# genomicepidemiology/ccphylo

Measured on AMD Instinct MI355X. Metric: taxa-pairs/sec (dist) + NJ iterations/sec at N taxa, 1/2/4/8 MI355X, higher is better.
Workload: dtype u2 packed codes -> MX-fp4 MFMA (exact integer counts), f64 LT and tree

## Files before the change

ccphylo_amd/csrc/ccg_dnj_form.h:

```cpp
#pragma once
#include <stdio.h>
#include <stdlib.h>

#ifdef __HIPCC__
#define CCG_FORM_HD __host__ __device__ __forceinline__
#else
#define CCG_FORM_HD inline
#endif

#define DNJ_B 128
#define DNJ_BANDS 64
#define DNJ_BANDS_MAX 128
#define SEG 2048
#define LB_SEG_DEFAULT (2 * SEG)
#define TBF 1024
#define FIND_RPT 16
#define PLAN_MAXB 256
#define UHIST 64

CCG_FORM_HD int dnj_umax(int n, int seg) { return n > 2 ? (n - 2) / seg + 1 : 1; }

struct DnjGrid {
	int scan_div = 4, scan_max = 2048, seg_mul = 0, prefold_n = 0;
	int small_wave = 0, adapt_rows = 500;
	int sphase_b = 512;
	int plan_help = 256;
	int scan_cmp = 1, cmp_blocks = 1024;
	long long prune_cells = 20000000;
	int prune_on = 1;
	int s_top = 0, s_bands = -1, s_split_n = 16384, plan_qdelay = 2, scan_wave = -1, plan_multi = 1;
	int plan_regsel = 0, plan_fr = FIND_RPT;
	int test_withhold = 0;
	int join_pf = 1;
	int scan_fold = 0;
	int scan_prune = 2;
	int lb = 1, lb_min_n = 16384;
	int lb_groups = 0;
	int seg_lb = 0, seg_lb_knob = 0;
	int scan_vblk = 1;
	void load() {
		if(const char *e = getenv("CCG_JOIN_PF")) join_pf = atoi(e);
		if(const char *e = getenv("CCG_SCAN_FOLD")) scan_fold = atoi(e);
		if(const char *e = getenv("CCG_SCAN_PRUNE")) scan_prune = atoi(e);
		if(const char *e = getenv("CCG_SCAN_VBLK")) scan_vblk = atoi(e);
		if(const char *e = getenv("CCG_S_TOP")) s_top = atoi(e) > 0 ? atoi(e) : 0;
		if(const char *e = getenv("CCG_S_BANDS")) s_bands = atoi(e) >= 0 ? atoi(e) : -1;
		if(const char *e = getenv("CCG_S_SPLIT_N")) s_split_n = atoi(e);
		if(const char *e = getenv("CCG_SCAN_DIV")) scan_div = atoi(e) > 0 ? atoi(e) : 4;
		if(const char *e = getenv("CCG_SCAN_MAX")) scan_max = atoi(e) > 0 ? atoi(e) : 2048;
		if(const char *e = getenv("CCG_SEG_MUL")) seg_mul = atoi(e) > 0 ? atoi(e) : 0;
		if(const char *e = getenv("CCG_PREFOLD_N")) prefold_n = atoi(e) >= 0 ? atoi(e) : 0;
		if(const char *e = getenv("CCG_SCAN_ADAPT")) adapt_rows = atoi(e) > 0 ? atoi(e) : 0;
		if(const char *e = getenv("CCG_SPHASE_BLOCKS")) sphase_b = atoi(e) > 0 ? atoi(e) : 512;
		if(const char *e = getenv("CCG_PLAN_HELP")) plan_help = atoi(e) >= 0 && atoi(e) < 512 ? atoi(e) : 256;
		if(const char *e = getenv("CCG_SCAN_CMP")) scan_cmp = atoi(e);
		if(const char *e = getenv("CCG_PRUNE_CELLS")) prune_cells = atoll(e) > 0 ? atoll(e) : 0;
		prune_on = 1;
		if(const char *e = getenv("CCG_SCAN_CMPB")) cmp_blocks = atoi(e) > 0 ? atoi(e) : 1024;
		if(const char *e = getenv("CCG_PLAN_QDELAY")) plan_qdelay = atoi(e) >= 0 ? atoi(e) : 2;
		if(const char *e = getenv("CCG_SCAN_WAVE")) scan_wave = atoi(e);
		if(const char *e = getenv("CCG_PLAN_MULTI")) plan_multi = atoi(e);
		if(const char *e = getenv("CCG_PLAN_REGSEL")) plan_regsel = atoi(e);
		if(const char *e = getenv("CCG_PLAN_FR")) plan_fr = atoi(e) < 1 ? 1 : atoi(e) > FIND_RPT ? FIND_RPT : atoi(e);
		if(const char *e = getenv("CCG_TEST_WITHHOLD")) test_withhold = atoi(e) & 3;
		if(const char *e = getenv("CCG_SCAN_LB")) lb = atoi(e);
		if(const char *e = getenv("CCG_LB_MIN_N")) lb_min_n = atoi(e);
		if(const char *e = getenv("CCG_LB_GROUPS")) lb_groups = atoi(e);
		if(const char *e = getenv("CCG_SEG_LB")) {
			char *end;
			const long v = strtol(e, &end, 10);
			if(end != e && !*end && v == 0) seg_lb_knob = -1;
			else if(end != e && !*end && v >= 64 && v <= 8 * SEG && v % 64 == 0) seg_lb_knob = (int) v;
			else fprintf(stderr, "ccphylo_amd: CCG_SEG_LB=%s ignored (0, or a multiple of 64 up to %d)\n", e, 8 * SEG);
		}
	}
	int plan_flags(bool prune = false, int helpers = 0) const {
		return (plan_qdelay & 0x3fff) | (test_withhold & 3) << 14 | (plan_regsel ? 0 : 1 << 16) | ((plan_fr - 1) & 15) << 17 | (prune ? 1 << 21 : 0) |
		       (helpers & 511) << 22;
	}
	unsigned plan_blocks(int n) const {
		if(!plan_multi) return 1;
		const int step = (TBF - 64) * plan_fr;
		const int g = (n - 1 + step - 1) / step;
		return (unsigned) (g < 1 ? 1 : g > PLAN_MAXB ? PLAN_MAXB : g);
	}
	int scan_mode(int n, int et = 8) const {
		return scan_wave >= 0 ? scan_wave : n > 16384 || small_wave ? (et == 8 ? 9 : 20) : 0;
	}
	int seg(int n) const {
		int m = seg_mul ? seg_mul : n / (8 * SEG);
		m = m < 1 ? 1 : m > 8 ? 8 : m;
		return m * SEG;
	}
	int seg_bounded(int n) const { return seg_lb_knob > 0 || seg_lb > seg(n) ? seg_lb : seg(n); }
	bool prefold(int n) const { return n > prefold_n; }
	int top(int n) const {
		const int t = s_top ? s_top : n > s_split_n ? 16 : DNJ_B;
		return t < 1 ? 1 : t > DNJ_B ? DNJ_B : t;
	}
	int bands(int n) const {
		int b = s_bands >= 0 ? s_bands : n > s_split_n ? DNJ_BANDS : 0;
		b = b > DNJ_BANDS_MAX ? DNJ_BANDS_MAX : b;
		return top(n) + b > DNJ_B ? DNJ_B - top(n) : b;
	}
	unsigned sphase_blocks() const { return sphase_b; }
	unsigned scan(int n) const {
		const long long g = (n + scan_div - 1) / scan_div;
		return (unsigned) (g < scan_max ? g : scan_max);
	}
};

enum ScanKernel {
	SCAN_BLOCK,
	SCAN_WAVE,
	SCAN_WAVE16,
	SCAN_GROUP,
	SCAN_GROUP_CMP
};
enum ScanSphase {
	SPHASE_NONE,
	SPHASE_SCAN,
	SPHASE_COMPACT
};
struct ScanForm {
	ScanKernel kernel;
	bool stream;
	int G, UC;
	int prune;
	bool cmp;
	bool lb;
	bool tfold;
	int helpers;
	ScanSphase sphase;
	bool fold;
	int sfold;
	unsigned grid;
	int launches;
	int seg;
};

inline int dnj_scan_base(int sm) {
	return sm <= 0 ? 0 : sm < 4 ? 1 : sm == 9 || sm == 21 || sm > 23 ? sm : sm < 20 ? 4 : 20;
}

inline ScanForm dnj_scan_form(const DnjGrid &g, int n, int et, bool gen, bool have_lbm) {
	const int sm = dnj_scan_base(g.scan_mode(n, et));
	const bool grp = sm == 20 || sm == 21, prefold = g.prefold(n);
	ScanForm f = {};
	f.tfold = prefold && g.scan_fold && sm >= 1;
	const bool lbseg = have_lbm && g.seg_lb > 0 && !gen && sm >= 4 && g.scan_cmp && !f.tfold &&
	                   dnj_umax(n, g.seg_bounded(n)) < UHIST;
	f.seg = lbseg ? g.seg_bounded(n) : g.seg(n);
	const bool fits = dnj_umax(n, f.seg) < UHIST;
	if(!gen && g.bands(n) && prefold && sm >= 4 && sm <= 23) {
		if(g.scan_prune == 1 && g.scan_fold) f.prune = 1;
		else if(g.scan_prune == 2 && g.prune_on && !g.scan_fold && (!grp || (g.scan_cmp && fits))) f.prune = 2;
	}
	f.helpers = f.prune == 2 ? g.plan_help : 0;
	f.sphase = f.prune != 2 ? SPHASE_NONE : g.plan_help ? SPHASE_COMPACT : SPHASE_SCAN;
	f.cmp = !gen && sm >= 4 && g.scan_cmp && !f.tfold && f.prune != 1 && fits;
	if(gen || sm < 4) f.kernel = sm >= 1 ? SCAN_WAVE : SCAN_BLOCK;
	else if(have_lbm && f.cmp && grp && g.lb_groups && f.prune == 0) {
		f.kernel = SCAN_GROUP_CMP;
		f.lb = true;
		f.G = 4;
		f.UC = 8;
	} else if(have_lbm && f.cmp) {
		f.kernel = SCAN_WAVE16;
		f.lb = true;
	} else if(grp) {
		f.kernel = f.cmp ? SCAN_GROUP_CMP : SCAN_GROUP;
		f.G = sm == 21 ? 8 : 4;
		f.UC = sm == 21 ? 4 : 8;
	} else {
		f.kernel = SCAN_WAVE16;
		f.stream = sm == 9;
	}
	f.grid = f.cmp && g.scan(n) > (unsigned) g.cmp_blocks ? (unsigned) g.cmp_blocks : g.scan(n);
	f.fold = prefold && !f.tfold;
	f.sfold = f.prune == 2;
	f.launches = 1 + (f.sphase != SPHASE_NONE) + f.fold;
	return f;
}

inline ScanForm dnj_scan_form_shard(const DnjGrid &g, int n, int et, bool have_lbm) {
	const int sm = g.scan_mode(n, et);
	ScanForm f = {};
	f.kernel = sm >= 4 ? SCAN_WAVE16 : sm >= 1 ? SCAN_WAVE : SCAN_BLOCK;
	f.stream = sm == 9;
	f.lb = have_lbm && sm >= 4;
	f.grid = g.scan(n);
	f.launches = 1;
	f.seg = g.seg(n);
	return f;
}
```

ccphylo_amd/csrc/ccg_dnj_search.h:

```cpp
#pragma once
#include <stdlib.h>
#include "ccg_tree_common.h"
#include "ccg_dnj_form.h"

struct DenseRows {
	__host__ __device__ __forceinline__ bool owns(long long) const { return true; }
	__host__ __device__ __forceinline__ long long row(long long r) const { return tri(r); }
};

#define SEG_S 1024
#define SEL_RPL 8
#define SEL_STEPS 8
#define FIND_CHUNKS 2048
#define REPLAY_CAP 2048
#define JOIN_UPRE 2048
#define FOLD_BLOCKS 256
#define SRDY_REP 64


template <int ET, bool GEN, int NT, int UNR, class Rows>
__device__ __forceinline__ void row_segment_min(const Rows &rows, const typename Elem<ET>::T *__restrict__ D, double bs,
                                                const double *__restrict__ sD, const int *__restrict__ N, int r,
                                                int c0, int c1, int Nr, double sDr, int isub, int Nm, double sDm,
                                                double &q, int &idx) {
	const typename Elem<ET>::T *row = D + rows.row(r);
	typename Elem<ET>::T v[UNR];
	int nk[UNR];
	double sk[UNR];
	auto load = [&](int base, typename Elem<ET>::T (&lv)[UNR], int (&lk)[UNR], double (&ls)[UNR]) {
#pragma unroll
		for(int m = 0; m < UNR; ++m) {
			int c = base + m * NT + (int) threadIdx.x;
			c = c < c1 ? c : c1 - 1;
			lv[m] = row[c];
			lk[m] = GEN ? N[c] : Nr;
			ls[m] = sD[c];
		}
	};
	load(c0, v, nk, sk);
	for(int base = c0; base < c1; base += UNR * NT) {
		typename Elem<ET>::T vn[UNR];
		int nkn[UNR];
		double skn[UNR];
		const bool more = base + UNR * NT < c1;
		if(more) load(base + UNR * NT, vn, nkn, skn);
#pragma unroll
		for(int m = 0; m < UNR; ++m) {
			const int c = base + m * NT + (int) threadIdx.x;
			const double d = Elem<ET>::get(v[m], bs);
			const int Nc = c == isub ? Nm : nk[m];
			const double sc = c == isub ? sDm : sk[m];
			const double x = qcrit(Nr, Nc, d, sDr, sc);
			const bool take = c < c1 && 0 <= d && qarg_better(x, c, q, idx);
			q = take ? x : q;
			idx = take ? c : idx;
		}
		if(more) {
#pragma unroll
			for(int m = 0; m < UNR; ++m) {
				v[m] = vn[m];
				nk[m] = nkn[m];
				sk[m] = skn[m];
			}
		}
	}
}

__device__ __forceinline__ void fold_units(const double *__restrict__ uq, const int *__restrict__ uj, int ua, int ub,
                                           double &q, int &idx) {
	for(int u = ua; u < ub; u += 4) {
		double oq[4];
		int oi[4];
#pragma unroll
		for(int m = 0; m < 4; ++m) {
			const int v = u + m < ub ? u + m : ub - 1;
			oq[m] = uq[v];
			oi[m] = uj[v];
		}
#pragma unroll
		for(int m = 0; m < 4; ++m) {
			if(u + m < ub && qarg_better(oq[m], oi[m], q, idx)) {
				q = oq[m];
				idx = oi[m];
			}
		}
	}
}

__device__ __forceinline__ void qarg_block_reduce1(double &q, int &idx, double *sq, int *si) {
	qarg_wave_reduce(q, idx);
	const int lane = threadIdx.x & 63, wid = threadIdx.x >> 6, nw = blockDim.x >> 6;
	if(lane == 0) {
		sq[wid] = q;
		si[wid] = idx;
	}
	__syncthreads();
	if(threadIdx.x == 0) {
		for(int w = 1; w < nw; ++w) {
			if(qarg_better(sq[w], si[w], q, idx)) {
				q = sq[w];
				idx = si[w];
			}
		}
	}
}

template <int ET, class Rows>
__global__ void k_init_hnj(Rows rows, const typename Elem<ET>::T *__restrict__ D, int n, double bs,
                           const double *__restrict__ sD, const int *__restrict__ N,
                           double *__restrict__ Q, int *__restrict__ P) {
	int i = blockIdx.x * (blockDim.x >> 6) + (threadIdx.x >> 6);
	int lane = threadIdx.x & 63;
	if(i >= n || !rows.owns(i)) return;
	double bq = DBL_MAX, bd = DBL_MAX;
	int bj = 0;
	const typename Elem<ET>::T *row = D + rows.row(i);
	int Ni = N[i];
	double sDi = sD[i];
	for(int j = lane; j < i; j += 64) {
		double d = Elem<ET>::get(row[j], bs);
		const double q = qcrit(Ni, N[j], d, sDi, sD[j]);
		const bool take = (0 <= d) & ((q < bq) | ((q == bq) & ((d < bd) | ((d == bd) & (j > bj)))));
		bq = take ? q : bq;
		bd = take ? d : bd;
		bj = take ? j : bj;
	}
#pragma unroll
	for(int off = 32; off > 0; off >>= 1) {
		const double oq = __shfl_xor(bq, off, 64), od = __shfl_xor(bd, off, 64);
		const int oj = __shfl_xor(bj, off, 64);
		const bool take = (oq < bq) | ((oq == bq) & ((od < bd) | ((od == bd) & (oj > bj))));
		bq = take ? oq : bq;
		bd = take ? od : bd;
		bj = take ? oj : bj;
	}
	if(lane == 0) {
		Q[i] = bq;
		P[i] = bj;
	}
}

template <int UNUSED = 0>
__global__ __launch_bounds__(TB) void k_dnj_prep(TreeBufs b, int n) {
	__shared__ double sq[TB / 64];
	__shared__ int si[TB / 64];
	double q = DBL_MAX;
	int idx = 0;
	for(int i = 1 + threadIdx.x; i < n; i += blockDim.x) {
		if(qarg_better(b.Q[i], i, q, idx)) {
			q = b.Q[i];
			idx = i;
		}
	}
	qarg_block_reduce(q, idx, sq, si);
// ... 1000 lines not shown
		if(last) {
			__hip_atomic_store(b.rf + e, q, __ATOMIC_RELAXED, __HIP_MEMORY_SCOPE_AGENT);
			__hip_atomic_store(b.rj + e, j, __ATOMIC_RELAXED, __HIP_MEMORY_SCOPE_AGENT);
			asm volatile("s_waitcnt vmcnt(0)" ::: "memory");
			if(CHUNKS) {
				const int c = e >> 6, ce = T - (c << 6) < 64 ? T - (c << 6) : 64;
				const unsigned seen = __hip_atomic_fetch_add(b.ccnt + c, 1u, __ATOMIC_RELAXED, __HIP_MEMORY_SCOPE_AGENT);
				if((int) seen == ce - 1) {
					chunk_done = 1;
					__hip_atomic_store(b.ccnt + c, 0u, __ATOMIC_RELAXED, __HIP_MEMORY_SCOPE_AGENT);
				}
			}
			if(sent) {
				const unsigned sseen = __hip_atomic_fetch_add(&b.ctl->scnt, 1u, __ATOMIC_RELAXED,
				                                              __HIP_MEMORY_SCOPE_AGENT);
				s_done = (int) sseen == b.ctl->pS - 1;
			}
		}
	}
	if(__shfl(s_done, 0)) {
		__builtin_amdgcn_fence(__ATOMIC_ACQUIRE, "wavefront");
		s_table(b, n);
	}
	if(!CHUNKS || !__shfl(chunk_done, 0)) return;
	__builtin_amdgcn_fence(__ATOMIC_ACQUIRE, "wavefront");
	const int c = e >> 6, e2 = (c << 6) + lane;
	const bool valid = e2 < T;
	const int rr = valid ? b.crow[e2] : 0;
	const double bnd = valid ? b.cbnd[e2] : 0.0;
	const double f = valid ? __hip_atomic_load(b.rf + e2, __ATOMIC_RELAXED, __HIP_MEMORY_SCOPE_AGENT) : DBL_MAX;
	const int fj = valid ? __hip_atomic_load(b.rj + e2, __ATOMIC_RELAXED, __HIP_MEMORY_SCOPE_AGENT) : 0;
	const double mq = readlane_d(wave_incl_min(f), 63);
	const unsigned long long hm = __ballot(valid && f == mq);
	const unsigned long long bm = __ballot(valid && !(f >= bnd));
	const int first = hm ? __ffsll((long long) hm) - 1 : 0;
	const int fr = __shfl(rr, first), fjj = __shfl(fj, first);
	if(lane == 0) {
		b.chg[c] = mq;
		b.chr[c] = fr;
		b.chj[c] = fjj;
		b.chb[c] = bm != 0ull;
	}
}

__device__ __forceinline__ void tail_unit(const FoldTail &, const TreeBufs &b, int n, int u, int ua, int ub, int r,
                                          double q, int j, int e, int T, bool sent = false) {
	(void) r;
	fold_arrive(b, n, b.cq, b.cj, u, ua, ub, q, j, e, T, sent);
}

template <int ET, bool GEN, class Rows, class Tail = NoTail>
__global__ __launch_bounds__(TB) void k_dnj_scan(const typename Elem<ET>::T *__restrict__ D, double bs, TreeBufs b,
                                                 int n, Rows rows, int seg, Tail tail = Tail()) {
	__shared__ int erow[REPLAY_CAP];
	__shared__ double sq[TB / 64];
	__shared__ int si[TB / 64];
	TreeCtl *ctl = b.ctl;
	const int tid = threadIdx.x;
	TS_ENTRY(2);
	TS(2, 0);
	TS_SAMP(0);
	const int r0 = b.crow[tid];
	const int done = ctl->done, T = ctl->T;
	if(done) return;
	tail.begin(b, n);
	if(T == 0) return;
	const int umax = dnj_umax(n, seg), nunits = T * umax;
	if((int) blockIdx.x >= nunits) return;
	const bool lds = T <= REPLAY_CAP;
	if(lds) {
		if(tid < T) erow[tid] = r0;
		for(int e = TB + tid; e < T; e += TB) erow[e] = b.crow[e];
	}
	__syncthreads();
	TS(2, 1);
	TS_SAMP(1);
	for(int u = blockIdx.x; u < nunits; u += gridDim.x) {
		const int e = u / umax, ua = e * umax;
		const int r = lds ? erow[e] : b.crow[e];
		const int c0 = (u - ua) * seg;
		if(c0 >= r || !rows.owns(r)) continue;
		const int c1 = c0 + seg < r ? c0 + seg : r;
		const int Nr = GEN ? b.N[r] : n;
		double qq = DBL_MAX;
		int idx = 0;
		row_segment_min<ET, GEN, TB, SEG / TB / 2>(rows, D, bs, b.sD, b.N, r, c0, c1, Nr, b.sD[r], -1, 0, 0.0, qq, idx);
		qarg_block_reduce1(qq, idx, sq, si);
		if(tid == 0) tail.unit(b, n, u, ua, ua + dcdiv(r, seg), r, qq, idx);
		if(u + (int) gridDim.x < nunits) __syncthreads();
	}
	TS(2, 2);
	TS_SAMP(2);
	TS_EXIT(2);
}

template <int ET, bool GEN, class Rows, class Tail = NoTail, int SCAN_UW = 8>
__global__ __launch_bounds__(TB) void k_dnj_scan_w(const typename Elem<ET>::T *__restrict__ D, double bs, TreeBufs b,
                                                   int n, Rows rows, int seg, Tail tail = Tail()) {
	__shared__ int erow[REPLAY_CAP];
	TreeCtl *ctl = b.ctl;
	const int tid = threadIdx.x, lane = tid & 63;
	const int r0 = b.crow[tid];
	const int done = ctl->done, T = ctl->T;
	if(done) return;
	tail.begin(b, n);
	if(T == 0) return;
	const int umax = dnj_umax(n, seg), nunits = T * umax;
	if((int) blockIdx.x * (TB / 64) >= nunits) return;
	const bool lds = T <= REPLAY_CAP;
	if(lds) {
		if(tid < T) erow[tid] = r0;
		for(int e = TB + tid; e < T; e += TB) erow[e] = b.crow[e];
	}
	__syncthreads();
	const int gw = blockIdx.x * (TB / 64) + (tid >> 6), nw = gridDim.x * (TB / 64);
	for(int u = gw; u < nunits; u += nw) {
		const int e = u / umax, ua = e * umax;
		const int r = lds ? erow[e] : b.crow[e];
		const int c0 = (u - ua) * seg;
		if(c0 >= r || !rows.owns(r)) continue;
		const int c1 = c0 + seg < r ? c0 + seg : r;
		const int Nr = GEN ? b.N[r] : n;
		const double sDr = b.sD[r];
		const typename Elem<ET>::T *row = D + rows.row(r);
		double q = DBL_MAX;
		int idx = 0;
		for(int base = c0; base < c1; base += 64 * SCAN_UW) {
			typename Elem<ET>::T v[SCAN_UW];
			double sk[SCAN_UW];
			int nk[SCAN_UW];
#pragma unroll
			for(int m = 0; m < SCAN_UW; ++m) {
				int c = base + 64 * m + lane;
				c = c < c1 ? c : c1 - 1;
				v[m] = row[c];
				sk[m] = b.sD[c];
				nk[m] = GEN ? b.N[c] : Nr;
			}
#pragma unroll
			for(int m = 0; m < SCAN_UW; ++m) {
				const int c = base + 64 * m + lane;
				const double d = Elem<ET>::get(v[m], bs);
				const double x = qcrit(Nr, nk[m], d, sDr, sk[m]);
				const bool take = c < c1 && 0 <= d && qarg_better(x, c, q, idx);
				q = take ? x : q;
				idx = take ? c : idx;
			}
		}
		qarg_wave_reduce(q, idx);
		tail_unit(tail, b, n, u, ua, ua + dcdiv(r, seg), r, q, idx, e, T);
	}
}

static_assert(8 * SEG <= 4 * 64 * LBW && SEG_S <= 4 * 64 * LBW, "lb_unit loads at most 256 block bounds per unit");
template <int ET>
__device__ __forceinline__ int lb_unit(const typename Elem<ET>::T *__restrict__ row, double bs, const TreeBufs &b, int n,
                                       int r, int c0, int c1, double sDr, double &q, int &idx, int isub,
                                       double sDm, bool ubinf) {
	typedef typename Elem<ET>::T T;
	constexpr int BB = ET == 8 ? LB_BB_D : LB_BB_N;
	const int lane = threadIdx.x & 63;
	const int bl0 = c0 / LBW, nbk = (c1 - c0 + LBW - 1) / LBW;
	const double ub = ubinf ? INFINITY : b.ubq[r];
	unsigned lbb[4];
	double msb[4];
	const unsigned *line = lb_line(b, r);
#pragma unroll
	for(int h = 0; h < 4; ++h) {
		const int t = lane + 64 * h;
		lbb[h] = t < nbk ? line[bl0 + t] : 0u;
		msb[h] = t < nbk ? b.msd[bl0 + t] : 0.0;
	}
	unsigned long long need[4];
#pragma unroll
	for(int h = 0; h < 4; ++h) {
		const int t = lane + 64 * h;
		const double lb = qcrit(n, n, (double) __uint_as_float(lbb[h]), sDr, msb[h]);
		need[h] = __ballot(t < nbk && !(lb > ub));
	}
	int loaded = 0;
	int h = 0;
	while(true) {
		int blk[BB], nb = 0;
		while(nb < BB && h < 4) {
			if(!need[h]) {
				++h;
				continue;
			}
			const int bit = __ffsll((long long) need[h]) - 1;
			need[h] &= need[h] - 1;
			blk[nb++] = bl0 + 64 * h + bit;
		}
		if(!nb) break;
		T v[BB];
		double sk[BB];
#pragma unroll
		for(int m = 0; m < BB; ++m) {
			int c = (m < nb ? blk[m] : blk[0]) * LBW + lane;
			c = c < c1 ? c : c1 - 1;
			v[m] = row[c];
			sk[m] = b.sD[c];
		}
#pragma unroll
		for(int m = 0; m < BB; ++m) {
			const int c = (m < nb ? blk[m] : blk[0]) * LBW + lane;
			const double d = Elem<ET>::get(v[m], bs);
			const double x = qcrit(n, n, d, sDr, c == isub ? sDm : sk[m]);
			if(m < nb && c < c1 && 0 <= d && qarg_better(x, c, q, idx)) {
				q = x;
				idx = c;
			}
		}
		for(int m = 0; m < nb; ++m) loaded += (blk[m] + 1) * LBW < c1 ? LBW : c1 - blk[m] * LBW;
	}
	return (c1 - c0) - loaded;
}

template <int ET, int G>
__device__ __forceinline__ long long lb_unit_g(const typename Elem<ET>::T *const (&row)[G], double bs, const TreeBufs &b,
                                               int n, const int (&r)[G], const bool (&act)[G], int c0,
                                               const int (&c1)[G], int cmax, const double (&sDr)[G], double (&q)[G],
                                               int (&idx)[G]) {
	typedef typename Elem<ET>::T T;
	constexpr int BB = ET == 8 ? LB_BB_D : LB_BB_N;
	const int lane = threadIdx.x & 63;
	const int bl0 = c0 / LBW, nbkm = (cmax - c0 + LBW - 1) / LBW;
	double msb[4];
#pragma unroll
	for(int h = 0; h < 4; ++h) {
		const int t = lane + 64 * h;
		msb[h] = t < nbkm ? b.msd[bl0 + t] : 0.0;
	}
	unsigned long long need[G][4], any[4] = {0, 0, 0, 0};
#pragma unroll
	for(int k = 0; k < G; ++k) {
		const int nbk = act[k] ? (c1[k] - c0 + LBW - 1) / LBW : 0;
		const double ub = act[k] ? b.ubq[r[k]] : 0.0;
		const unsigned *line = lb_line(b, act[k] ? r[k] : 1);
#pragma unroll
		for(int h = 0; h < 4; ++h) {
			const int t = lane + 64 * h;
			const unsigned lbv = t < nbk ? line[bl0 + t] : 0u;
			const double lb = qcrit(n, n, (double) __uint_as_float(lbv), sDr[k], msb[h]);
			need[k][h] = __ballot(t < nbk && !(lb > ub));
			any[h] |= need[k][h];
		}
	}
	long long loaded = 0;
	int h = 0;
	while(true) {
		int blk[BB], nb = 0;
		while(nb < BB && h < 4) {
			if(!any[h]) {
				++h;
				continue;
			}
			const int bit = __ffsll((long long) any[h]) - 1;
			any[h] &= any[h] - 1;
			blk[nb++] = 64 * h + bit;
		}
		if(!nb) break;
		double sk[BB];
		T v[G][BB];
#pragma unroll
		for(int m = 0; m < BB; ++m) {
			const int t = m < nb ? blk[m] : blk[0];
			int c = (bl0 + t) * LBW + lane;
			sk[m] = b.sD[c < cmax ? c : cmax - 1];
#pragma unroll
			for(int k = 0; k < G; ++k) {
				v[k][m] = 0;
				if((need[k][t >> 6] >> (t & 63)) & 1)
					v[k][m] = row[k][c < c1[k] ? c : c1[k] - 1];
			}
		}
#pragma unroll
		for(int m = 0; m < BB; ++m) {
			const int t = m < nb ? blk[m] : blk[0];
			const int c = (bl0 + t) * LBW + lane;
#pragma unroll
			for(int k = 0; k < G; ++k) {
				if(m >= nb || !((need[k][t >> 6] >> (t & 63)) & 1)) continue;
				const double d = Elem<ET>::get(v[k][m], bs);
				const double x = qcrit(n, n, d, sDr[k], sk[m]);
				if(c < c1[k] && 0 <= d && qarg_better(x, c, q[k], idx[k])) {
					q[k] = x;
					idx[k] = c;
				}
			}
		}
		for(int m = 0; m < nb; ++m) {
			const int c = (bl0 + blk[m]) * LBW;
#pragma unroll
			for(int k = 0; k < G; ++k)
				if((need[k][blk[m] >> 6] >> (blk[m] & 63)) & 1) loaded += c + LBW < c1[k] ? LBW : c1[k] - c;
		}
	}
	long long span = 0;
#pragma unroll
	for(int k = 0; k < G; ++k) span += act[k] ? c1[k] - c0 : 0;
	return span - loaded;
}

template <int ET, class Rows, class Tail = NoTail, bool STREAM = false, int PRUNE = 0, bool CMP = false, bool LB = false>
__global__ __launch_bounds__(TB) void k_dnj_scan_v(const typename Elem<ET>::T *__restrict__ D, double bs, TreeBufs b,
                                                   int n, Rows rows, int seg, Tail tail = Tail()) {
	typedef typename Elem<ET>::T T;
	static_assert(!(LB && PRUNE == 1), "the block bounds serve the compacted scan (its S units fold elsewhere)");
	constexpr int VEC = 16 / (int) sizeof(T), UV = VEC >= 16 ? 1 : 16 / VEC;
	__shared__ int erow[REPLAY_CAP];
	TreeCtl *ctl = b.ctl;
	const int tid = threadIdx.x, lane = tid & 63;
	TS_ENTRY(2);
	TS(2, 0);
	TS_SAMP(0);
	const int r0 = b.crow[tid];
	const int done = ctl->done, Tn = ctl->T;
	if(done) return;
	tail.begin(b, n);
	if(Tn == 0) return;
	const int umax = dnj_umax(n, seg), nunits = Tn * umax;
	const int nSp = PRUNE ? ctl->pS : 0;
	const int su0 = PRUNE == 1 && nSp ? b.pS_uo[nSp] : 0;
	if((int) blockIdx.x * (TB / 64) >= (nunits > su0 ? nunits : su0)) return;
	const bool lds = Tn <= REPLAY_CAP;
	if(lds) {
		if(tid < Tn) erow[tid] = r0;
		for(int e = TB + tid; e < Tn; e += TB) erow[e] = b.crow[e];
	}
	__syncthreads();
	const int gw = blockIdx.x * (TB / 64) + (tid >> 6), nw = gridDim.x * (TB / 64);
	TS(2, 1);
	TS_SAMP(1);
	__shared__ int s_uo[DNJ_B + 1];
	int su = 0;
	if(PRUNE == 1 && nSp) {
		for(int t = tid; t <= nSp; t += TB) s_uo[t] = b.pS_uo[t];
		__syncthreads();
		su = s_uo[nSp];
	}
	long long pruned = 0, lbskip = 0;
	auto unit = [&](int u, int e, int r, int c0, int c1, bool skip, bool sent, int sua, int sub) {
		const int ua = e * umax;
		if(skip) {
			pruned += c1 - c0;
			tail_unit(tail, b, n, u, ua, ua + dcdiv(r, seg), r, DBL_MAX, 0, e, Tn);
			return;
		}
		const double sDr = b.sD[r];
		const long long ro = rows.row(r);
		const T *row = D + ro;
		if(LB) {
			double q = DBL_MAX;
			int idx = 0;
			lbskip += lb_unit<ET>(row, bs, b, n, r, c0, c1, sDr, q, idx);
			qarg_wave_reduce(q, idx);
			tail_unit(tail, b, n, u, ua, ua + dcdiv(r, seg), r, q, idx, e, Tn);
			return;
		}
		const int a = (int) ((VEC - (ro + c0) % VEC) % VEC);
		const int ca = c0 + a < c1 ? c0 + a : c1;
		const int nv = (c1 - ca) / VEC, ce = ca + nv * VEC;
		double q = DBL_MAX;
		int idx = 0;
		auto cell = [&](int c) {
			const double d = Elem<ET>::get(row[c], bs);
			const double x = qcrit(n, n, d, sDr, b.sD[c]);
			if(0 <= d && qarg_better(x, c, q, idx)) {
				q = x;
				idx = c;
			}
		};
		if(lane < ca - c0) cell(c0 + lane);
		if(lane < c1 - ce) cell(ce + lane);
		uint4 w[UV];
		double sk[UV][VEC];
		const bool sda = STREAM && (ca & 1) == 0;
		auto load = [&](int v0) {
#pragma unroll
			for(int m = 0; m < UV; ++m) {
				int k = v0 + 64 * m + lane;
				k = k < nv ? k : nv - 1;
				const uint4 *src = (const uint4 *) (row + ca + VEC * k);
				if(STREAM) {
					typedef unsigned u4v __attribute__((ext_vector_type(4)));
					const u4v x = __builtin_nontemporal_load((const u4v *) src);
					w[m] = make_uint4(x.x, x.y, x.z, x.w);
				} else {
					w[m] = *src;
				}
				if(sda) {
#pragma unroll
					for(int t = 0; t < VEC; t += 2) {
						const double2 x = *(const double2 *) (b.sD + ca + VEC * k + t);
						sk[m][t] = x.x;
						sk[m][t + 1] = x.y;
					}
				} else {
#pragma unroll
					for(int t = 0; t < VEC; ++t) sk[m][t] = b.sD[ca + VEC * k + t];
				}
			}
		};
		auto compare = [&](int v0) {
#pragma unroll
			for(int m = 0; m < UV; ++m) {
				const int k = v0 + 64 * m + lane;
				const T *ev = (const T *) &w[m];
#pragma unroll
				for(int t = 0; t < VEC; ++t) {
					const int c = ca + VEC * k + t;
					const double d = Elem<ET>::get(ev[t], bs);
					const double x = qcrit(n, n, d, sDr, sk[m][t]);
					const bool take = k < nv && 0 <= d && qarg_better(x, c, q, idx);
					q = take ? x : q;
					idx = take ? c : idx;
				}
			}
		};
		for(int v0 = 0; v0 < nv; v0 += 64 * UV) {
			load(v0);
			compare(v0);
		}
		qarg_wave_reduce(q, idx);
		if(PRUNE == 1 && sent) fold_arrive(b, n, b.uq, b.uj, u, sua, sub, q, idx, e, Tn, true);
		else tail_unit(tail, b, n, u, ua, ua + dcdiv(r, seg), r, q, idx, e, Tn);
	};
	for(int v = gw; v < su; v += nw) {
		int lo = 0, hi = nSp;
		while(hi - lo > 1) {
			const int mid = (lo + hi) >> 1;
			if(s_uo[mid] <= v) lo = mid; else hi = mid;
		}
		const int r = b.pS_row[lo], c0 = (v - s_uo[lo]) * SEG_S;
		unit(v, b.pS_ent[lo], r, c0, c0 + SEG_S < r ? c0 + SEG_S : r, false, true, s_uo[lo], s_uo[lo + 1]);
	}
	SBound sb;
	bool have_sb = false, ready = false;
	if(PRUNE == 1 && nSp && (int) blockIdx.x * (TB / 64) < nunits) {
		__shared__ int s_ready;
		__syncthreads();
		if(tid == 0) s_ready = s_table_wait(b, n);
		__syncthreads();
		ready = s_ready;
	}
	if(PRUNE == 2 && nSp) ready = b.srdy[0] == (unsigned) n;
	int nu = 0;
	(void) nu;
	if(CMP && PRUNE == 2 && nSp) {
		int H = 0;
		const int pb = ctl->pblk;
		for(int g = 0; g < pb; ++g) H += b.uhist[g * UHIST + lane];
		const int inch = wave_incl_sum(H), Eall = __builtin_amdgcn_readlane(inch, 63) - inch;
		const int cnt = b.bcnt[lane];
		const int incc = wave_incl_sum(cnt), totc = __builtin_amdgcn_readlane(incc, 63);
		const int Es = totc - incc;
		const int C = totc - incc + cnt;
		int R;
		const int P = wave_excl_scan(Es, &R);
		for(int v = gw; v < R; v += nw) {
			const int k = 63 - __clzll((long long) __ballot(Es > 0 && P <= v));
			const int j = v - __shfl(P, k);
			const int ub = 63 - __clzll((long long) __ballot(lane > k && C > j));
			const int p = j - (__shfl(C, ub) - __shfl(cnt, ub));
			const int e = b.blist[__shfl(Eall, ub) + p];
			const int r = lds ? erow[e] : b.crow[e];
			const int c0 = k * seg;
			TS_U(2 * nu);
			unit(e * umax + k, e, r, c0, c0 + seg < r ? c0 + seg : r, false, false, 0, 0);
			TS_U(2 * nu + 1);
			++nu;
		}
	} else if(CMP) {
		int H = 0;
		const int pb = ctl->pblk;
		for(int g = 0; g < pb; ++g) H += b.uhist[g * UHIST + lane];
		int tot;
		const int inc = wave_incl_sum(H);
		tot = __builtin_amdgcn_readlane(inc, 63);
		const int E = tot - inc;
		int R;
		const int P = wave_excl_scan(E, &R);
		for(int v = gw; v < R; v += nw) {
			const unsigned long long mk = __ballot(E > 0 && P <= v);
			const int k = 63 - __clzll((long long) mk);
			const int e = v - __shfl(P, k);
			const int r = lds ? erow[e] : b.crow[e];
			const int c0 = k * seg;
			bool skip = false;
			if(PRUNE == 2 && nSp) {
				if(b.eS[e]) continue;
				if(!have_sb) {
					sb.load(b, n, ready);
					have_sb = true;
				}
				skip = sb.ok && !(b.cbnd[e] < sb.at(r));
			}
			TS_U(2 * nu);
			unit(e * umax + k, e, r, c0, c0 + seg < r ? c0 + seg : r, skip, false, 0, 0);
			TS_U(2 * nu + 1);
			++nu;
		}
	}
	for(int u = CMP ? nunits : gw; u < nunits; u += nw) {
		const int e = u / umax, ua = e * umax;
		const int r = lds ? erow[e] : b.crow[e];
		const int c0 = (u - ua) * seg;
		if(c0 >= r || !rows.owns(r)) continue;
// ... 170 lines not shown
		if(tid < Tn) erow[tid] = r0;
		for(int e = TB + tid; e < Tn; e += TB) erow[e] = b.crow[e];
	}
	int su = 0;
	if(PRUNE && nSp)
		for(int t = tid; t <= nSp; t += TB) s_uo[t] = b.pS_uo[t];
	__syncthreads();
	if(PRUNE && nSp) su = s_uo[nSp];
	const int gw = blockIdx.x * (TB / 64) + (tid >> 6), nw = gridDim.x * (TB / 64);
	long long pruned = 0;
	for(int v = gw; v < su; v += nw) {
		int lo = 0, hi = nSp;
		while(hi - lo > 1) {
			const int mid = (lo + hi) >> 1;
			if(s_uo[mid] <= v) lo = mid; else hi = mid;
		}
		const int e = b.pS_ent[lo], r = b.pS_row[lo], c0 = (v - s_uo[lo]) * SEG_S;
		const int c1 = c0 + SEG_S < r ? c0 + SEG_S : r;
		const double sDr = b.sD[r];
		const T *row = D + tri(r);
		double q = DBL_MAX;
		int idx = 0;
		for(int base = c0; base < c1; base += 64 * UC) {
			double sk[UC];
			T vv[UC];
#pragma unroll
			for(int m = 0; m < UC; ++m) {
				const int c = base + 64 * m + lane;
				const int cc = c < c1 ? c : c1 - 1;
				sk[m] = b.sD[cc];
				vv[m] = row[cc];
			}
#pragma unroll
			for(int m = 0; m < UC; ++m) {
				const int c = base + 64 * m + lane;
				const double d = Elem<ET>::get(vv[m], bs);
				const double x = qcrit(n, n, d, sDr, sk[m]);
				const bool take = c < c1 && 0 <= d && qarg_better(x, c, q, idx);
				q = take ? x : q;
				idx = take ? c : idx;
			}
		}
		qarg_wave_reduce(q, idx);
		fold_arrive(b, n, b.uq, b.uj, v, s_uo[lo], s_uo[lo + 1], q, idx, e, Tn, true);
	}
	SBound sb;
	bool have_sb = false, ready = false;
	if(PRUNE && nSp && (int) blockIdx.x * (TB / 64) < nunits) {
		__shared__ int s_ready;
		__syncthreads();
		if(tid == 0) s_ready = s_table_wait(b, n);
		__syncthreads();
		ready = s_ready;
	}
	for(int u = gw; u < nunits; u += nw) {
		const int g = u / umax, s = u - g * umax, c0 = s * seg;
		int r[G], c1[G];
		bool act[G], skip[G];
		int cmax = c0;
#pragma unroll
		for(int k = 0; k < G; ++k) {
			const int e = g * G + k;
			r[k] = e < Tn ? (lds ? erow[e] : b.crow[e]) : 0;
			act[k] = e < Tn && c0 < r[k];
			skip[k] = false;
			if(PRUNE && nSp && act[k] && b.eS[e]) act[k] = false;
		}
		if(PRUNE && nSp) {
			bool any = false;
#pragma unroll
			for(int k = 0; k < G; ++k) any = any || act[k];
			if(any && !have_sb) {
				sb.load(b, n, ready);
				have_sb = true;
			}
			if(any && sb.ok) {
#pragma unroll
				for(int k = 0; k < G; ++k) {
					if(act[k] && !(b.cbnd[g * G + k] < sb.at(r[k]))) {
						skip[k] = true;
						act[k] = false;
					}
				}
			}
		}
#pragma unroll
		for(int k = 0; k < G; ++k) {
			c1[k] = act[k] ? (c0 + seg < r[k] ? c0 + seg : r[k]) : c0;
			cmax = c1[k] > cmax ? c1[k] : cmax;
		}
		if(PRUNE) {
#pragma unroll
			for(int k = 0; k < G; ++k) {
				if(!skip[k]) continue;
				const int e = g * G + k;
				pruned += (c0 + seg < r[k] ? c0 + seg : r[k]) - c0;
				tail_unit(FoldTail(), b, n, e * umax + s, e * umax, e * umax + dcdiv(r[k], seg), r[k], DBL_MAX, 0, e,
				          Tn);
			}
		}
		if(cmax == c0) continue;
		double sDr[G], q[G];
		int idx[G];
		const T *row[G];
#pragma unroll
		for(int k = 0; k < G; ++k) {
			sDr[k] = act[k] ? b.sD[r[k]] : 0.0;
			row[k] = D + tri(act[k] ? r[k] : 1);
			q[k] = DBL_MAX;
			idx[k] = 0;
		}
		for(int base = c0; base < cmax; base += 64 * UC) {
			double sk[UC];
			T v[G][UC];
#pragma unroll
			for(int m = 0; m < UC; ++m) {
				const int c = base + 64 * m + lane;
				sk[m] = b.sD[c < cmax ? c : cmax - 1];
#pragma unroll
				for(int k = 0; k < G; ++k) v[k][m] = row[k][c < c1[k] ? c : (act[k] ? c1[k] - 1 : 0)];
			}
#pragma unroll
			for(int m = 0; m < UC; ++m) {
				const int c = base + 64 * m + lane;
#pragma unroll
				for(int k = 0; k < G; ++k) {
					const double d = Elem<ET>::get(v[k][m], bs);
					const double x = qcrit(n, n, d, sDr[k], sk[m]);
					const bool take = c < c1[k] && 0 <= d && qarg_better(x, c, q[k], idx[k]);
					q[k] = take ? x : q[k];
					idx[k] = take ? c : idx[k];
				}
			}
		}
#pragma unroll
		for(int k = 0; k < G; ++k) {
			if(!act[k]) continue;
			double qq = q[k];
			int ii = idx[k];
			qarg_wave_reduce(qq, ii);
			const int e = g * G + k;
			if(FOLD) {
				tail_unit(FoldTail(), b, n, e * umax + s, e * umax, e * umax + dcdiv(r[k], seg), r[k], qq, ii, e, Tn);
			} else if(lane == 0) {
				b.cq[e * umax + s] = qq;
				b.cj[e * umax + s] = ii;
			}
		}
	}
	if(PRUNE && pruned && lane == 0)
		atomicAdd((unsigned long long *) &ctl->cells_pruned, (unsigned long long) pruned);
}

template <int ET, int G, int UC, bool PRUNE2, bool LB = false>
__global__ __launch_bounds__(TB) void k_dnj_scan_gc(const typename Elem<ET>::T *__restrict__ D, double bs, TreeBufs b,
                                                    int n, int seg) {
	typedef typename Elem<ET>::T T;
	static_assert(!(LB && PRUNE2), "the bounded row groups run without S-bound pruning");
	const TreeCtl *ctl = b.ctl;
	const int tid = threadIdx.x, lane = tid & 63;
	const int done = ctl->done, Tn = ctl->T;
	if(done || Tn == 0) return;
	const int umax = dnj_umax(n, seg);
	const int nSp = PRUNE2 ? ctl->pS : 0;
	const bool surv = PRUNE2 && nSp > 0;
	const int gw = blockIdx.x * (TB / 64) + (tid >> 6), nw = gridDim.x * (TB / 64);
	int H = 0;
	const int pb = ctl->pblk;
	for(int g = 0; g < pb; ++g) H += b.uhist[g * UHIST + lane];
	const int inch = wave_incl_sum(H), Eall = __builtin_amdgcn_readlane(inch, 63) - inch;
	const int cnt = surv ? b.bcnt[lane] : H;
	const int incc = wave_incl_sum(cnt), totc = __builtin_amdgcn_readlane(incc, 63);
	const int Es = totc - incc;
	const int C = Es + cnt;
	const int NG = (Es + G - 1) / G;
	int R;
	const int PG = wave_excl_scan(NG, &R);
	long long lbskip = 0;
	for(int v = gw; v < R; v += nw) {
		const int k = 63 - __clzll((long long) __ballot(NG > 0 && PG <= v));
		const int grp = v - __shfl(PG, k), EsK = __shfl(Es, k);
		const int c0 = k * seg;
		int r[G], e[G], c1[G];
		bool act[G];
		int cmax = c0;
#pragma unroll
		for(int t = 0; t < G; ++t) {
			const int pos = grp * G + t;
			act[t] = pos < EsK;
			e[t] = 0;
			r[t] = 1;
			if(act[t]) {
				if(surv) {
					const int ub = 63 - __clzll((long long) __ballot(lane > k && C > pos));
					const int pin = pos - (__shfl(C, ub) - __shfl(cnt, ub));
					e[t] = b.blist[__shfl(Eall, ub) + pin];
				} else {
					e[t] = pos;
				}
				r[t] = b.crow[e[t]];
			}
			c1[t] = act[t] ? (c0 + seg < r[t] ? c0 + seg : r[t]) : c0;
			cmax = c1[t] > cmax ? c1[t] : cmax;
		}
		double sDr[G], q[G];
		int idx[G];
		const T *row[G];
#pragma unroll
		for(int t = 0; t < G; ++t) {
			sDr[t] = act[t] ? b.sD[r[t]] : 0.0;
			row[t] = D + tri(act[t] ? r[t] : 1);
			q[t] = DBL_MAX;
			idx[t] = 0;
		}
		if(LB) lbskip += lb_unit_g<ET, G>(row, bs, b, n, r, act, c0, c1, cmax, sDr, q, idx);
		for(int base = c0; !LB && base < cmax; base += 64 * UC) {
			double sk[UC];
			T vv[G][UC];
#pragma unroll
			for(int m = 0; m < UC; ++m) {
				const int c = base + 64 * m + lane;
				sk[m] = b.sD[c < cmax ? c : cmax - 1];
#pragma unroll
				for(int t = 0; t < G; ++t) vv[t][m] = row[t][c < c1[t] ? c : (act[t] ? c1[t] - 1 : 0)];
			}
#pragma unroll
			for(int m = 0; m < UC; ++m) {
				const int c = base + 64 * m + lane;
#pragma unroll
				for(int t = 0; t < G; ++t) {
					const double d = Elem<ET>::get(vv[t][m], bs);
					const double x = qcrit(n, n, d, sDr[t], sk[m]);
					const bool take = c < c1[t] && 0 <= d && qarg_better(x, c, q[t], idx[t]);
					q[t] = take ? x : q[t];
					idx[t] = take ? c : idx[t];
				}
			}
		}
#pragma unroll
		for(int t = 0; t < G; ++t) {
			if(!act[t]) continue;
			double qq = q[t];
			int ii = idx[t];
			qarg_wave_reduce(qq, ii);
			if(lane == 0) {
				b.cq[e[t] * umax + k] = qq;
				b.cj[e[t] * umax + k] = ii;
			}
		}
	}
	if(LB && lbskip && lane == 0)
		atomicAdd((unsigned long long *) (b.lbskip + (long long) ((blockIdx.x * (TB / 64) + (tid >> 6)) % LB_SCAN) * LB_SLOT),
		          (unsigned long long) lbskip);
}

template <int UNUSED = 0>
__global__ __launch_bounds__(TB) void k_dnj_fold(TreeBufs b, int n, int seg, int sfold = 0) {
	const TreeCtl *ctl = b.ctl;
	if(ctl->done) return;
	const int T = ctl->T, lane = threadIdx.x & 63, umax = dnj_umax(n, seg);
	sfold = sfold && ctl->pS > 0;
	if(blockIdx.x == 0 && threadIdx.x < UHIST) b.bcnt[threadIdx.x] = 0;
	const int nc = (T + 63) >> 6;
	const int w0 = (int) (blockIdx.x * (TB / 64) + (threadIdx.x >> 6)), nw = (int) (gridDim.x * (TB / 64));
	for(int c = w0; c < nc; c += nw) {
		const int e = (c << 6) + lane;
		const bool valid = e < T;
		const int r = valid ? b.crow[e] : 0;
		const double bnd = valid ? b.cbnd[e] : 0.0;
		const bool sdone = sfold && valid && b.eS[e], pruned = sfold && valid && !sdone && b.ePr[e];
		const int ua = e * umax, ub = ua + (valid && !sdone && !pruned ? dcdiv(r, seg) : 0);
		double q = sdone ? b.rf[e] : DBL_MAX;
		int idx = sdone ? b.rj[e] : 0;
		int u = ua;
		for(; u + 4 <= ub; u += 4) {
			double oq[4];
			int oi[4];
#pragma unroll
			for(int m = 0; m < 4; ++m) {
				oq[m] = b.cq[u + m];
				oi[m] = b.cj[u + m];
			}
#pragma unroll
			for(int m = 0; m < 4; ++m) {
				if(qarg_better(oq[m], oi[m], q, idx)) {
					q = oq[m];
					idx = oi[m];
				}
			}
		}
		for(; u < ub; ++u) {
			const double oq = b.cq[u];
			const int oi = b.cj[u];
			if(qarg_better(oq, oi, q, idx)) {
				q = oq;
				idx = oi;
			}
		}
		if(valid && !sdone) {
			b.rf[e] = q;
			b.rj[e] = idx;
		}
		const double mq = readlane_d(wave_incl_min(valid ? q : DBL_MAX), 63);
		const unsigned long long hm = __ballot(valid && q == mq);
		const unsigned long long bm = __ballot(valid && !(q >= bnd));
		const int first = hm ? __ffsll((long long) hm) - 1 : 0;
		const int fr = __shfl(r, first), fj = __shfl(idx, first);
		if(lane == 0) {
			b.chg[c] = mq;
			b.chr[c] = fr;
			b.chj[c] = fj;
			b.chb[c] = bm != 0ull;
		}
	}
}

__device__ __forceinline__ void replay_wave(int total, double m0, const int *e_row, const int *e_j, const double *e_b,
                            const double *e_f, unsigned char *e_acc, bool writer, const TreeBufs &b, int &pi,
                            int &pj, bool *had_bad, int n, unsigned char *acc_out = nullptr) {
	(void) n;
	const int lane = threadIdx.x & 63;
	int bad = 0;
	for(int e0 = lane; e0 < total; e0 += 256) {
		double f[4], bb[4];
#pragma unroll
		for(int k = 0; k < 4; ++k) {
			const int e = e0 + 64 * k < total ? e0 + 64 * k : total - 1;
			f[k] = e_f[e];
			bb[k] = e_b[e];
		}
#pragma unroll
		for(int k = 0; k < 4; ++k) {
			if(e0 + 64 * k < total) {
				bad |= !(f[k] >= bb[k]);
				e_acc[e0 + 64 * k] = 0;
			}
		}
	}
	const bool any_bad = __any(bad);
	*had_bad = any_bad;
	wave_sync();
	TS(3, 6);
	if(any_bad) {
		double m = m0;
		int start = 0;
		for(;;) {
			int hit = -1;
			double cm = m;
			for(int c0 = start; c0 < total; c0 += 64) {
				const int e = c0 + lane;
				const bool valid = e < total;
				const double f = valid ? e_f[e] : DBL_MAX, bb = valid ? e_b[e] : DBL_MAX;
				const bool good = valid && f >= bb;
				const double x = wave_incl_min(good ? f : DBL_MAX);
				double pre = dpp_d<DPP_WAVE_SHR1, 0xF>(DBL_MAX, x);
				pre = pre < cm ? pre : cm;
				const unsigned long long hm = __ballot(valid && !good && bb < pre);
				if(hm) {
					hit = c0 + __ffsll((long long) hm) - 1;
					break;
				}
				const double last = readlane_d(x, 63);
				cm = last < cm ? last : cm;
			}
			if(hit < 0) break;
			if(lane == 0) e_acc[hit] = 1;
			m = e_f[hit];
			start = hit + 1;
// ... 77 lines not shown
```

ccphylo_amd/csrc/ccg_tree_common.h:

```cpp
#pragma once
#include <string.h>
#include "ccg_internal.h"

#define TB 256
#define NJ_RB 8
#define NJ_SEG (TB * 8)

struct Entry {
	double f, bnd;
	int row, j;
};

struct TreeCtl {
	int done;
	int final_n;
	int njoins;
	int i, j;
	double Li, Lj, Dij;
	int cand;
	double cand_q;
	int cand_p;
	int pos_i, pos_j;
	int nS, smin;
	int ntop;
	int T;
	double m0;
	unsigned tick;
	int neg, exact, method, has_missing;
	int serial_sums, serial_replays;
	int chain_sums;
	int xnj;
	double xsum;
	long long rows, cells, cells_top, cells_rest;
	long long ref_rows, ref_cells;
	int hj, hi, hjb, hib;
	int rtotal;
	int pS;
	unsigned scnt;
	long long cells_pruned;
	long long cells_help;
	long long cells_lbskip;
	int vtag;
	int pblk;
	int xs_why[8];
};

struct XsBlk;
struct XsCross;
struct XsTie;

struct TreeBufs {
	double *sD, *Q, *contrib;
	int *N, *P;
	int *S, *uoff;
	double *Sb;
	double *uq;
	int *uj;
	Entry *Sent;
	double *ef, *eb;
	int *erow, *ej;
	unsigned char *eacc;
	int *crow;
	double *cbnd;
	int *coff;
	double *cq;
	int *cj;
	double *wsum, *wabs;
	int *wcnt, *wexp;
	double *qpart;
	int *ipart;
	double *cfq;
	int *cfp;
	long long *fpart;
	double *bmq;
	int *bmr, *bmp;
	double *bmqp;
	int *Spos;
	int *cslot;
	double *rf;
	int *rj;
	ccg_join *joins;
	TreeCtl *ctl;
	unsigned long long *xagg;
	XsBlk *xblk;
	XsCross *xcr;
	XsTie *xti;
	unsigned long long *ppub;
	unsigned long long *jpub;
	double *chg;
	int *chr, *chj, *chb;
	unsigned *ecnt, *ccnt;
	int *pS_row, *pS_ent, *pS_uo;
	double *pS_q, *pS_bnd;
	unsigned char *eS;
	double *bmv, *vsuf;
	int *bcnt, *blist;
	unsigned char *ePr;
	unsigned long long *shdr;
	double *sfq;
	int *sfj;
	unsigned *ecS;
	int *uhist;
	unsigned *srdy;
	int maxu;
	unsigned *lbm;
	double *msd;
	double *ubq;
	long long lbs;
	int lbw;
	int xs_allpre;
	long long *lbskip;
};

#define LBW 64
#define LB_SLOT 16
#define LB_SCAN 4096
#define LB_HELP 8192

__device__ __forceinline__ unsigned *lb_line(const TreeBufs &b, int r) {
	const long long p = b.lbw ? (long long) ((r >> 3) / b.lbw) * 8 + (r & 7) : r;
	return b.lbm + p * b.lbs;
}

__device__ __forceinline__ unsigned lb_bits(double x) {
	return x > 0.0 ? __float_as_uint(__double2float_rd(x)) : 0u;
}


struct TreeWork {
	TreeBufs b;
	void *mem;
};
int ccg_tree_alloc(DevMem &mem, TreeWork *w, int n, hipStream_t st);
size_t ccg_tree_bytes(int n);
int ccg_tree_linkage_impl(ccg_ctx *ctx, const ccg_tree_args *a, void *Dd, ccg_join *joins, int *njoins, int *final_n,
                          double *final_d, int64_t *stats);

__host__ __device__ static inline unsigned cdiv(long long a, long long b) { return (unsigned) ((a + b - 1) / b); }
__device__ __forceinline__ int dcdiv(int a, int b) { return (a + b - 1) / b; }

__device__ __forceinline__ int block_excl_scan(int v, int *s, int *total) {
	const int lane = threadIdx.x & 63, wid = threadIdx.x >> 6, nw = blockDim.x >> 6;
	const int x = wave_incl_sum(v);
	if(lane == 63) s[wid] = x;
	__syncthreads();
	int pre = 0, tot = 0;
	for(int w = 0; w < nw; ++w) {
		if(w < wid) pre += s[w];
		tot += s[w];
	}
	__syncthreads();
	*total = tot;
	return pre + x - v;
}

__device__ __forceinline__ void wave_sync() {
	__builtin_amdgcn_fence(__ATOMIC_RELEASE, "wavefront");
	__builtin_amdgcn_wave_barrier();
	__builtin_amdgcn_fence(__ATOMIC_ACQUIRE, "wavefront");
}

__device__ __forceinline__ int wave_excl_scan(int v, int *total) {
	const int inc = wave_incl_sum(v);
	*total = __builtin_amdgcn_readlane(inc, 63);
	return inc - v;
}

__device__ __forceinline__ double wave_sum_fixed(double x) {
#define S_(C, R) x += dpp_d<C, R>(0.0, x);
	CCG_DPP_STEPS(S_)
#undef S_
	return readlane_d(x, 63);
}

__device__ __forceinline__ int wave_sum_int(int v) { return __builtin_amdgcn_readlane(wave_incl_sum(v), 63); }
__device__ __forceinline__ long long wave_sum_int(long long v) { return readlane_l(wave_incl_sum_l(v), 63); }
__device__ __forceinline__ int wave_min_int(int v) { return __builtin_amdgcn_readlane(wave_incl_min_i(v), 63); }
__device__ __forceinline__ unsigned wave_min_u32(unsigned v) {
#define S_(C, R)                                                          \
	{                                                                     \
		const unsigned t_ = (unsigned) dpp_i<C, R>((int) 0xFFFFFFFFu, (int) v); \
		v = t_ < v ? t_ : v;                                              \
	}
	CCG_DPP_STEPS(S_)
#undef S_
	return (unsigned) __builtin_amdgcn_readlane((int) v, 63);
}
__device__ __forceinline__ double wave_max_d(double x) {
#define S_(C, R)                                   \
	{                                              \
		const double t_ = dpp_d<C, R>(-DBL_MAX, x); \
		x = t_ > x ? t_ : x;                       \
	}
	CCG_DPP_STEPS(S_)
#undef S_
	return readlane_d(x, 63);
}

static __device__ void limb_length(double *Li, double *Lj, double sDi, double sDj, int Ni_, int Nj_, double Dij, int neg) {
	int Ni = Ni_ - 2, Nj = Nj_ - 2;
	if(0 < Ni && 0 < Nj) {
		double delta = ((sDi - Dij) / Ni) - ((sDj - Dij) / Nj);
		*Li = (Dij + delta) / 2;
		*Lj = (Dij - delta) / 2;
		if(!neg) {
			if(*Li < 0) {
				*Lj = Dij;
				*Li = 0;
			} else if(*Lj < 0) {
				*Li = Dij;
				*Lj = 0;
			}
		}
	} else if(0 < Ni) {
		*Li = 0;
		*Lj = Dij;
	} else if(0 < Nj) {
		*Li = Dij;
		*Lj = 0;
	} else {
		*Li = *Lj = Dij / 2;
	}
}

__device__ __forceinline__ int low_exp(double x) {
	unsigned long long u = (unsigned long long) __double_as_longlong(x);
	int ex = (int) ((u >> 52) & 0x7FF);
	unsigned long long m = u & ((1ull << 52) - 1);
	if(ex == 0x7FF) return INT32_MIN;
	if(ex == 0) {
		if(m == 0) return INT32_MAX;
		return -1074 + __ffsll((long long) m) - 1;
	}
	m |= 1ull << 52;
	return ex - 1075 + __ffsll((long long) m) - 1;
}

__device__ __forceinline__ void update_partials(const TreeBufs &b, int n, bool exact, int k, double d, int cnt,
                                                int slot) {
	__shared__ double ssum[TB / 64], sabs[TB / 64];
	__shared__ int scnt[TB / 64], sexp[TB / 64];
	if(exact && k < n) b.contrib[k] = d;
	const double s = wave_sum_fixed(d), a = wave_sum_fixed(fabs(d));
	cnt = wave_sum_int(cnt);
	const int e = wave_min_int(low_exp(d));
	const int lane = threadIdx.x & 63, wid = threadIdx.x >> 6;
	if(lane == 0) {
		ssum[wid] = s;
		sabs[wid] = a;
		scnt[wid] = cnt;
		sexp[wid] = e;
	}
	__syncthreads();
	if(threadIdx.x == 0) {
		double t = 0, ta = 0;
		int c = 0, te = INT32_MAX;
		for(int w = 0; w < TB / 64; ++w) {
			t += ssum[w];
			ta += sabs[w];
			c += scnt[w];
			te = sexp[w] < te ? sexp[w] : te;
		}
		b.wsum[slot] = t;
		b.wabs[slot] = ta;
		b.wcnt[slot] = c;
		b.wexp[slot] = te;
	}
}


static __device__ void fold_update_wave(const TreeBufs &b, int G, bool exact, bool general, double *sd_out, int *nj_out,
                                 bool *need_serial) {
	const int lane = threadIdx.x & 63;
	*need_serial = false;
	if(general) {
		*sd_out = b.wsum[0];
		*nj_out = 1 + b.wcnt[0];
		return;
	}
	double s = 0, a = 0;
	int c = 0, e = INT32_MAX;
	for(int g = lane; g < G; g += 64) {
		s += b.wsum[g];
		a += b.wabs[g];
		c += b.wcnt[g];
		int oe = b.wexp[g];
		e = oe < e ? oe : e;
	}
	const double sd = wave_sum_fixed(s);
	a = wave_sum_fixed(a);
	c = wave_sum_int(c);
	e = wave_min_int(e);
	if(exact) {
		bool provable = e != INT32_MIN && (e == INT32_MAX || (e > -1000 && a * (1.0 + 1e-9) < ldexp(1.0, 53 + e)));
		*need_serial = !provable;
	}
	*sd_out = sd;
	*nj_out = 1 + c;
}

#define XC_CH 1024
template <int NT>
static __device__ double serial_sum_t(const double *__restrict__ c, int n) {
	constexpr int PER = XC_CH / NT;
	__shared__ __attribute__((aligned(16))) double buf[2 * XC_CH];
	__shared__ double s_sd;
	double sd = 0;
	double nxt[PER];
#pragma unroll
	for(int m = 0; m < PER; ++m) {
		int kk = m * NT + threadIdx.x;
		buf[m * NT + threadIdx.x] = kk < n ? c[kk] : 0.0;
	}
	__syncthreads();
	for(int c0 = 0, p = 0; c0 < n; c0 += XC_CH, p ^= 1) {
#pragma unroll
		for(int m = 0; m < PER; ++m) {
			int kk = c0 + XC_CH + m * NT + threadIdx.x;
// ... 967 lines not shown
```

ccphylo_amd/csrc/ccg_tree_run.h:

```cpp
#pragma once
#include <vector>
#include "ccg_tree_common.h"

struct KTimer {
	bool on = false;
	hipStream_t st;
	hipEvent_t ev[1025];
	int cls[1025];
	int used;
	long long cnt[CCG_NKSTAT], ns[CCG_NKSTAT];
	void init(hipStream_t s, bool enable) {
		abort();
		on = enable;
		st = s;
		used = 0;
		memset(cnt, 0, sizeof(cnt));
		memset(ns, 0, sizeof(ns));
		if(on) {
			for(int k = 0; k < 1025; ++k) hipEventCreate(&ev[k]);
			hipEventRecord(ev[0], st);
			used = 1;
		}
	}
	void harvest() {
		hipEventSynchronize(ev[used - 1]);
		for(int k = 1; k < used; ++k) {
			float ms = 0;
			hipEventElapsedTime(&ms, ev[k - 1], ev[k]);
			cnt[cls[k]] += 1;
			ns[cls[k]] += (long long) (ms * 1.0e6);
		}
		hipEvent_t t = ev[0];
		ev[0] = ev[used - 1];
		ev[used - 1] = t;
		used = 1;
	}
	void mark(int c) {
		if(!on) return;
		cls[used] = c;
		hipEventRecord(ev[used++], st);
		if(used == 1025) harvest();
	}
	void abort() {
		if(!on) return;
		for(int k = 0; k < 1025; ++k) hipEventDestroy(ev[k]);
		on = false;
	}
	void finish() {
		if(!on) return;
		harvest();
		abort();
	}
};

static inline TreeCtl tree_ctl_seed(const ccg_tree_args *a) {
	TreeCtl c;
	memset(&c, 0, sizeof(c));
	c.neg = (a->flags & 2) != 0;
	c.exact = a->exact != 0;
	c.method = a->method;
	c.hj = c.hi = -1;
	return c;
}

struct TreeStats {
	long long rows = 0, cells = 0, launches = 0, us = 0;
	long long cells_top = 0, cells_rest = 0, serial_sums = 0, chain_sums = 0;
	long long slot8 = 0;
	long long hard_columns = 0;
	long long ref_rows = 0, ref_cells = 0;
	void write(int64_t *stats, bool profile, const KTimer &kt) const {
		if(!stats) return;
		stats[0] = rows;
		stats[1] = cells;
		stats[2] = launches;
		stats[3] = us;
		if(!profile) return;
		for(int c = 0; c < CCG_NKSTAT; ++c) {
			stats[4 + 2 * c] = kt.cnt[c];
			stats[5 + 2 * c] = kt.ns[c];
		}
		const long long tail[8] = {cells_top, cells_rest, serial_sums, chain_sums, slot8, hard_columns, ref_rows, ref_cells};
		for(int k = 0; k < 8; ++k) stats[4 + 2 * CCG_NKSTAT + k] = tail[k];
	}
};

template <class Ctl>
struct TreeRun {
	ccg_ctx *ctx;
	hipStream_t st;
	const Ctl *dctl;
	KTimer kt;
	long long launches = 0;
	int since_check = 0;
	float ms = 0;
	TreeRun(ccg_ctx *c, const Ctl *device_ctl) : ctx(c), st(c->stream), dctl(device_ctl) {}
	TreeRun(const TreeRun &) = delete;
	~TreeRun() {
		kt.abort();
		hipStreamSynchronize(st);
	}
	int read_ctl(Ctl &h) {
		CCG_CHECK(hipMemcpyAsync(&h, dctl, sizeof(h), hipMemcpyDeviceToHost, st));
		CCG_CHECK(hipStreamSynchronize(st));
		return CCG_OK;
	}
	int begin(const Ctl &seed, bool profile) {
		CCG_CHECK(hipMemcpyAsync((void *) dctl, &seed, sizeof(seed), hipMemcpyHostToDevice, st));
		CCG_CHECK(hipEventRecord(ctx->ev0, st));
		kt.init(st, profile);
		return CCG_OK;
	}
	int check(Ctl &h, bool *read) {
		*read = ++since_check == 1024;
		if(!*read) return CCG_OK;
		since_check = 0;
		return read_ctl(h);
	}
	int finish(Ctl &h, int n, const ccg_join *dev_joins, ccg_join *joins, int *njoins, int *final_n, double *final_d) {
		CCG_CHECK(hipEventRecord(ctx->ev1, st));
		kt.finish();
		CCG_TRY(read_ctl(h));
		CCG_CHECK(hipEventElapsedTime(&ms, ctx->ev0, ctx->ev1));
		if(h.done && h.final_n < 0) {
			ccg_set_last_msg("k_dnj_plan / k_dnj_join: a block's bounded wait on another block timed out");
			return CCG_EHIP;
		}
		*njoins = h.njoins;
		*final_n = h.done ? h.final_n : n;
		*final_d = -1.0;
		if(h.njoins) CCG_CHECK(hipMemcpyAsync(joins, dev_joins, (size_t) h.njoins * sizeof(ccg_join), hipMemcpyDeviceToHost, st));
		return CCG_OK;
	}
	template <int ET>
	int final_distance(const void *dev_src, double bs, double *final_d) {
		typename Elem<ET>::T v;
		CCG_CHECK(hipMemcpyAsync(&v, dev_src, sizeof(v), hipMemcpyDeviceToHost, st));
		CCG_CHECK(hipStreamSynchronize(st));
		*final_d = (ET == 8 || ET == 4) ? (double) v : v / bs;
		return CCG_OK;
	}
	TreeStats stats() const {
		TreeStats s;
		s.launches = launches;
		s.us = (long long) (ms * 1000.0);
		return s;
	}
	int end() {
		CCG_CHECK(hipStreamSynchronize(st));
		return CCG_OK;
	}
};

struct LbLayout {
	long long LS;
	size_t lbb, msb, ubb, skb;
	size_t bytes() const { return lbb + msb + ubb + skb; }
};
static inline LbLayout lb_layout(int n0, long long owned_rows) {
	LbLayout l;
	l.LS = (n0 + LBW - 1) / LBW;
	l.lbb = ((size_t) owned_rows * l.LS * 4 + 255) & ~(size_t) 255;
	l.msb = ((size_t) (l.LS + 1) * 8 + 255) & ~(size_t) 255;
	l.ubb = ((size_t) n0 * 8 + 255) & ~(size_t) 255;
	l.skb = (size_t) (LB_SCAN + LB_HELP) * LB_SLOT * 8;
	return l;
}
static inline int lb_bind(TreeBufs &b, void *mem, const LbLayout &l, int lbw, hipStream_t st) {
	char *m = (char *) mem;
	b.lbm = (unsigned *) m;
	b.msd = (double *) (m + l.lbb);
	b.ubq = (double *) (m + l.lbb + l.msb);
	b.lbs = l.LS;
	b.lbw = lbw;
	b.lbskip = (long long *) (m + l.lbb + l.msb + l.ubb);
	CCG_CHECK(hipMemsetAsync(b.lbskip, 0, l.skb, st));
	return CCG_OK;
}
static inline int lb_harvest(const TreeBufs &b, size_t slots, hipStream_t st, TreeCtl &h) {
	if(!b.lbskip) return CCG_OK;
	std::vector<long long> sl(slots * LB_SLOT);
	CCG_CHECK(hipMemcpyAsync(sl.data(), b.lbskip, sl.size() * 8, hipMemcpyDeviceToHost, st));
	CCG_CHECK(hipStreamSynchronize(st));
	for(size_t x = 0; x < slots; ++x) {
		h.cells_lbskip += sl[x * LB_SLOT];
		h.cells_help -= sl[x * LB_SLOT + 1];
	}
	return CCG_OK;
}
```

ccphylo_amd/csrc/tree.hip:

```cpp
#include <string.h>
#include <stdio.h>
#include <vector>
#include <stdlib.h>
#include "ccg_tree_run.h"

#include "ccg_dnj_search.h"

static thread_local DnjGrid g_grid;

template <int ET>
__global__ __launch_bounds__(TB) void k_init_rows(const typename Elem<ET>::T *__restrict__ D, int n, double bs,
                                                  double *__restrict__ sD, int *__restrict__ N, TreeCtl *ctl) {
	__shared__ double buf[TB / 64][64];
	const int lane = threadIdx.x & 63, wid = threadIdx.x >> 6;
	const int k = blockIdx.x * (TB / 64) + wid;
	if(k >= n) return;
	double s = 0;
	int c = 1, miss = 0;
	const typename Elem<ET>::T *row = D + tri(k);
	for(int m0 = 0; m0 < k; m0 += 64) {
		int m = m0 + lane;
		double d = m < k ? Elem<ET>::get(row[m], bs) : 0.0;
		bool ok = m < k && 0 <= d;
		miss |= m < k && !ok;
		c += __popcll(__ballot(ok));
		buf[wid][lane] = ok ? d : 0.0;
		__builtin_amdgcn_wave_barrier();
		if(lane == 0) {
			int lim = k - m0 < 64 ? k - m0 : 64;
			for(int u = 0; u < lim; ++u) s += buf[wid][u];
		}
		__builtin_amdgcn_wave_barrier();
	}
	miss = __any(miss);
	if(lane == 0) {
		sD[k] = s;
		N[k] = c;
		if(miss) atomicOr(&ctl->has_missing, 1);
	}
}

template <int ET>
__global__ __launch_bounds__(TB) void k_init_cols(const typename Elem<ET>::T *__restrict__ D, int n, double bs,
                                                  double *__restrict__ sD, int *__restrict__ N, TreeCtl *ctl) {
	const int k = blockIdx.x * TB + threadIdx.x;
	if(k >= n) return;
	double s = sD[k];
	int c = N[k], miss = 0;
	for(int m = k + 1; m < n; ++m) {
		double d = Elem<ET>::get(D[tri(m) + k], bs);
		if(0 <= d) {
			s += d;
			++c;
		} else {
			miss = 1;
		}
	}
	sD[k] = s;
	N[k] = c;
	if(miss) atomicOr(&ctl->has_missing, 1);
}

template <int ET>
__device__ __forceinline__ void update_body(typename Elem<ET>::T *__restrict__ D, double bs, const TreeBufs &b, int n,
                                            int i, int j, double Dij, bool exact, int k, double Dik, double Dkj,
                                            double sDk, int Nk, int slot) {
	double d = 0;
	int cnt = 0;
	typename Elem<ET>::T v = 0;
	if(k < n && k != i && k != j) {
		d = (Dik + Dkj - Dij) / 2;
		d = d < 0 ? 0 : d;
		v = Elem<ET>::put(d, 0.25, bs);
		D[k < j ? tri(j) + k : tri(k) + j] = v;
		b.sD[k] = sDk - (Dik + Dkj - d);
		b.N[k] = Nk - 1;
		cnt = 1;
	}
	if(b.lbm) {
		const bool rowj = k < j;
		const unsigned x = lb_bits(Elem<ET>::get(v, bs));
		const unsigned mn = wave_min_u32(rowj ? x : 0xFFFFFFFFu);
		if((threadIdx.x & 63) == 0 && k < j) b.lbm[(long long) j * b.lbs + (k >> 6)] = mn;
		if(k > j && k < n && k != i) __hip_atomic_fetch_min(b.lbm + (long long) k * b.lbs + (j >> 6), x, __ATOMIC_RELAXED, __HIP_MEMORY_SCOPE_AGENT);
	}
	update_partials(b, n, exact, k, d, cnt, slot);
	if(exact) xs_join_row(b, n, slot, d, xs_tag(n));
}


template <int ET>
__device__ __forceinline__ void join_tail(typename Elem<ET>::T *__restrict__ D, double bs, const TreeBufs &b, int n,
                                          int general, int i, int j, int ci, int cj, typename Elem<ET>::T pij,
                                          typename Elem<ET>::T pik, typename Elem<ET>::T pkj, double sDk, int Nk,
                                          int neg, int nj, int exact) {
	TreeCtl *ctl = b.ctl;
	const int tid = threadIdx.x, k = blockIdx.x * TB + tid;
	const bool writer = blockIdx.x == 0;
	if(i == 0 && j == 0) {
		if(writer && tid == 0) {
			ctl->done = 1;
			ctl->final_n = n;
		}
		return;
	}
	const bool hit = i == ci && j == cj;
	const double Dij = Elem<ET>::get(hit ? pij : D[tri(i) + j], bs);
	double Dik = 0, Dkj = 0;
	if(!general && k < n && k != i && k != j) {
		Dik = Elem<ET>::get(hit ? pik : D[k < i ? tri(i) + k : tri(k) + i], bs);
		Dkj = Elem<ET>::get(hit ? pkj : D[k < j ? tri(j) + k : tri(k) + j], bs);
	}
	if(writer && tid == 0) {
		double Li, Lj;
		limb_length(&Li, &Lj, b.sD[i], b.sD[j], b.N[i], b.N[j], Dij, neg);
		ctl->i = i;
		ctl->j = j;
		ctl->Li = Li;
		ctl->Lj = Lj;
		ctl->Dij = Dij;
		ccg_join J;
		J.i = i;
		J.j = j;
		J.Li = Li;
		J.Lj = Lj;
		b.joins[nj] = J;
		ctl->njoins = nj + 1;
	}
	TS(3, 4);
	if(general) return;
	update_body<ET>(D, bs, b, n, i, j, Dij, exact, k, Dik, Dkj, sDk, Nk, blockIdx.x);
	TS(3, 5);
}

template <int ET>
__global__ __launch_bounds__(TB) void k_lb_init(const typename Elem<ET>::T *__restrict__ D, int n, double bs,
                                                TreeBufs b) {
	constexpr int BB = 8;
	const int lane = threadIdx.x & 63;
	const int r = blockIdx.x * (TB / 64) + (threadIdx.x >> 6);
	if(r >= n) return;
	if(r < (n + LBW - 1) / LBW) {
		const int c = r * LBW + lane;
		const double mx = wave_max_d(c < n ? b.sD[c] : -DBL_MAX);
		if(lane == 0) b.msd[r] = mx;
	}
	if(lane == 0) b.ubq[r] = INFINITY;
	const typename Elem<ET>::T *row = D + tri(r);
	const int nbk = (r + LBW - 1) / LBW;
	for(int u0 = 0; u0 < nbk; u0 += BB) {
		unsigned x[BB];
#pragma unroll
		for(int m = 0; m < BB; ++m) {
			const int c = (u0 + m) * LBW + lane;
			x[m] = u0 + m < nbk && c < r ? lb_bits(Elem<ET>::get(row[c], bs)) : 0xFFFFFFFFu;
		}
#pragma unroll
		for(int m = 0; m < BB; ++m) {
			const unsigned mn = wave_min_u32(x[m]);
			if(lane == 0 && u0 + m < nbk) b.lbm[(long long) r * b.lbs + u0 + m] = mn;
		}
	}
}

template <int ET, bool GEN>
__global__ __launch_bounds__(TB) void k_dnj_join(typename Elem<ET>::T *__restrict__ D, double bs, TreeBufs b, int n,
                                                 int general, int prefold, int seg) {
	__shared__ int e_row[DNJ_B + REPLAY_CAP], e_j[DNJ_B + REPLAY_CAP];
	__shared__ double e_b[DNJ_B + REPLAY_CAP], e_f[DNJ_B + REPLAY_CAP];
	__shared__ unsigned char e_acc[DNJ_B + REPLAY_CAP];
	__shared__ int s_pi, s_pj, s_stop, s_nj, s_neg, s_exact, s_nS, s_merged;
	__shared__ double s_m0;
	__shared__ double lq[JOIN_UPRE];
	__shared__ int lj[JOIN_UPRE];
	TreeCtl *ctl = b.ctl;
	const int tid = threadIdx.x, lane = tid & 63, wid = tid >> 6;
	const bool writer = blockIdx.x == 0;
	TS_ENTRY(3);
	TS(3, 0);
	const int k = blockIdx.x * TB + tid;
	int ci = ctl->pos_i, cj = ctl->pos_j;
	ci = ci < 0 || ci >= n ? 0 : ci;
	cj = cj < 0 || cj >= ci ? 0 : cj;
	typename Elem<ET>::T pik = 0, pkj = 0;
	double sDk = 0;
	int Nk = 0;
	if(!general && k < n) {
		sDk = b.sD[k];
		Nk = b.N[k];
		if(k != ci && k != cj) {
			pik = D[k < ci ? tri(ci) + k : tri(k) + ci];
			pkj = D[k < cj ? tri(cj) + k : tri(k) + cj];
		}
	}
	const typename Elem<ET>::T pij = D[tri(ci) + cj];
	if(prefold) {
#pragma unroll
		for(int m = 0; m < JOIN_UPRE / TB; ++m) {
			lq[tid + m * TB] = b.rf[tid + m * TB];
			lj[tid + m * TB] = b.rj[tid + m * TB];
		}
	} else {
#pragma unroll
		for(int m = 0; m < JOIN_UPRE / TB; ++m) {
			lq[tid + m * TB] = b.cq[tid + m * TB];
			lj[tid + m * TB] = b.cj[tid + m * TB];
		}
	}
	__syncthreads();
	if(wid == 0) {
		const int done = ctl->done, nS = ctl->nS, T = ctl->T;
		const bool merged = ctl->ntop != nS;
		const int pos_i = ctl->pos_i, pos_j = ctl->pos_j;
		const double m0 = ctl->m0;
		Entry se0, se1;
		se0 = b.Sent[lane];
		se1 = b.Sent[lane + 64];
		const int sp0 = merged ? b.Spos[lane] : lane, sp1 = merged ? b.Spos[lane + 64] : lane + 64;
		int rr[4], cs[4];
		double bb[4];
#pragma unroll
		for(int m = 0; m < 4; ++m) {
			cs[m] = merged ? b.cslot[lane + 64 * m] : nS + lane + 64 * m;
			rr[m] = b.crow[lane + 64 * m];
			bb[m] = b.cbnd[lane + 64 * m];
		}
		const int umax = dnj_umax(n, seg);
		if(lane == 0) {
			s_nj = ctl->njoins;
			s_neg = ctl->neg;
			s_exact = ctl->exact;
		}
		if(done) {
			if(lane == 0) s_stop = 1;
		} else {
			TS(3, 1);
			int pi = pos_i, pj = pos_j;
			const bool lds = T <= REPLAY_CAP;
			int *x_row = lds ? e_row : b.erow, *x_j = lds ? e_j : b.ej;
			double *x_b = lds ? e_b : b.eb, *x_f = lds ? e_f : b.ef;
			if(lane < nS) {
				x_row[sp0] = se0.row;
				x_j[sp0] = se0.j;
				x_b[sp0] = se0.bnd;
				x_f[sp0] = se0.f;
			}
			if(lane + 64 < nS) {
				x_row[sp1] = se1.row;
				x_j[sp1] = se1.j;
				x_b[sp1] = se1.bnd;
				x_f[sp1] = se1.f;
			}
#pragma unroll
			for(int m = 0; m < 4; ++m) {
				const int e = lane + 64 * m;
				if(e >= T) continue;
				const int ua = e * umax, ub = ua + dcdiv(rr[m], seg);
				double q = DBL_MAX;
				int idx = 0;
				if(prefold) {
					q = lq[e];
					idx = lj[e];
				} else if(ub <= JOIN_UPRE) {
					for(int u = ua; u < ub; ++u) {
						if(qarg_better(lq[u], lj[u], q, idx)) {
							q = lq[u];
							idx = lj[u];
						}
					}
				} else {
					fold_units(b.cq, b.cj, ua, ub, q, idx);
				}
				x_row[cs[m]] = rr[m];
				x_j[cs[m]] = idx;
				x_b[cs[m]] = bb[m];
				x_f[cs[m]] = q;
			}
			wave_sync();
			if(lane == 0) {
				s_stop = 0;
				s_merged = merged;
				s_pi = pi;
				s_pj = pj;
				s_nS = nS;
				s_m0 = m0;
			}
		}
	}
	const int T = ctl->T;
	if(T > 256) {
		__syncthreads();
		if(!s_stop) {
			const bool lds = T <= REPLAY_CAP;
			int *x_row = lds ? e_row : b.erow, *x_j = lds ? e_j : b.ej;
			double *x_b = lds ? e_b : b.eb, *x_f = lds ? e_f : b.ef;
			for(int e0 = 256 + tid; prefold && e0 < T; e0 += 8 * TB) {
				int r[8], idx[8], sl[8];
				double bnd[8], q[8];
#pragma unroll
				for(int m = 0; m < 8; ++m) {
					const int e = e0 + m * TB < T ? e0 + m * TB : e0;
					r[m] = b.crow[e];
					bnd[m] = b.cbnd[e];
					q[m] = e < JOIN_UPRE ? lq[e] : b.rf[e];
					idx[m] = e < JOIN_UPRE ? lj[e] : b.rj[e];
					sl[m] = s_merged ? b.cslot[e] : s_nS + e;
				}
#pragma unroll
				for(int m = 0; m < 8; ++m) {
					if(e0 + m * TB >= T) continue;
					x_row[sl[m]] = r[m];
					x_j[sl[m]] = idx[m];
					x_b[sl[m]] = bnd[m];
// ... 443 lines not shown
		__syncthreads();
		if(threadIdx.x == 0) {
			int lim = n - c0 < (int) blockDim.x ? n - c0 : (int) blockDim.x;
			for(int u = 0; u < lim; ++u) sd += sbuf[u];
			s_carry += tot;
		}
		__syncthreads();
	}
	if(threadIdx.x == 0) {
		b.wsum[0] = sd;
		b.wcnt[0] = s_cnt;
	}
}

template <int ET, bool BANDS, bool VBLK = false>
__global__ __launch_bounds__(TB) void k_dnj_requeue(typename Elem<ET>::T *__restrict__ D, double bs, TreeBufs b,
                                                    int n, int general, int exact_arg) {
	__shared__ double sq[5][TB / 64], sfq[TB / 64];
	__shared__ int si[5][TB / 64], sfp[TB / 64], sbp[TB / 64];
	__shared__ double sfv[TB / 64], sbq[TB / 64];
	__shared__ double s_sd;
	__shared__ int s_nj, s_i, s_j, s_stop, s_serial, s_chain;
	TreeCtl *ctl = b.ctl;
	const int nn = n - 1;
	const int tid = threadIdx.x, lane = tid & 63, wid = tid >> 6;
	const int k = blockIdx.x * TB + tid;
	TS_ENTRY(4);
	TS(4, 0);
	int Nk = 0, pkk0 = 0;
	double sDk = 0, qk0 = 0;
	typename Elem<ET>::T vm = 0;
	if(k < n) {
		Nk = b.N[k];
		sDk = b.sD[k];
		qk0 = b.Q[k];
		pkk0 = b.P[k];
	}
	if(k < nn) vm = D[tri(nn) + k];
	typename Elem<ET>::T vp = 0;
	double sdp0 = 0.0;
	const bool PV = VBLK || b.ubq;
	if(PV && k >= 1 && k < n) {
		const int p0 = pkk0 >= 0 && pkk0 < k ? pkk0 : 0;
		vp = D[tri(k) + p0];
		sdp0 = b.sD[p0];
	}
	const int Nm0 = b.N[nn];
	const double sDm0 = b.sD[nn];
	int jq = ctl->j;
	jq = jq < 0 || jq >= n ? 0 : jq;
	typename Elem<ET>::T vj = 0;
	if(k < n && k != jq) vj = k < jq ? D[tri(jq) + k] : D[tri(k) + jq];
	if(wid == 0) {
		const int done = ctl->done;
		const bool exact = exact_arg != 0;
		if(lane == 0) {
			s_i = ctl->i;
			s_j = ctl->j;
			s_stop = done;
		}
		{
			double sd;
			int nj;
			bool need, chain;
			row_sum_j_wave(b, n, exact, general, &sd, &nj, &need, &chain);
			if(lane == 0) {
				s_sd = sd;
				s_nj = nj;
				s_serial = need;
				s_chain = chain;
			}
		}
	}
	__syncthreads();
	if(s_stop) return;
	const int i = s_i, j = s_j, Nj = s_nj;
	if(s_chain) {
		const double r = serial_sum_t<TB>(b.contrib, n);
		if(tid == 0) s_sd = r;
		if(blockIdx.x == 0 && tid == 0) ctl->chain_sums++;
		__syncthreads();
	}
	const double sdj = s_sd;
	TS(4, 1);
	if(blockIdx.x == 0 && tid == 0) {
		b.sD[j] = sdj;
		b.N[j] = Nj;
		if(s_serial) ctl->serial_sums++;
	}
	const bool move = i != nn;
	const int Nm = move ? Nm0 : 0;
	const double sDm = move ? sDm0 : 0;
	if(k == j) {
		Nk = Nj;
		sDk = sdj;
	}
	double rq = DBL_MAX, pq = DBL_MAX, r2q = DBL_MAX, p2q = DBL_MAX, fq = DBL_MAX;
	int rj = 0, pk = -1, r2j = 0, p2k = -1, fp = 0;
	if(k < n) {
		if(k < j) {
			double d = Elem<ET>::get(vj, bs);
			if(0 <= d) {
				rq = qcrit(Nj, Nk, d, sdj, sDk);
				rj = k;
			}
		}
		if(k > j && k != i) {
			double qk = qk0;
			int pkk = pkk0;
			bool upd = false;
			double d = Elem<ET>::get(vj, bs);
			if(0 <= d) {
				double q = qcrit(Nj, Nk, d, sdj, sDk);
				if(q <= qk) {
					qk = q;
					pkk = j;
					upd = true;
					pq = q;
					pk = k;
				}
			}
			if(move && k > i && k < nn) {
				D[tri(k) + i] = vm;
				double dm = Elem<ET>::get(vm, bs);
				if(0 <= dm) {
					double q = qcrit(Nm, Nk, dm, sDm, sDk);
					if(q <= qk) {
						qk = q;
						pkk = i;
						upd = true;
						p2q = q;
						p2k = k;
					}
				}
			}
			if(upd) {
				b.Q[k] = qk;
				b.P[k] = pkk;
			}
			fq = qk;
			fp = pkk;
		}
		if(move && k < i) {
			D[tri(i) + k] = vm;
			double dm = Elem<ET>::get(vm, bs);
			if(0 <= dm) {
				r2q = qcrit(Nm, Nk, dm, sDm, sDk);
				r2j = k;
			}
		}
	}
	if(b.lbm) {
		const unsigned x = lb_bits(Elem<ET>::get(vm, bs));
		if(move) {
			const unsigned mn = wave_min_u32(k < i ? x : 0xFFFFFFFFu);
			if(lane == 0 && k < i) b.lbm[(long long) i * b.lbs + (k >> 6)] = mn;
			if(k > i && k < nn) __hip_atomic_fetch_min(b.lbm + (long long) k * b.lbs + (i >> 6), x, __ATOMIC_RELAXED, __HIP_MEMORY_SCOPE_AGENT);
		}
		const double sf = k < nn ? (move && k == i ? sDm : sDk) : -DBL_MAX;
		const double mx = wave_max_d(sf);
		if(lane == 0 && k < nn) b.msd[k >> 6] = mx;
	}
	double vk = DBL_MAX, qpc = INFINITY;
	if(PV && k >= 1 && k < nn && k != i && k != j) {
		const bool later = k > j;
		const int pf = later ? fp : pkk0;
		const double qf = later ? fq : qk0;
		double d = -1.0, sp = 0.0;
		if(pf == j && later) {
			d = Elem<ET>::get(vj, bs);
			sp = sdj;
		} else if(pf == i && move && later) {
			d = Elem<ET>::get(vm, bs);
			sp = sDm;
		} else if(pf == pkk0 && pkk0 >= 0 && pkk0 < k && pkk0 != i && pkk0 != j) {
			d = Elem<ET>::get(vp, bs);
			sp = sdp0;
		}
		if(0 <= d) {
			const double q = qcrit(nn, nn, d, sDk, sp);
			qpc = q;
			vk = q > qf ? q : qf;
		}
		if(b.ubq) b.ubq[k] = qpc;
	}
	if(VBLK) {
		vk = readlane_d(wave_incl_min(vk), 63);
		if(lane == 0) sfv[wid] = vk;
	}
	double bq = DBL_MAX, bqc = INFINITY;
	int bk = 0, bp = 0;
	if(BANDS) {
		if(k >= 1 && k < nn && k != i && k != j) {
			bq = k > j ? fq : qk0;
			bk = k;
			bp = k > j ? fp : pkk0;
			bqc = qpc;
		}
		qarg_wave_reduce_carry(bq, bk, bqc, bp);
	}
	qarg_wave_reduce(rq, rj);
	qarg_wave_reduce_carry(pq, pk, fq, fp);
	qarg_wave_reduce(r2q, r2j);
	qarg_wave_reduce(p2q, p2k);
	if(lane == 0) {
		sq[0][wid] = rq;
		si[0][wid] = rj;
		sq[1][wid] = pq;
		si[1][wid] = pk;
		sfq[wid] = fq;
		sfp[wid] = fp;
		sq[2][wid] = r2q;
		si[2][wid] = r2j;
		sq[3][wid] = p2q;
		si[3][wid] = p2k;
		if(BANDS) {
			sq[4][wid] = bq;
			si[4][wid] = bk;
			sbp[wid] = bp;
			sbq[wid] = bqc;
		}
	}
	__syncthreads();
	if(tid < (BANDS ? 5 : 4)) {
		double q = sq[tid][0], cq = sfq[0], xq = BANDS ? sbq[0] : 0.0;
		int ix = si[tid][0], cp = sfp[0], xp = BANDS ? sbp[0] : 0;
		for(int w = 1; w < TB / 64; ++w) {
			if(qarg_better(sq[tid][w], si[tid][w], q, ix)) {
				q = sq[tid][w];
				ix = si[tid][w];
				cq = sfq[w];
				cp = sfp[w];
				if(BANDS) {
					xp = sbp[w];
					xq = sbq[w];
				}
			}
		}
		if(tid == 4) {
			b.bmq[blockIdx.x] = q;
			b.bmr[blockIdx.x] = ix;
			b.bmp[blockIdx.x] = xp;
			b.bmqp[blockIdx.x] = xq;
		} else {
			b.qpart[4 * blockIdx.x + tid] = q;
			b.ipart[4 * blockIdx.x + tid] = ix;
		}
		if(tid == 1) {
			b.cfq[blockIdx.x] = cq;
			b.cfp[blockIdx.x] = cp;
		}
	}
	if(VBLK && tid == 0) {
		double v = sfv[0];
		for(int w = 1; w < TB / 64; ++w) v = sfv[w] < v ? sfv[w] : v;
		b.bmv[blockIdx.x] = v;
		if(blockIdx.x == 0) ctl->vtag = nn;
	}
	TS(4, 2);
	TS_EXIT(4);
}


__host__ __device__ __forceinline__ long long nj_prefix(long long s, long long nb) {
	return s * nb - (long long) (NJ_SEG / NJ_RB) * s * (s - 1) / 2;
}
__host__ __device__ __forceinline__ long long nj_blocks(int n) {
	const long long nb = (n + NJ_RB - 1) / NJ_RB, nseg = (n - 1 + NJ_SEG - 1) / NJ_SEG;
	return nj_prefix(nseg, nb);
}

template <int ET, bool GEN, bool MAXQ = false>
__global__ __launch_bounds__(TB) void k_nj_argmin(const typename Elem<ET>::T *__restrict__ D, double bs, TreeBufs b,
                                                  int n) {
	__shared__ double sq[TB / 64];
	__shared__ long long sf[TB / 64];
	if(b.ctl->done) return;
	const long long nb = (n + NJ_RB - 1) / NJ_RB;
	const long long idx = blockIdx.x;
	long long s = 0;
	while(nj_prefix(s + 1, nb) <= idx) ++s;
	const int band = (int) ((NJ_SEG / NJ_RB) * s + (idx - nj_prefix(s, nb)));
	const int c0 = (int) s * NJ_SEG;
	constexpr int M = NJ_SEG / TB;
	double sc[M];
	int nc[M];
#pragma unroll
	for(int m = 0; m < M; ++m) {
		int c = c0 + m * TB + (int) threadIdx.x;
		c = c < n ? c : n - 1;
		sc[m] = b.sD[c];
		nc[m] = GEN ? b.N[c] : n;
	}
	double bq = MAXQ ? DBL_MAX : 1.0;
	long long bf = -1;
	const int r0 = band * NJ_RB, r1 = r0 + NJ_RB < n ? r0 + NJ_RB : n;
	constexpr int G = 4;
	for(int rg = r0; rg < r1; rg += G) {
		typename Elem<ET>::T v[G][M];
		double sr[G];
		int nr[G];
#pragma unroll
		for(int g = 0; g < G; ++g) {
			const int r = rg + g < r1 ? rg + g : r1 - 1;
			const long long base = tri(r);
			sr[g] = b.sD[r];
			nr[g] = GEN ? b.N[r] : n;
#pragma unroll
			for(int m = 0; m < M; ++m) {
				const int c = c0 + m * TB + (int) threadIdx.x;
				v[g][m] = D[base + (c < r ? c : 0)];
			}
		}
#pragma unroll
// ... 349 lines not shown
				if(0 <= d && q <= Qk && (Pk < i || q < Qk)) {
					Qk = q;
					Pk = i;
				}
			}
		}
		if(k != j) {
			b.Q[k] = Qk;
			b.P[k] = Pk;
		}
	}
	if((int) blockIdx.x * TB < j) {
		qk_block_reduce<TB>(rq, rk, sq, sk);
		if(tid == 0) {
			b.bmq[blockIdx.x] = rq;
			b.bmr[blockIdx.x] = rk;
		}
	}
	if(move && (int) blockIdx.x * TB < i) {
		qk_block_reduce<TB>(pq, pk2, sq2, sk2);
		if(tid == 0) {
			b.cfq[blockIdx.x] = pq;
			b.cfp[blockIdx.x] = pk2;
		}
	}
}

static size_t tree_layout(TreeBufs *bp, int n, char *m) {
	const size_t nb = (size_t) cdiv(n, TB) + 1;
	const size_t maxu = cdiv(n, SEG_S) + 1;
	const size_t ncand = (size_t) n + 257;
	DnjGrid g;
	g.load();
	int umax = dnj_umax(n, g.seg(n));
	for(int mm = 2; mm <= 9; ++mm) {
		const int k = 16384 * mm - 1;
		if(k <= n && dnj_umax(k, g.seg(k)) > umax) umax = dnj_umax(k, g.seg(k));
	}
	if(g.seg_lb_knob > 0 && g.lb && n > g.lb_min_n && dnj_umax(n, g.seg_lb_knob) > umax) umax = dnj_umax(n, g.seg_lb_knob);
	size_t cunits = ncand * (size_t) umax;
	if(cunits < JOIN_UPRE) cunits = JOIN_UPRE;
	const size_t nq = (size_t) nj_blocks(n) + 1;
	size_t sz = 0;
	auto take = [&](size_t bytes) {
		size_t off = sz;
		sz += (bytes + 255) & ~(size_t) 255;
		return off;
	};
	size_t o_sD = take((n + 1) * 8), o_Q = take((n + 1) * 8), o_c = take((n + 1) * 8);
	size_t o_N = take((n + 1) * 4), o_P = take((n + 1) * 4);
	size_t o_S = take(DNJ_B * 4), o_uo = take((DNJ_B + 1) * 4), o_Sb = take(DNJ_B * 8);
	size_t o_uq = take(DNJ_B * maxu * 8), o_uj = take(DNJ_B * maxu * 4);
	size_t o_Se = take(DNJ_B * sizeof(Entry));
	const size_t nent = (size_t) DNJ_B + ncand;
	size_t o_ef = take(nent * 8), o_eb = take(nent * 8), o_er = take(nent * 4), o_ej = take(nent * 4);
	size_t o_ea = take(nent);
	size_t o_cr = take(ncand * 4), o_cb = take(ncand * 8), o_co = take(ncand * 4);
	size_t o_cq = take(cunits * 8), o_cj = take(cunits * 4);
	size_t o_ws = take(nb * 8), o_wa = take(nb * 8), o_wc = take(nb * 4), o_we = take(nb * 4);
	size_t o_qp = take((nb > nq ? nb : nq) * 4 * 8), o_ip = take((nb > nq ? nb : nq) * 4 * 4);
	size_t o_fp = take(nq * 8), o_cfq = take(nb * 8), o_cfp = take(nb * 4);
	size_t o_j = take((size_t) n * sizeof(ccg_join)), o_ctl = take(sizeof(TreeCtl));
	const size_t nrf = ncand > JOIN_UPRE ? ncand : JOIN_UPRE;
	size_t o_bp = take(nb * 4), o_bqp = take(nb * 8);
	size_t o_bq = take(nb * 8), o_br = take(nb * 4), o_sp = take((DNJ_B + 1) * 4), o_cs = take(ncand * 4);
	size_t o_rf = take(nrf * 8), o_rj = take(nrf * 4);
	size_t o_xa = take(nb * 8), o_xb = take(nb * sizeof(XsBlk)), o_xc = take(nb * XB_CAP * sizeof(XsCross));
	size_t o_xt = take(nb * XB_CAP_T * sizeof(XsTie));
	size_t o_pp = take(PLAN_MAXB * 8), o_jp = take(8);
	const size_t nch = ncand / 64 + 2;
	size_t o_hg = take(nch * 8), o_hr = take(nch * 4), o_hj = take(nch * 4), o_hb = take(nch * 4);
	size_t o_ec = take(nent * 4), o_cc = take(nch * 4);
	size_t o_pr = take(DNJ_B * 4), o_pe = take(DNJ_B * 4), o_pu = take((DNJ_B + 1) * 4), o_pq = take(DNJ_B * 8);
	size_t o_pb = take(DNJ_B * 8), o_eS = take(nent), o_bv = take(nb * 8), o_vs = take(nb * 8);
	size_t o_sr = take(SRDY_REP * 128), o_uh = take((size_t) PLAN_MAXB * UHIST * 4);
	size_t o_bc = take(UHIST * 4), o_bl = take(ncand * 4), o_ep = take(nent);
	size_t o_sh = take(128), o_sf = take(DNJ_B * 8), o_sj = take(DNJ_B * 4), o_es = take(DNJ_B * 4);
	if(!m) return sz;
	TreeBufs &b = *bp;
	b.sD = (double *) (m + o_sD);
	b.Q = (double *) (m + o_Q);
	b.contrib = (double *) (m + o_c);
	b.N = (int *) (m + o_N);
	b.P = (int *) (m + o_P);
	b.S = (int *) (m + o_S);
	b.uoff = (int *) (m + o_uo);
	b.Sb = (double *) (m + o_Sb);
	b.uq = (double *) (m + o_uq);
	b.uj = (int *) (m + o_uj);
	b.Sent = (Entry *) (m + o_Se);
	b.ef = (double *) (m + o_ef);
	b.eb = (double *) (m + o_eb);
	b.erow = (int *) (m + o_er);
	b.ej = (int *) (m + o_ej);
	b.eacc = (unsigned char *) (m + o_ea);
	b.crow = (int *) (m + o_cr);
	b.cbnd = (double *) (m + o_cb);
	b.cq = (double *) (m + o_cq);
	b.coff = (int *) (m + o_co);
	b.cj = (int *) (m + o_cj);
	b.wsum = (double *) (m + o_ws);
	b.wabs = (double *) (m + o_wa);
	b.wcnt = (int *) (m + o_wc);
	b.wexp = (int *) (m + o_we);
	b.qpart = (double *) (m + o_qp);
	b.ipart = (int *) (m + o_ip);
	b.fpart = (long long *) (m + o_fp);
	b.cfq = (double *) (m + o_cfq);
	b.cfp = (int *) (m + o_cfp);
	b.joins = (ccg_join *) (m + o_j);
	b.bmq = (double *) (m + o_bq);
	b.bmr = (int *) (m + o_br);
	b.bmp = (int *) (m + o_bp);
	b.bmqp = (double *) (m + o_bqp);
	b.Spos = (int *) (m + o_sp);
	b.cslot = (int *) (m + o_cs);
	b.rf = (double *) (m + o_rf);
	b.rj = (int *) (m + o_rj);
	b.ctl = (TreeCtl *) (m + o_ctl);
	b.xagg = (unsigned long long *) (m + o_xa);
	b.xblk = (XsBlk *) (m + o_xb);
	b.xcr = (XsCross *) (m + o_xc);
	b.xti = (XsTie *) (m + o_xt);
	b.ppub = (unsigned long long *) (m + o_pp);
	b.jpub = (unsigned long long *) (m + o_jp);
	b.chg = (double *) (m + o_hg);
	b.chr = (int *) (m + o_hr);
	b.chj = (int *) (m + o_hj);
	b.chb = (int *) (m + o_hb);
	b.ecnt = (unsigned *) (m + o_ec);
	b.ccnt = (unsigned *) (m + o_cc);
	b.pS_row = (int *) (m + o_pr);
	b.pS_ent = (int *) (m + o_pe);
	b.pS_uo = (int *) (m + o_pu);
	b.pS_q = (double *) (m + o_pq);
	b.pS_bnd = (double *) (m + o_pb);
	b.eS = (unsigned char *) (m + o_eS);
	b.bmv = (double *) (m + o_bv);
	b.vsuf = (double *) (m + o_vs);
	b.srdy = (unsigned *) (m + o_sr);
	b.uhist = (int *) (m + o_uh);
	b.bcnt = (int *) (m + o_bc);
	b.blist = (int *) (m + o_bl);
	b.ePr = (unsigned char *) (m + o_ep);
	b.shdr = (unsigned long long *) (m + o_sh);
	b.sfq = (double *) (m + o_sf);
	b.sfj = (int *) (m + o_sj);
	b.ecS = (unsigned *) (m + o_es);
	b.maxu = (int) maxu;
	b.lbm = NULL;
	b.msd = NULL;
	b.ubq = NULL;
	b.lbs = 0;
	b.lbw = 0;
	b.lbskip = NULL;
	b.xs_allpre = getenv("CCG_XS_ALLPRE") && atoi(getenv("CCG_XS_ALLPRE")) != 0;
	return sz;
}

size_t ccg_tree_bytes(int n) { return tree_layout(NULL, n, NULL); }

int ccg_tree_alloc(DevMem &mem, TreeWork *w, int n, hipStream_t st) {
	const size_t sz = tree_layout(NULL, n, NULL);
	CCG_TRY(mem.alloc(sz));
	CCG_CHECK(hipMemsetAsync(mem.p, 0, sz, st));
	w->mem = mem.p;
	tree_layout(&w->b, n, mem.p);
	return CCG_OK;
}

static int tree_alloc_ctx(ccg_ctx *c, TreeWork *w, int n) {
	const size_t sz = tree_layout(NULL, n, NULL);
	void *m;
	const int rc = ccg_ctx_workspace(c, CCG_WS_TREE, sz, &m);
	if(rc) return rc;
	CCG_CHECK(hipMemsetAsync(m, 0, sz, c->stream));
	w->mem = m;
	tree_layout(&w->b, n, (char *) m);
	return CCG_OK;
}

template <int ET, bool GEN>
static void enqueue_plan(hipStream_t st, typename Elem<ET>::T *D, double bs, const TreeBufs &b, int n, int first,
                         const ScanForm &f) {
	const int seg = f.seg;
	const unsigned gp = g_grid.plan_blocks(n);
	if(g_grid.bands(n)) k_dnj_plan<ET, GEN, DenseRows, true><<<gp + f.helpers, TBF, 0, st>>>(D, bs, b, n, first, DenseRows(), seg, g_grid.top(n), g_grid.bands(n), g_grid.plan_flags(f.prune != 0, f.helpers));
	else k_dnj_plan<ET, GEN, DenseRows, false><<<gp, TBF, 0, st>>>(D, bs, b, n, first, DenseRows(), seg, g_grid.top(n), 0, g_grid.plan_flags());
}

template <int ET, bool STREAM>
static void launch_scan_v(const ScanForm &f, hipStream_t st, typename Elem<ET>::T *D, double bs, const TreeBufs &b, int n, int seg) {
	const DenseRows dr;
	if(f.cmp && f.prune == 2) k_dnj_scan_v<ET, DenseRows, NoTail, STREAM, 2, true><<<f.grid, TB, 0, st>>>(D, bs, b, n, dr, seg);
	else if(f.cmp) k_dnj_scan_v<ET, DenseRows, NoTail, STREAM, 0, true><<<f.grid, TB, 0, st>>>(D, bs, b, n, dr, seg);
	else if(f.prune == 2) k_dnj_scan_v<ET, DenseRows, NoTail, STREAM, 2><<<f.grid, TB, 0, st>>>(D, bs, b, n, dr, seg);
	else if(f.prune == 1) k_dnj_scan_v<ET, DenseRows, FoldTail, STREAM, 1><<<f.grid, TB, 0, st>>>(D, bs, b, n, dr, seg);
	else if(f.tfold) k_dnj_scan_v<ET, DenseRows, FoldTail, STREAM><<<f.grid, TB, 0, st>>>(D, bs, b, n, dr, seg);
	else k_dnj_scan_v<ET, DenseRows, NoTail, STREAM><<<f.grid, TB, 0, st>>>(D, bs, b, n, dr, seg);
}

template <int ET, int G, int UC>
static void launch_scan_g(const ScanForm &f, hipStream_t st, typename Elem<ET>::T *D, double bs, const TreeBufs &b, int n, int seg) {
	if(f.cmp && f.prune == 2) k_dnj_scan_gc<ET, G, UC, true><<<f.grid, TB, 0, st>>>(D, bs, b, n, seg);
	else if(f.cmp) k_dnj_scan_gc<ET, G, UC, false><<<f.grid, TB, 0, st>>>(D, bs, b, n, seg);
	else if(f.prune) k_dnj_scan_g<ET, G, UC, true, true><<<f.grid, TB, 0, st>>>(D, bs, b, n, seg);
	else if(f.tfold) k_dnj_scan_g<ET, G, UC, true><<<f.grid, TB, 0, st>>>(D, bs, b, n, seg);
	else k_dnj_scan_g<ET, G, UC><<<f.grid, TB, 0, st>>>(D, bs, b, n, seg);
}

template <int ET, bool GEN>
static void enqueue_scan(const ScanForm &f, hipStream_t st, typename Elem<ET>::T *D, double bs, const TreeBufs &b, int n, int seg) {
	const DenseRows dr;
	switch(f.kernel) {
		case SCAN_BLOCK: k_dnj_scan<ET, GEN><<<f.grid, TB, 0, st>>>(D, bs, b, n, dr, seg); break;
		case SCAN_WAVE:
			if(f.tfold) k_dnj_scan_w<ET, GEN, DenseRows, FoldTail><<<f.grid, TB, 0, st>>>(D, bs, b, n, dr, seg);
			else k_dnj_scan_w<ET, GEN><<<f.grid, TB, 0, st>>>(D, bs, b, n, dr, seg);
			break;
		case SCAN_WAVE16:
			if(f.lb && f.prune == 2) k_dnj_scan_v<ET, DenseRows, NoTail, false, 2, true, true><<<f.grid, TB, 0, st>>>(D, bs, b, n, dr, seg);
			else if(f.lb) k_dnj_scan_v<ET, DenseRows, NoTail, false, 0, true, true><<<f.grid, TB, 0, st>>>(D, bs, b, n, dr, seg);
			else if(f.stream) launch_scan_v<ET, true>(f, st, D, bs, b, n, seg);
			else launch_scan_v<ET, false>(f, st, D, bs, b, n, seg);
			break;
		case SCAN_GROUP:
		case SCAN_GROUP_CMP:
			if(f.lb) k_dnj_scan_gc<ET, 4, 8, false, true><<<f.grid, TB, 0, st>>>(D, bs, b, n, seg);
			else if(f.G == 8) launch_scan_g<ET, 8, 4>(f, st, D, bs, b, n, seg);
			else launch_scan_g<ET, 4, 8>(f, st, D, bs, b, n, seg);
			break;
	}
}

template <int ET, bool GEN>
static int enqueue_iteration(hipStream_t st, typename Elem<ET>::T *D, double bs, const TreeBufs &b, int n, int first,
                             int method, int exact, KTimer &kt) {
	const unsigned gn = cdiv(n, TB);
	const int general = GEN;
	if(method == CCG_TREE_DNJ) {
		const int prefold = g_grid.prefold(n);
		const ScanForm f = dnj_scan_form(g_grid, n, ET, GEN, b.lbm != NULL);
		const int seg = f.seg;
		enqueue_plan<ET, GEN>(st, D, bs, b, n, first, f);
		kt.mark(CCG_K_FIND);
		if(f.sphase == SPHASE_COMPACT) k_dnj_sphase<ET, false><<<g_grid.sphase_blocks(), TB, 0, st>>>(D, bs, b, n, seg);
		else if(f.sphase == SPHASE_SCAN) k_dnj_sphase<ET><<<g_grid.sphase_blocks(), TB, 0, st>>>(D, bs, b, n, seg);
		enqueue_scan<ET, GEN>(f, st, D, bs, b, n, seg);
		if(f.fold) k_dnj_fold<><<<FOLD_BLOCKS, TB, 0, st>>>(b, n, seg, f.sfold);
		kt.mark(CCG_K_REST);
		if(prefold && g_grid.join_pf) k_dnj_join_pf<ET, GEN><<<gn, TB, 0, st>>>(D, bs, b, n, general, g_grid.join_pf == 2);
		else k_dnj_join<ET, GEN><<<gn, TB, 0, st>>>(D, bs, b, n, general, prefold, seg);
		if(GEN) k_update_general<ET><<<1, 1024, 0, st>>>(D, bs, b, n);
		kt.mark(CCG_K_UPDATE);
		if(g_grid.bands(n - 1) && g_grid.scan_vblk && dnj_scan_form(g_grid, n - 1, ET, GEN, b.lbm != NULL).prune)
			k_dnj_requeue<ET, true, true><<<gn, TB, 0, st>>>(D, bs, b, n, general, exact);
		else if(g_grid.bands(n - 1)) k_dnj_requeue<ET, true><<<gn, TB, 0, st>>>(D, bs, b, n, general, exact);
		else k_dnj_requeue<ET, false><<<gn, TB, 0, st>>>(D, bs, b, n, general, exact);
		kt.mark(CCG_K_REQUEUE);
		return (GEN ? 4 : 3) + f.launches;
	}
	if(method == CCG_TREE_HNJ) {
		k_hnj_argmin<><<<gn, TB, 0, st>>>(b, n);
		kt.mark(CCG_K_ARGMIN);
		k_nj_join<ET><<<gn, TB, 0, st>>>(D, bs, b, n, (int) gn, general, DBL_MAX);
		if(GEN) k_update_general<ET><<<1, 1024, 0, st>>>(D, bs, b, n);
		kt.mark(CCG_K_UPDATE);
		k_hnj_update<ET><<<gn, TB, 0, st>>>(D, bs, b, n, general, exact);
		kt.mark(CCG_K_POP);
		return GEN ? 4 : 3;
	}
	const unsigned g = (unsigned) nj_blocks(n);
	if(method == CCG_TREE_MN) k_nj_argmin<ET, GEN, true><<<g, TB, 0, st>>>(D, bs, b, n);
	else k_nj_argmin<ET, GEN><<<g, TB, 0, st>>>(D, bs, b, n);
	kt.mark(CCG_K_ARGMIN);
	k_nj_join<ET><<<gn, TB, 0, st>>>(D, bs, b, n, (int) g, general, method == CCG_TREE_MN ? DBL_MAX : 1.0);
	if(GEN) k_update_general<ET><<<1, 1024, 0, st>>>(D, bs, b, n);
	kt.mark(CCG_K_UPDATE);
	k_nj_pop<ET><<<gn, TB, 0, st>>>(D, b, n, general, exact);
	kt.mark(CCG_K_POP);
	return GEN ? 4 : 3;
}

#ifdef CCG_TRACE
static int trace_report(int method, int trace_hi, const TreeCtl &h) {
	static unsigned long long tr[256 * NKT * 16];
	CCG_CHECK(hipMemcpyFromSymbol(tr, HIP_SYMBOL(g_trace), sizeof(tr), 0, hipMemcpyDeviceToHost));
	const int nk = method == CCG_TREE_DNJ ? NKT : 0;
	double acc[NKT][16] = {{0}}, gap[NKT] = {0}, itv = 0;
	int cnt = 0;
	bool present[NKT] = {false};
	for(int s = 0; s < 256; ++s)
		for(int k = 0; k < nk; ++k) present[k] = present[k] || tr[(s * NKT + k) * 16 + 15];
	for(int s = 0; s < 256; ++s) {
		const unsigned long long *e = tr + s * NKT * 16;
		bool ok = true;
		for(int k = 0; k < nk; ++k) ok = ok && (!present[k] || (e[k * 16 + 15] && e[k * 16 + 14]));
		if(!ok) continue;
		++cnt;
		int k0 = 0, prev = -1;
		while(k0 < nk && !present[k0]) ++k0;
		for(int k = k0; k < nk; ++k) {
			if(!present[k]) continue;
			unsigned long long t0 = ~e[k * 16 + 15];
			for(int p = 0; p < 15; ++p)
				if(e[k * 16 + p]) acc[k][p] += ((double) e[k * 16 + p] - (double) t0) / 100.0;
			if(prev >= 0) gap[k] += ((double) t0 - (double) e[prev * 16 + 14]) / 100.0;
			prev = k;
		}
		if(s + 1 < 256 && tr[((s + 1) * NKT + k0) * 16 + 15]) {
			gap[k0] += ((double) ~tr[((s + 1) * NKT + k0) * 16 + 15] - (double) e[(nk - 1) * 16 + 14]) / 100.0;
			itv += ((double) ~tr[((s + 1) * NKT + k0) * 16 + 15] - (double) ~e[k0 * 16 + 15]) / 100.0;
		}
	}
	const char *kn[NKT] = {"select", "plan/find", "scan", "join", "requeue"};
	fprintf(stderr, "trace: %d joins at n <= %d; iteration %.2f us; serial replays %d, serial sums %d\n", cnt,
	        trace_hi, cnt ? itv / (cnt - 1) : 0, h.serial_replays, h.serial_sums);
	{
		static unsigned long long sp[256 * 64 * 3];
		CCG_CHECK(hipMemcpyFromSymbol(sp, HIP_SYMBOL(g_samp), sizeof(sp), 0, hipMemcpyDeviceToHost));
		double st_max = 0, en_max = 0, dur = 0, st_med = 0, stg = 0;
		int sc = 0, jc = 0;
		for(int s = 0; s < 256; ++s) {
			const unsigned long long t0 = ~tr[(s * NKT + 2) * 16 + 15];
			if(!tr[(s * NKT + 2) * 16 + 15]) continue;
			double smax = 0, emax = 0;
			int any = 0;
			for(int q = 0; q < 64; ++q) {
				const unsigned long long *e = sp + (s * 64 + q) * 3;
				if(!e[0] || !e[2] || e[0] < t0) continue;
				const double a = (e[0] - t0) / 100.0, z = (e[2] - t0) / 100.0;
				smax = a > smax ? a : smax;
				emax = z > emax ? z : emax;
				dur += z - a;
				if(e[1] >= e[0]) stg += (e[1] - e[0]) / 100.0;
				st_med += a;
				++sc;
				any = 1;
			}
			if(any) {
				st_max += smax;
				en_max += emax;
				++jc;
			}
		}
		{
			static unsigned long long ua[256 * 64 * 8];
			CCG_CHECK(hipMemcpyFromSymbol(ua, HIP_SYMBOL(g_uamp), sizeof(ua), 0, hipMemcpyDeviceToHost));
			double ud[4] = {0}, ug[4] = {0}, us0 = 0;
			int uc[4] = {0}, gc[4] = {0}, s0c = 0;
			for(int s = 0; s < 256; ++s) {
				const unsigned long long t0 = ~tr[(s * NKT + 2) * 16 + 15];
				if(!tr[(s * NKT + 2) * 16 + 15]) continue;
				for(int q = 0; q < 64; ++q) {
					const unsigned long long *e = ua + (s * 64 + q) * 8;
					const unsigned long long *sp0 = sp + (s * 64 + q) * 3;
					if(e[0] && e[0] >= t0 && sp0[0] && e[0] >= sp0[0]) {
						us0 += (e[0] - sp0[0]) / 100.0;
						++s0c;
					}
					for(int k = 0; k < 4; ++k) {
						if(e[2 * k] && e[2 * k + 1] >= e[2 * k] && e[2 * k] >= t0) {
							ud[k] += (e[2 * k + 1] - e[2 * k]) / 100.0;
							++uc[k];
						}
						if(k && e[2 * k] && e[2 * k - 1] && e[2 * k] >= e[2 * k - 1] && e[2 * k] >= t0) {
							ug[k] += (e[2 * k] - e[2 * k - 1]) / 100.0;
							++gc[k];
						}
					}
				}
			}
			fprintf(stderr, "  scan units (wave 0 of sampled blocks): entry->first unit %.2f us;", s0c ? us0 / s0c : 0.0);
			for(int k = 0; k < 4; ++k)
				fprintf(stderr, " unit%d n=%d dur %.2f gap %.2f;", k, uc[k], uc[k] ? ud[k] / uc[k] : 0.0, gc[k] ? ug[k] / gc[k] : 0.0);
			fprintf(stderr, "\n");
			memset(ua, 0, sizeof(ua));
			CCG_CHECK(hipMemcpyToSymbol(HIP_SYMBOL(g_uamp), ua, sizeof(ua), 0, hipMemcpyHostToDevice));
		}
		if(jc) fprintf(stderr, "  scan samples: %d joins, %.1f working blocks sampled/join; last start %.2f us, last end %.2f us, mean start %.2f, mean duration %.2f us (setup %.2f)\n",
		                jc, (double) sc / jc, st_max / jc, en_max / jc, st_med / sc, dur / sc, stg / sc);
	}
	for(int k = 0; k < nk && cnt; ++k) {
		if(!present[k]) continue;
		fprintf(stderr, "  %-14s gap-before %6.2f  span %6.2f  block0:", kn[k], gap[k] / cnt, acc[k][14] / cnt);
		for(int p = 0; p < 14; ++p) fprintf(stderr, " %6.2f", acc[k][p] / cnt);
		fprintf(stderr, "\n");
	}
	return CCG_OK;
}
#endif

template __global__ void k_exact_sum<>(TreeBufs b, int n, int G);

static bool g_progress = false;

template <int ET>
static int tree_run_t(ccg_ctx *ctx, const ccg_tree_args *a, void *Dd, ccg_join *joins, int *njoins,
                      int *final_n, double *final_d, int64_t *stats, const ccg_dnj_state *sin,
                      ccg_dnj_state *sout) {
	typedef typename Elem<ET>::T T;
	T *D = (T *) Dd;
	const int n0 = a->n;
	const double bs = a->byteScale;
	hipStream_t st = ctx->stream;
	TreeWork w;
	g_grid = DnjGrid();
	g_grid.load();
	g_progress = getenv("CCG_PROGRESS") != nullptr;
	const bool cmp_env = getenv("CCG_SCAN_CMPB") != nullptr;
	auto cmp_share = [&](int blocks) {
		return ctx->cus > 0 && ctx->cus < ctx->ncu ? (blocks * ctx->cus / ctx->ncu > 64 ? blocks * ctx->cus / ctx->ncu : 64)
		                                           : blocks;
	};
	if(!cmp_env) g_grid.cmp_blocks = cmp_share(g_grid.cmp_blocks);
	int rc = tree_alloc_ctx(ctx, &w, n0);
	if(rc) return rc;
	TreeBufs b = w.b;
	TreeCtl init = tree_ctl_seed(a);
	if(sin) {
		init.cand = sin->cand;
		init.cand_q = sin->Q[sin->cand];
		init.cand_p = sin->P[sin->cand];
	}
	TreeRun<TreeCtl> run(ctx, b.ctl);
	KTimer &kt = run.kt;
	long long &launches = run.launches;
	CCG_TRY(run.begin(init, a->profile != 0));
	k_init_rows<ET><<<cdiv(n0, TB / 64), TB, 0, st>>>(D, n0, bs, b.sD, b.N, b.ctl);
	k_init_cols<ET><<<cdiv(n0, TB), TB, 0, st>>>(D, n0, bs, b.sD, b.N, b.ctl);
	launches += 2;
	bool resumed_counts = false;
	if(sin) {
		CCG_CHECK(hipMemcpyAsync(b.sD, sin->sD, (size_t) n0 * 8, hipMemcpyHostToDevice, st));
		CCG_CHECK(hipMemcpyAsync(b.Q, sin->Q, (size_t) n0 * 8, hipMemcpyHostToDevice, st));
		CCG_CHECK(hipMemcpyAsync(b.N, sin->N, (size_t) n0 * 4, hipMemcpyHostToDevice, st));
		CCG_CHECK(hipMemcpyAsync(b.P, sin->P, (size_t) n0 * 4, hipMemcpyHostToDevice, st));
		for(int k = 0; k < n0 && !resumed_counts; ++k) resumed_counts = sin->N[k] != n0;
	} else if(a->method == CCG_TREE_DNJ) {
		k_init_hnj<ET><<<cdiv(n0, TB / 64), TB, 0, st>>>(DenseRows(), D, n0, bs, b.sD, b.N, b.Q, b.P);
		k_dnj_prep<><<<1, TB, 0, st>>>(b, n0);
		launches += 2;
	} else if(a->method == CCG_TREE_HNJ) {
		k_init_hnj<ET><<<cdiv(n0, TB / 64), TB, 0, st>>>(DenseRows(), D, n0, bs, b.sD, b.N, b.Q, b.P);
		launches += 1;
	}
	kt.mark(CCG_K_INIT);
	CCG_CHECK(hipGetLastError());
	TreeCtl h;
	CCG_TRY(run.read_ctl(h));
	const bool general = h.has_missing != 0 || resumed_counts;
	if(a->method == CCG_TREE_DNJ && !general && g_grid.lb && n0 > g_grid.lb_min_n) {
		const LbLayout lb = lb_layout(n0, n0);
		void *lbmem = NULL;
		if(ccg_ctx_workspace(ctx, CCG_WS_TREE_LB, lb.bytes(), &lbmem) == CCG_OK) {
			CCG_TRY(lb_bind(b, lbmem, lb, 0, st));
			k_lb_init<ET><<<cdiv(n0, TB / 64), TB, 0, st>>>(D, n0, bs, b);
			launches += 1;
			CCG_CHECK(hipGetLastError());
			if(!getenv("CCG_SCAN_PRUNE")) g_grid.scan_prune = 0;
			g_grid.seg_lb = g_grid.seg_lb_knob < 0 ? 0 : g_grid.seg_lb_knob ? g_grid.seg_lb_knob : LB_SEG_DEFAULT;
			if(!cmp_env) {
				const ScanForm f = dnj_scan_form(g_grid, n0, ET, false, true);
				int per_cu = 0;
				const void *fn = f.prune == 2 ? (const void *) k_dnj_scan_v<ET, DenseRows, NoTail, false, 2, true, true>
				                              : (const void *) k_dnj_scan_v<ET, DenseRows, NoTail, false, 0, true, true>;
				if(f.kernel == SCAN_GROUP_CMP) fn = (const void *) k_dnj_scan_gc<ET, 4, 8, false, true>;
				CCG_CHECK(hipOccupancyMaxActiveBlocksPerMultiprocessor(&per_cu, fn, TB, 0));
				const int cus = ctx->cus > 0 && ctx->cus < ctx->ncu ? ctx->cus : ctx->ncu;
				g_grid.cmp_blocks = per_cu * cus > 64 ? per_cu * cus : 64;
			}
		} else {
			(void) hipGetLastError();
		}
	}
#ifdef CCG_TRACE
	const char *tn = getenv("CCG_TRACE_N");
	int trace_hi = tn ? atoi(tn) : n0 / 2;
	CCG_CHECK(hipMemcpyToSymbolAsync(HIP_SYMBOL(g_trace_hi), &trace_hi, sizeof(int), 0, hipMemcpyHostToDevice, st));
	static unsigned long long zero_tr[256 * 4 * 16];
	CCG_CHECK(hipMemcpyToSymbolAsync(HIP_SYMBOL(g_trace), zero_tr, sizeof(zero_tr), 0, hipMemcpyHostToDevice, st));
#endif
	int n = n0;
	long long win_rows = h.rows, win_cells = h.cells;
	const int stop_n = a->max_joins > 0 && a->max_joins < n0 - 2 ? n0 - a->max_joins : 2;
	while(n > stop_n) {
		launches += general ? enqueue_iteration<ET, true>(st, D, bs, b, n, n == n0, a->method, a->exact, kt)
		                    : enqueue_iteration<ET, false>(st, D, bs, b, n, n == n0, a->method, a->exact, kt);
		CCG_CHECK(hipGetLastError());
		--n;
		bool read;
		CCG_TRY(run.check(h, &read));
		if(read) {
			g_grid.small_wave = g_grid.adapt_rows && h.rows - win_rows > 1024LL * g_grid.adapt_rows;
			g_grid.prune_on = !g_grid.prune_cells || h.cells - win_cells > 1024LL * g_grid.prune_cells;
			win_rows = h.rows;
			win_cells = h.cells;
			if(g_progress && (n0 - n) % (16 * 1024) == 0)
				fprintf(stderr, "ccg_tree: %d joins, n = %d, rows %lld cells %lld (reference rule %lld / %lld)\n", n0 - n,
				        n, h.rows, h.cells, h.ref_rows, h.ref_cells);
			if(h.done) break;
		}
	}
	CCG_TRY(run.finish(h, n, b.joins, joins, njoins, final_n, final_d));
	if(*final_n == 2) CCG_TRY(run.final_distance<ET>(D, bs, final_d));
	CCG_TRY(lb_harvest(b, (size_t) LB_SCAN + LB_HELP, st, h));
	if(getenv("CCG_XS_WHY"))
		fprintf(stderr, "xs_why: value %d nc %d nt %d stuck %d ex0 %d cap %d walk %d (chain sums %d of %d)\n",
		        h.xs_why[0], h.xs_why[1], h.xs_why[2], h.xs_why[3], h.xs_why[4], h.xs_why[5], h.xs_why[6],
		        h.chain_sums, h.serial_sums);
#ifdef CCG_TRACE
	CCG_TRY(trace_report(a->method, trace_hi, h));
#endif
	if(sout) {
		const bool over = h.done || n <= 2;
		sout->n = over ? 0 : n;
		sout->cand = 0;
		if(!over) {
			if(n != n0) {
				if(general) enqueue_plan<ET, true>(st, D, bs, b, n, 0, dnj_scan_form(g_grid, n, ET, true, b.lbm != NULL));
				else enqueue_plan<ET, false>(st, D, bs, b, n, 0, dnj_scan_form(g_grid, n, ET, false, b.lbm != NULL));
				CCG_CHECK(hipGetLastError());
			}
			TreeCtl h2;
			CCG_CHECK(hipMemcpyAsync(&h2, b.ctl, sizeof(h2), hipMemcpyDeviceToHost, st));
			CCG_CHECK(hipMemcpyAsync(sout->sD, b.sD, (size_t) n * 8, hipMemcpyDeviceToHost, st));
			CCG_CHECK(hipMemcpyAsync(sout->Q, b.Q, (size_t) n * 8, hipMemcpyDeviceToHost, st));
			CCG_CHECK(hipMemcpyAsync(sout->N, b.N, (size_t) n * 4, hipMemcpyDeviceToHost, st));
			CCG_CHECK(hipMemcpyAsync(sout->P, b.P, (size_t) n * 4, hipMemcpyDeviceToHost, st));
			CCG_CHECK(hipStreamSynchronize(st));
			sout->cand = h2.cand;
		}
	}
	TreeStats s = run.stats();
	s.rows = h.rows;
	s.cells = h.cells - h.cells_pruned - h.cells_lbskip;
	s.cells_top = h.cells_top;
	s.cells_rest = h.cells_rest - h.cells_pruned - h.cells_lbskip;
	s.serial_sums = h.serial_sums;
	s.chain_sums = h.chain_sums;
	s.slot8 = h.cells_help;
	s.ref_rows = h.ref_rows;
	s.ref_cells = h.ref_cells;
	s.write(stats, a->profile != 0, kt);
	return run.end();
}

template <int NT>
__global__ __launch_bounds__(NT) void k_selftest_row_sum(TreeBufs b, int n, double *out, int *par,
                                                        unsigned long long *stamps) {
	double s;
	if(stamps && threadIdx.x == 0) stamps[15] = __builtin_amdgcn_s_memrealtime();
	const bool ok = exact_sum_w<NT, XS_RB>(b.contrib, n, &s, stamps);
	if(!ok) s = serial_sum_t<NT>(b.contrib, n);
	if(threadIdx.x == 0) {
		out[0] = s;
		par[0] = ok;
	}
}

int ccg_selftest_row_sum_impl(ccg_ctx *ctx, const double *c, int n, double *out, int *parallel) {
	hipStream_t st = ctx->stream;
	DevMem mem;
	CCG_TRY(mem.alloc((size_t) (n + 1) * 8 + 64 + 64 * 8));
	StreamSync idle(st);
	char *m = mem.p;
	TreeBufs b;
	memset(&b, 0, sizeof(b));
	b.contrib = (double *) m;
	double *dout = (double *) (m + (size_t) (n + 1) * 8);
	int *dpar = (int *) (dout + 1);
	unsigned long long *dst = (unsigned long long *) (m + (size_t) (n + 1) * 8 + 64);
	CCG_CHECK(hipMemcpyAsync(b.contrib, c, (size_t) n * 8, hipMemcpyHostToDevice, st));
	const bool small = getenv("CCG_SELFTEST_TB256") != nullptr;
	auto launch = [&](unsigned long long *stp) {
		if(small) k_selftest_row_sum<TB><<<1, TB, 0, st>>>(b, n, dout, dpar, stp);
		else k_selftest_row_sum<XS_NT><<<1, XS_NT, 0, st>>>(b, n, dout, dpar, stp);
	};
	launch(nullptr);
	CCG_CHECK(hipGetLastError());
	if(const char *e = getenv("CCG_SELFTEST_REPS")) {
		const int reps = atoi(e);
		CCG_CHECK(hipEventRecord(ctx->ev0, st));
		for(int r = 0; r < reps; ++r) launch(nullptr);
		CCG_CHECK(hipEventRecord(ctx->ev1, st));
		CCG_CHECK(hipEventSynchronize(ctx->ev1));
		float ms = 0;
		CCG_CHECK(hipEventElapsedTime(&ms, ctx->ev0, ctx->ev1));
		fprintf(stderr, "selftest_row_sum n=%d: %.2f us per launch\n", n, 1000.0 * ms / (reps > 0 ? reps : 1));
		unsigned long long hs[64] = {0};
		CCG_CHECK(hipMemsetAsync(dst, 0, 64 * 8, st));
		launch(dst);
		CCG_CHECK(hipMemcpyAsync(hs, dst, 64 * 8, hipMemcpyDeviceToHost, st));
		CCG_CHECK(hipStreamSynchronize(st));
		for(int w = 0; w < 4; ++w) {
			fprintf(stderr, "  wave %d phases (us from entry):", w);
			for(int i = 0; i < 15; ++i)
				fprintf(stderr, " %d:%.2f", i, hs[16 * w + i] ? (double) (hs[16 * w + i] - hs[15]) / 100.0 : -1.0);
			fprintf(stderr, "\n");
		}
	}
	CCG_CHECK(hipMemcpyAsync(out, dout, 8, hipMemcpyDeviceToHost, st));
	CCG_CHECK(hipMemcpyAsync(parallel, dpar, 4, hipMemcpyDeviceToHost, st));
	CCG_CHECK(hipStreamSynchronize(st));
	return CCG_OK;
}

int ccg_tree_impl(ccg_ctx *ctx, const ccg_tree_args *a, void *Dd, ccg_join *joins, int *njoins, int *final_n,
                  double *final_d, int64_t *stats, const ccg_dnj_state *sin, ccg_dnj_state *sout) {
	if(a->method == CCG_TREE_UPGMA || a->method == CCG_TREE_CF || a->method == CCG_TREE_FF) {
		if(sin || sout) return CCG_EINVAL;
		return ccg_tree_linkage_impl(ctx, a, Dd, joins, njoins, final_n, final_d, stats);
	}
	if(a->method != CCG_TREE_NJ && a->method != CCG_TREE_DNJ && a->method != CCG_TREE_HNJ && a->method != CCG_TREE_MN)
		return CCG_EINVAL;
	if(!ccg_etype_ok(a->etype)) return CCG_EINVAL;
	return with_etype(a->etype, [&](auto et) {
		return tree_run_t<decltype(et)::value>(ctx, a, Dd, joins, njoins, final_n, final_d, stats, sin, sout);
	});
}
// ... 1 lines not shown
```

ccphylo_amd/csrc/tree_shard_dnj.hip:

```cpp
#define CCG_DNJ_NO_TRACE
#include <stdio.h>
#include <string.h>
#include <stdlib.h>
#include <vector>
#include "ccg_dnj_search.h"
#include "ccg_shard.h"

static_assert(SB == 8, "one bit byte per shard band");
struct RecSlot {
	size_t f_off, j_off, bytes;
};
static __host__ __device__ inline RecSlot rec_slot(int n, int world) {
	const int nb = (n + SB - 1) / SB, omb = (nb + world - 1) / world;
	RecSlot s;
	s.f_off = ((size_t) omb + 15) & ~(size_t) 15;
	s.j_off = s.f_off + (size_t) omb * SB * 8;
	s.bytes = (s.j_off + (size_t) omb * SB * 4 + 15) & ~(size_t) 15;
	return s;
}
static __host__ __device__ inline int rec_owner(int r, int world) { return (r / SB) % world; }
static __host__ __device__ inline int rec_pos(int r, int world) { return (r / SB) / world * SB + r % SB; }

static __host__ __device__ inline size_t rec_bits_bytes(int n) { return (size_t) ((n + 63) / 64) * 8; }
static __host__ __device__ inline size_t rec_bytes(int n) { return rec_bits_bytes(n) + (size_t) n * 12; }
// ... 179 lines not shown
		__syncthreads();
		if(tid == 0) {
			int fe = 0x7fffffff;
			long long na = 0, ca = 0;
			for(int w = 0; w < PICK_T / 64; ++w) {
				fe = s_wf[w] < fe ? s_wf[w] : fe;
				na += s_na[w];
				ca += s_ca[w];
			}
			const int pi = fe < 0x7fffffff ? x_row[fe] : pos_i, pj = fe < 0x7fffffff ? x_j[fe] : pos_j;
			s_i = pi;
			s_j = pj;
			if(writer) {
				if(na) {
					atomicAdd((unsigned long long *) &ctl->ref_rows, (unsigned long long) na);
					atomicAdd((unsigned long long *) &ctl->ref_cells, (unsigned long long) ca);
				}
				if(pi == 0 && pj == 0) {
					ctl->done = 1;
					ctl->final_n = n;
				} else {
					ctl->i = pi;
					ctl->j = pj;
				}
				ctl->rtotal = total;
			}
		}
	} else if(tid < 64) {
		int pi = pos_i, pj = pos_j;
		bool had_bad;
		if(lds) replay_wave(total, m0, e_row, e_j, e_b, e_f, e_acc, writer, b, pi, pj, &had_bad, n, acc_out);
		else replay_wave(total, m0, b.erow, b.ej, b.eb, b.ef, pacc + (size_t) blockIdx.x * pstride, writer, b, pi, pj,
		                 &had_bad, n, acc_out);
		if(tid == 0) {
			s_i = pi;
			s_j = pj;
			if(writer) {
				if(pi == 0 && pj == 0) {
					ctl->done = 1;
					ctl->final_n = n;
				} else {
					ctl->i = pi;
					ctl->j = pj;
				}
				ctl->rtotal = total;
				ctl->serial_replays += had_bad;
			}
		}
	}
	__syncthreads();
	PTS(4);
	const int i = s_i, j = s_j;
	if(i == 0 && j == 0) return;
	if(writer && lds) {
		for(int e = tid; e < total; e += PICK_T) {
			b.erow[e] = e_row[e];
			b.ef[e] = e_f[e];
			b.ej[e] = e_j[e];
		}
	}
	const bool own_m = sh.owns(n - 1);
	const typename Elem<ET>::T *rowm = D + (own_m ? sh.off(n - 1) : 0);
	for(int k = blockIdx.x * PICK_T + tid; k < n; k += gridDim.x * PICK_T) {
		typename Elem<ET>::T xi = 0, xj = 0;
		if(k > i) {
			if(sh.owns(k)) xi = D[sh.off(k) + i];
		} else if(k < i && sh.owns(i)) {
			xi = D[sh.off(i) + k];
		}
		if(k > j) {
			if(sh.owns(k)) xj = D[sh.off(k) + j];
		} else if(k < j && sh.owns(j)) {
			xj = D[sh.off(j) + k];
		}
		X[k] = xi;
		X[n + k] = xj;
		X[2 * n + k] = own_m && k < n - 1 ? rowm[k] : (typename Elem<ET>::T) 0;
	}
	PTS(5);
	if(dbg && blockIdx.x == 0 && threadIdx.x == 0) dbg[(n & 1023) * 8 + 6] = total;
#undef PTS
}

template <int ET>
__global__ __launch_bounds__(TB) void k_shd_join(typename Elem<ET>::T *__restrict__ D, double bs, TreeBufs b, int n,
                                                 Shard sh, const typename Elem<ET>::T *__restrict__ X,
                                                 typename Elem<ET>::T *__restrict__ Xm,
                                                 typename Elem<ET>::T *__restrict__ Xj,
                                                 const unsigned char *__restrict__ acc) {
	__shared__ int s_stop, s_nj, s_neg, s_exact, s_i, s_j;
	TreeCtl *ctl = b.ctl;
	const int tid = threadIdx.x;
	const int k = blockIdx.x * TB + tid;
	double sDk = 0, Dik = 0, Dkj = 0;
	int Nk = 0;
	if(k < n) {
		sDk = b.sD[k];
		Nk = b.N[k];
		Dik = Elem<ET>::get(X[k], bs);
		Dkj = Elem<ET>::get(X[n + k], bs);
	}
	if(tid == 0) {
		s_stop = ctl->done;
		s_nj = ctl->njoins;
		s_neg = ctl->neg;
		s_exact = ctl->exact;
		s_i = ctl->i;
		s_j = ctl->j;
	}
	__syncthreads();
	if(s_stop) return;
	for(int e = k, tot = ctl->rtotal; e < tot; e += gridDim.x * TB) {
		if(acc[e]) {
			b.Q[b.erow[e]] = b.ef[e];
			b.P[b.erow[e]] = b.ej[e];
		}
	}
	const int i = s_i, j = s_j;
	const double Dij = Elem<ET>::get(X[j], bs);
	if(blockIdx.x == 0 && tid == 0) {
		double Li, Lj;
		limb_length(&Li, &Lj, b.sD[i], b.sD[j], b.N[i], b.N[j], Dij, s_neg);
		ctl->Li = Li;
		ctl->Lj = Lj;
		ctl->Dij = Dij;
		ccg_join J;
		J.i = i;
		J.j = j;
		J.Li = Li;
		J.Lj = Lj;
		b.joins[s_nj] = J;
		ctl->njoins = s_nj + 1;
	}
	double d = 0;
	int cnt = 0;
	typename Elem<ET>::T v = 0;
	if(k < n && k != i && k != j) {
		d = (Dik + Dkj - Dij) / 2;
		d = d < 0 ? 0 : d;
		v = Elem<ET>::put(d, 0.25, bs);
		if(k > j) {
			if(sh.owns(k)) D[sh.off(k) + j] = v;
		} else if(sh.owns(j)) {
			D[sh.off(j) + k] = v;
		}
		Xj[k] = v;
		if(k == n - 1) Xm[j] = v;
		b.sD[k] = sDk - (Dik + Dkj - d);
		b.N[k] = Nk - 1;
		cnt = 1;
	}
	if(b.lbm) {
		const unsigned x = lb_bits(Elem<ET>::get(v, bs));
		if(sh.owns(j)) {
			const unsigned mn = wave_min_u32(k < j ? x : 0xFFFFFFFFu);
			if((tid & 63) == 0 && k < j) lb_line(b, j)[k >> 6] = mn;
		}
		if(k > j && k < n && k != i && sh.owns(k))
			__hip_atomic_fetch_min(lb_line(b, k) + (j >> 6), x, __ATOMIC_RELAXED, __HIP_MEMORY_SCOPE_AGENT);
	}
	update_partials(b, n, s_exact, k, d, cnt, blockIdx.x);
	if(s_exact) xs_join_row(b, n, blockIdx.x, d, xs_tag(n));
}

template <int ET, bool BANDS>
__global__ __launch_bounds__(TB) void k_shd_requeue(typename Elem<ET>::T *__restrict__ D, double bs, TreeBufs b,
                                                    int n, Shard sh, const typename Elem<ET>::T *__restrict__ Xm,
                                                    const typename Elem<ET>::T *__restrict__ Xj, void *R) {
	__shared__ double sq[5][TB / 64], sfq[TB / 64];
	__shared__ int si[5][TB / 64], sfp[TB / 64], sbp[TB / 64];
	__shared__ double s_sd;
	__shared__ int s_nj, s_i, s_j, s_stop, s_serial, s_chain;
	TreeCtl *ctl = b.ctl;
	const int nn = n - 1;
	const int tid = threadIdx.x, lane = tid & 63, wid = tid >> 6;
	const int k = blockIdx.x * TB + tid;
	int Nk = 0, pkk0 = 0;
	double sDk = 0, qk0 = 0;
	typename Elem<ET>::T vm = 0, vj = 0;
	if(k < n) {
		Nk = b.N[k];
		sDk = b.sD[k];
		qk0 = b.Q[k];
		pkk0 = b.P[k];
		vj = Xj[k];
	}
	if(k < nn) vm = Xm[k];
	typename Elem<ET>::T vp = 0;
	double sdp0 = 0.0;
	const bool PV = b.ubq != nullptr;
	if(PV && k >= 1 && k < n && sh.owns(k)) {
		const int p0 = pkk0 >= 0 && pkk0 < k ? pkk0 : 0;
		vp = D[sh.off(k) + p0];
		sdp0 = b.sD[p0];
	}
	const int Nm0 = b.N[nn];
	const double sDm0 = b.sD[nn];
	if(wid == 0) {
		const int done = ctl->done;
		const bool exact = ctl->exact;
		if(lane == 0) {
			s_i = ctl->i;
			s_j = ctl->j;
			s_stop = done;
		}
		if(!done) {
			double sd;
			int nj;
			bool need, chain;
			row_sum_j_wave(b, n, exact, false, &sd, &nj, &need, &chain);
			if(lane == 0) {
				s_sd = sd;
				s_nj = nj;
				s_serial = need;
				s_chain = chain;
			}
		}
	}
	__syncthreads();
	if(s_stop) return;
	const int i = s_i, j = s_j, Nj = s_nj;
	if(s_chain) {
		const double r = serial_sum_t<TB>(b.contrib, n);
		if(tid == 0) s_sd = r;
		if(blockIdx.x == 0 && tid == 0) ctl->chain_sums++;
		__syncthreads();
	}
	const double sdj = s_sd;
	if(blockIdx.x == 0 && tid == 0) {
		b.sD[j] = sdj;
		b.N[j] = Nj;
		if(s_serial) ctl->serial_sums++;
	}
	const bool move = i != nn;
	const int Nm = move ? Nm0 : 0;
	const double sDm = move ? sDm0 : 0;
	if(k == j) {
		Nk = Nj;
		sDk = sdj;
	}
	double rq = DBL_MAX, pq = DBL_MAX, r2q = DBL_MAX, p2q = DBL_MAX, fq = DBL_MAX;
	int rj = 0, pk = -1, r2j = 0, p2k = -1, fp = 0;
	if(k < n) {
		if(k < j) {
			const double d = Elem<ET>::get(vj, bs);
			if(0 <= d) {
				rq = qcrit(Nj, Nk, d, sdj, sDk);
				rj = k;
			}
		}
		if(k > j && k != i) {
			double qk = qk0;
			int pkk = pkk0;
			bool upd = false;
			const double d = Elem<ET>::get(vj, bs);
			if(0 <= d) {
				const double q = qcrit(Nj, Nk, d, sdj, sDk);
				if(q <= qk) {
					qk = q;
					pkk = j;
					upd = true;
					pq = q;
					pk = k;
				}
			}
			if(move && k > i && k < nn) {
				if(sh.owns(k)) D[sh.off(k) + i] = vm;
				const double dm = Elem<ET>::get(vm, bs);
				if(0 <= dm) {
					const double q = qcrit(Nm, Nk, dm, sDm, sDk);
					if(q <= qk) {
						qk = q;
						pkk = i;
						upd = true;
						p2q = q;
						p2k = k;
					}
				}
			}
			if(upd) {
				b.Q[k] = qk;
				b.P[k] = pkk;
			}
			fq = qk;
			fp = pkk;
		}
		if(move && k < i) {
			if(sh.owns(i)) D[sh.off(i) + k] = vm;
			const double dm = Elem<ET>::get(vm, bs);
			if(0 <= dm) {
				r2q = qcrit(Nm, Nk, dm, sDm, sDk);
				r2j = k;
			}
		}
	}
	if((size_t) k * 4 < rec_slot(n, sh.world).f_off) ((unsigned *) R)[k] = 0;
	if(b.lbm) {
		const unsigned x = lb_bits(Elem<ET>::get(vm, bs));
		if(move) {
			if(sh.owns(i)) {
				const unsigned mn = wave_min_u32(k < i ? x : 0xFFFFFFFFu);
				if(lane == 0 && k < i) lb_line(b, i)[k >> 6] = mn;
			}
			if(k > i && k < nn && sh.owns(k))
				__hip_atomic_fetch_min(lb_line(b, k) + (i >> 6), x, __ATOMIC_RELAXED, __HIP_MEMORY_SCOPE_AGENT);
		}
		const double sf = k < nn ? (move && k == i ? sDm : sDk) : -DBL_MAX;
		const double mx = wave_max_d(sf);
		if(lane == 0 && k < nn) b.msd[k >> 6] = mx;
	}
	double qpc = INFINITY;
	if(PV && k >= 1 && k < nn && k != i && k != j && sh.owns(k)) {
		const bool later = k > j;
		const int pf = later ? fp : pkk0;
		double d = -1.0, sp = 0.0;
		if(pf == j && later) {
			d = Elem<ET>::get(vj, bs);
			sp = sdj;
		} else if(pf == i && move && later) {
			d = Elem<ET>::get(vm, bs);
			sp = sDm;
		} else if(pf == pkk0 && pkk0 >= 0 && pkk0 < k && pkk0 != i && pkk0 != j) {
			d = Elem<ET>::get(vp, bs);
			sp = sdp0;
		}
		if(0 <= d) qpc = qcrit(nn, nn, d, sDk, sp);
		b.ubq[k] = qpc;
	}
	double bq = DBL_MAX, bqc = INFINITY;
	int bk = 0, bp = 0;
	__shared__ double sbq[TB / 64];
	if(BANDS) {
		if(k >= 1 && k < nn && k != i && k != j) {
			bq = k > j ? fq : qk0;
			bk = k;
			bp = k > j ? fp : pkk0;
			bqc = qpc;
		}
		qarg_wave_reduce_carry(bq, bk, bqc, bp);
	}
	qarg_wave_reduce(rq, rj);
	qarg_wave_reduce_carry(pq, pk, fq, fp);
	qarg_wave_reduce(r2q, r2j);
	qarg_wave_reduce(p2q, p2k);
	if(lane == 0) {
		sq[0][wid] = rq;
		si[0][wid] = rj;
		sq[1][wid] = pq;
		si[1][wid] = pk;
		sfq[wid] = fq;
		sfp[wid] = fp;
		sq[2][wid] = r2q;
		si[2][wid] = r2j;
		sq[3][wid] = p2q;
		si[3][wid] = p2k;
		if(BANDS) {
			sq[4][wid] = bq;
			si[4][wid] = bk;
			sbp[wid] = bp;
			sbq[wid] = bqc;
		}
	}
	__syncthreads();
	if(tid < (BANDS ? 5 : 4)) {
		double q = sq[tid][0], cq = sfq[0], xq = BANDS ? sbq[0] : 0.0;
		int ix = si[tid][0], cp = sfp[0], xp = BANDS ? sbp[0] : 0;
		for(int w = 1; w < TB / 64; ++w) {
			if(qarg_better(sq[tid][w], si[tid][w], q, ix)) {
				q = sq[tid][w];
				ix = si[tid][w];
				cq = sfq[w];
				cp = sfp[w];
				if(BANDS) {
					xp = sbp[w];
					xq = sbq[w];
				}
			}
		}
		if(tid == 4) {
			b.bmq[blockIdx.x] = q;
			b.bmr[blockIdx.x] = ix;
			b.bmp[blockIdx.x] = xp;
			if(PV) b.bmqp[blockIdx.x] = xq;
		} else {
			b.qpart[4 * blockIdx.x + tid] = q;
			b.ipart[4 * blockIdx.x + tid] = ix;
		}
		if(tid == 1) {
			b.cfq[blockIdx.x] = cq;
			b.cfp[blockIdx.x] = cp;
		}
	}
}

template <int ET>
__global__ __launch_bounds__(TB) void k_shd_lb_init(const typename Elem<ET>::T *__restrict__ D, int n, double bs,
                                                    TreeBufs b, Shard sh) {
	constexpr int BB = 8;
	const int lane = threadIdx.x & 63;
	const int w = blockIdx.x * (TB / 64) + (threadIdx.x >> 6);
	if(w >= n) return;
	if(w < (n + LBW - 1) / LBW) {
		const int c = w * LBW + lane;
		const double mx = wave_max_d(c < n ? b.sD[c] : -DBL_MAX);
		if(lane == 0) b.msd[w] = mx;
	}
	if(lane == 0) b.ubq[w] = INFINITY;
	const int r = ((w >> 3) * sh.world + sh.rank) * 8 + (w & 7);
	if(r >= n) return;
	const typename Elem<ET>::T *row = D + sh.off(r);
	unsigned *line = lb_line(b, r);
	const int nbk = (r + LBW - 1) / LBW;
	for(int u0 = 0; u0 < nbk; u0 += BB) {
		unsigned x[BB];
#pragma unroll
		for(int m = 0; m < BB; ++m) {
			const int c = (u0 + m) * LBW + lane;
			x[m] = u0 + m < nbk && c < r ? lb_bits(Elem<ET>::get(row[c], bs)) : 0xFFFFFFFFu;
		}
#pragma unroll
		for(int m = 0; m < BB; ++m) {
			const unsigned mn = wave_min_u32(x[m]);
			if(lane == 0 && u0 + m < nbk) line[u0 + m] = mn;
		}
	}
}

template <int ET>
static int shd_init_hnj(const typename Elem<ET>::T *D, int n0, double bs, const Shard &sh, CollRun &cr,
                        hipStream_t st, TreeBufs &b, void *R) {
	const RecView v = rec_view(R, n0);
	CCG_CHECK(hipMemsetAsync(R, 0, rec_bytes(n0), st));
	k_init_hnj<ET><<<cdiv(n0, TB / 64), TB, 0, st>>>(sh, D, n0, bs, b.sD, b.N, v.f, v.j);
	CCG_CHECK(hipGetLastError());
	cr.kt->mark(CCG_K_INIT);
	int rc = cr.allreduce(v.f, (size_t) n0 * 12);
	if(rc) return rc;
	CCG_CHECK(hipMemcpyAsync(b.Q, v.f, (size_t) n0 * 8, hipMemcpyDeviceToDevice, st));
	CCG_CHECK(hipMemcpyAsync(b.P, v.j, (size_t) n0 * 4, hipMemcpyDeviceToDevice, st));
	CCG_CHECK(hipMemsetAsync(R, 0, rec_bytes(n0), st));
	k_dnj_prep<><<<1, TB, 0, st>>>(b, n0);
	CCG_CHECK(hipGetLastError());
	cr.kt->mark(CCG_K_INIT);
	return CCG_OK;
}

struct ShdLayout {
	size_t o_R, o_X, o_Xm, o_Sl, o_G, o_Xj, o_pf, o_pa, o_pc, o_rp, o_is, sz = 0;
	ShdLayout(int n0, int world, int es) {
		auto take = [&](size_t bytes) {
			size_t off = sz;
			sz += (bytes + 255) & ~(size_t) 255;
			return off;
		};
		const RecSlot rs0 = rec_slot(n0, world);
		o_R = take(rec_bytes(n0));
		o_X = take((size_t) 3 * n0 * es);
		o_Xm = take((size_t) n0 * es + 8);
		o_Sl = take(rs0.bytes);
		o_G = take((size_t) world * rs0.bytes);
		o_Xj = take((size_t) n0 * es + 8);
		o_pf = take((size_t) n0);
		o_pa = take((size_t) PICK_MAXB * n0);
		o_pc = take((size_t) n0 * 4);
		o_rp = take(sh_rp_bytes(n0));
		o_is = take(sh_init_scratch_bytes(n0, world));
	}
};

size_t ccg_shard_dnj_bytes(int n, int world, int es) { return ccg_tree_bytes(n) + ShdLayout(n, world, es).sz; }

static void pick_ts_report(const unsigned long long *dbg, hipStream_t st) {
	static thread_local unsigned long long hd[1024 * 8];
	if(hipMemcpyAsync(hd, dbg, sizeof(hd), hipMemcpyDeviceToHost, st) != hipSuccess ||
	   hipStreamSynchronize(st) != hipSuccess)
		memset(hd, 0, sizeof(hd));
	double acc[8] = {0};
	int cnt = 0;
	for(int s_ = 0; s_ < 1024; ++s_) {
		const unsigned long long *t_ = hd + s_ * 8;
		if(!t_[0] || !t_[5]) continue;
		for(int p_ = 1; p_ < 6; ++p_) acc[p_] += (double) (t_[p_] - t_[p_ - 1]) * 10.0;
		acc[6] += (double) t_[6];
		++cnt;
	}
	if(cnt)
		fprintf(stderr, "pick phases over %d joins (ns): entry->loads %.0f, count+scan %.0f, entries %.0f, replay %.0f, gather %.0f; total entries %.1f\n",
		        cnt, acc[1] / cnt, acc[2] / cnt, acc[3] / cnt, acc[4] / cnt, acc[5] / cnt, acc[6] / cnt);
}

template <int ET>
static int tree_shard_dnj_run_t(ccg_ctx *ctx, const ccg_tree_args *a, const ccg_coll *coll, void *Dd,
                                ccg_join *joins, int *njoins, int *final_n, double *final_d, int64_t *stats) {
	typedef typename Elem<ET>::T T;
	T *D = (T *) Dd;
	const int n0 = a->n;
	const double bs = a->byteScale;
	hipStream_t st = ctx->stream;
	const Shard sh = {coll->rank, coll->world};
	TreeWork w;
	DevMem wmem, mem, lbmem, dbgmem;
	CCG_TRY(ccg_tree_alloc(wmem, &w, n0, st));
	TreeBufs b = w.b;
	const ShdLayout L(n0, coll->world, ET);
	const RecSlot rs0 = rec_slot(n0, coll->world);
	CCG_TRY(mem.alloc(L.sz));
	char *m = mem.p;
	size_t hcap = sh_init_host_bytes(n0, coll->world);
	if((size_t) 3 * n0 * ET > hcap) hcap = (size_t) 3 * n0 * ET;
	if(rec_bytes(n0) > hcap) hcap = rec_bytes(n0);
	if((size_t) coll->world * rs0.bytes > hcap) hcap = (size_t) coll->world * rs0.bytes;
	PinnedMem hm;
	if(coll->host_staged && !hm.alloc(hcap)) return CCG_ENOMEM;
	DnjGrid grid;
	grid.load();
	void *R = m + L.o_R, *Sl = m + L.o_Sl, *G = m + L.o_G;
	T *X = (T *) (m + L.o_X), *Xm = (T *) (m + L.o_Xm), *Xj = (T *) (m + L.o_Xj);
	ShInitStat istat = {0, 0};
	unsigned char *pflag = (unsigned char *) (m + L.o_pf), *pacc = (unsigned char *) (m + L.o_pa);
	unsigned *pcnt = (unsigned *) (m + L.o_pc);
	unsigned long long *dbg = NULL;
	if(getenv("CCG_PICK_TS") && dbgmem.alloc(1024 * 8 * 8) == CCG_OK && hipMemsetAsync(dbgmem.p, 0, 1024 * 8 * 8, st) == hipSuccess)
		dbg = (unsigned long long *) dbgmem.p;
	const TreeCtl init = tree_ctl_seed(a);
	TreeRun<TreeCtl> run(ctx, b.ctl);
	KTimer &kt = run.kt;
	CollRun cr = {coll, st, hm.p, &kt};
	CCG_CHECK(hipMemsetAsync(m, 0, L.sz, st));
	CCG_TRY(run.begin(init, a->profile != 0));
	int missing = 0;
	CCG_TRY(sh_init_summad<ET>(D, n0, bs, sh, cr, st, m + L.o_rp, m + L.o_is, b, &run.launches, &missing, &istat));
	if(missing) return CCG_EUNSUP;
	CCG_TRY(shd_init_hnj<ET>(D, n0, bs, sh, cr, st, b, R));
	run.launches += 2;
	if(grid.lb && n0 > grid.lb_min_n) {
		const LbLayout lb = lb_layout(n0, (long long) cdiv(cdiv(n0, 8), sh.world) * 8);
		if(lbmem.alloc(lb.bytes()) == CCG_OK) {
			CCG_TRY(lb_bind(b, lbmem.p, lb, sh.world, st));
			k_shd_lb_init<ET><<<cdiv(n0, TB / 64), TB, 0, st>>>(D, n0, bs, b, sh);
			CCG_CHECK(hipGetLastError());
			run.launches += 1;
		}
	}
	TreeCtl hc;
	int n = n0;
	const int stop_n = a->max_joins > 0 && a->max_joins < n0 - 2 ? n0 - a->max_joins : 2;
	while(n > stop_n) {
		const unsigned gn = cdiv(n, TB), gp = cdiv(n, PICK_T) < PICK_MAXB ? cdiv(n, PICK_T) : PICK_MAXB;
		T *Xmr = X + 2 * (size_t) n;
		const int seg = grid.seg(n);
		const unsigned gpl = grid.plan_blocks(n);
		if(grid.bands(n)) k_dnj_plan<ET, false, Shard, true><<<gpl, TBF, 0, st>>>(D, bs, b, n, n == n0, sh, seg, grid.top(n), grid.bands(n), grid.plan_flags());
		else k_dnj_plan<ET, false, Shard, false><<<gpl, TBF, 0, st>>>(D, bs, b, n, n == n0, sh, seg, grid.top(n), 0, grid.plan_flags());
		kt.mark(CCG_K_FIND);
		{
			const ScanForm f = dnj_scan_form_shard(grid, n, ET, b.lbm != NULL);
			const RecTail<ET> rt{D, sh, Sl, pcnt};
			switch(f.kernel) {
				case SCAN_WAVE16:
					if(f.lb && f.stream) k_dnj_scan_v<ET, Shard, RecTail<ET>, true, 0, false, true><<<f.grid, TB, 0, st>>>(D, bs, b, n, sh, seg, rt);
					else if(f.lb) k_dnj_scan_v<ET, Shard, RecTail<ET>, false, 0, false, true><<<f.grid, TB, 0, st>>>(D, bs, b, n, sh, seg, rt);
					else if(f.stream) k_dnj_scan_v<ET, Shard, RecTail<ET>, true><<<f.grid, TB, 0, st>>>(D, bs, b, n, sh, seg, rt);
					else k_dnj_scan_v<ET, Shard, RecTail<ET>><<<f.grid, TB, 0, st>>>(D, bs, b, n, sh, seg, rt);
					break;
				case SCAN_WAVE: k_dnj_scan_w<ET, false, Shard, RecTail<ET>><<<f.grid, TB, 0, st>>>(D, bs, b, n, sh, seg, rt); break;
				default: k_dnj_scan<ET, false><<<f.grid, TB, 0, st>>>(D, bs, b, n, sh, seg, rt);
			}
		}
		kt.mark(CCG_K_REST);
		CCG_TRY(cr.allgather(Sl, G, rec_slot(n, sh.world).bytes));
		k_shd_pick<ET><<<gp, PICK_T, 0, st>>>(D, b, n, sh, G, X, pacc, pflag, n0, dbg);
		kt.mark(CCG_K_UPDATE);
		CCG_TRY(cr.allreduce(X, (size_t) 3 * n * ET));
		k_shd_join<ET><<<gn, TB, 0, st>>>(D, bs, b, n, sh, X, Xmr, Xj, pflag);
		kt.mark(CCG_K_UPDATE);
		if(grid.bands(n - 1)) k_shd_requeue<ET, true><<<gn, TB, 0, st>>>(D, bs, b, n, sh, Xmr, Xj, Sl);
		else k_shd_requeue<ET, false><<<gn, TB, 0, st>>>(D, bs, b, n, sh, Xmr, Xj, Sl);
		kt.mark(CCG_K_REQUEUE);
		CCG_CHECK(hipGetLastError());
		run.launches += 5;
		--n;
		bool read;
		CCG_TRY(run.check(hc, &read));
		if(read && hc.done) break;
	}
	CCG_TRY(run.finish(hc, n, b.joins, joins, njoins, final_n, final_d));
	if(dbg) pick_ts_report(dbg, st);
	if(*final_n == 2) {
		CCG_TRY(cr.bcast(sh.rank == 0 ? (const void *) (D + sh.off(1)) : NULL, Xm, ET, 0));
		CCG_TRY(run.final_distance<ET>(Xm, bs, final_d));
	}
	CCG_TRY(lb_harvest(b, LB_SCAN, st, hc));
	TreeStats s = run.stats();
	s.rows = hc.rows;
	s.cells = hc.cells - hc.cells_lbskip;
	s.cells_top = hc.cells_top;
	s.cells_rest = hc.cells_rest - hc.cells_lbskip;
	s.serial_sums = hc.serial_sums;
	s.chain_sums = hc.chain_sums;
	s.slot8 = istat.coll_bytes;
	s.hard_columns = istat.hard;
	s.ref_rows = hc.ref_rows;
	s.ref_cells = hc.ref_cells;
	s.write(stats, a->profile != 0, kt);
	return run.end();
}

int ccg_tree_shard_dnj_impl(ccg_ctx *c, const ccg_tree_args *a, const ccg_coll *coll, void *Dloc, ccg_join *joins,
                            int *njoins, int *final_n, double *final_d, int64_t *stats) {
	return with_etype(a->etype, [&](auto et) {
		return tree_shard_dnj_run_t<decltype(et)::value>(c, a, coll, Dloc, joins, njoins, final_n, final_d, stats);
	});
}
```

Baseline: 212.2 million.

## Make lower-bound block width configurable (16/32/64) for DNJ pruned scan

Generalizes the per-row lower-bound cache used to skip blocks of the Q-criterion scan from fixed 64-column blocks to 16, 32 or 64 columns, selected through an environment variable. Narrower blocks give tighter bounds so more cells can be skipped, and several blocks are packed into one wave load. The cost is larger bound tables, more bound maintenance in join and update kernels, and piecewise loops. The default stays at width 64, and a waves-per-eu attribute is added for narrow widths. It also adds an allocation-fit fallback.

New measurement: 190.6 million. 0.898x the previous value.

```diff
diff --git a/ccphylo_amd/csrc/ccg_dnj_form.h b/ccphylo_amd/csrc/ccg_dnj_form.h
--- a/ccphylo_amd/csrc/ccg_dnj_form.h
+++ b/ccphylo_amd/csrc/ccg_dnj_form.h
@@ -12,6 +12,7 @@
 #define DNJ_BANDS 64
 #define DNJ_BANDS_MAX 128
 #define SEG 2048
+#define LB_SH_DEFAULT 6
 #define LB_SEG_DEFAULT (2 * SEG)
 #define TBF 1024
 #define FIND_RPT 16
@@ -35,6 +36,7 @@
 	int scan_fold = 0;
 	int scan_prune = 2;
 	int lb = 1, lb_min_n = 16384;
+	int lb_sh = LB_SH_DEFAULT;
 	int lb_groups = 0;
 	int seg_lb = 0, seg_lb_knob = 0;
 	int scan_vblk = 1;
@@ -66,6 +68,11 @@
 		if(const char *e = getenv("CCG_SCAN_LB")) lb = atoi(e);
 		if(const char *e = getenv("CCG_LB_MIN_N")) lb_min_n = atoi(e);
 		if(const char *e = getenv("CCG_LB_GROUPS")) lb_groups = atoi(e);
+		if(const char *e = getenv("CCG_LB_WIDTH")) {
+			const int v = atoi(e);
+			if(v == 64 || v == 32 || v == 16) lb_sh = v == 64 ? 6 : v == 32 ? 5 : 4;
+			else fprintf(stderr, "ccphylo_amd: CCG_LB_WIDTH=%s ignored (64, 32 or 16)\n", e);
+		}
 		if(const char *e = getenv("CCG_SEG_LB")) {
 			char *end;
 			const long v = strtol(e, &end, 10);
diff --git a/ccphylo_amd/csrc/ccg_dnj_search.h b/ccphylo_amd/csrc/ccg_dnj_search.h
--- a/ccphylo_amd/csrc/ccg_dnj_search.h
+++ b/ccphylo_amd/csrc/ccg_dnj_search.h
@@ -1,5 +1,6 @@
 #pragma once
 #include <stdlib.h>
+#include <type_traits>
 #include "ccg_tree_common.h"
 #include "ccg_dnj_form.h"
 
@@ -1306,158 +1307,207 @@
 	}
 }
 
-static_assert(8 * SEG <= 4 * 64 * LBW && SEG_S <= 4 * 64 * LBW, "lb_unit loads at most 256 block bounds per unit");
+#define LB_PIECE 256
+static_assert(LB_PIECE == 4 * 64 && LB_PIECE <= 256, "four bound registers per lane; a block of the piece indexed by a byte");
+static_assert(8 * SEG <= LB_PIECE << LB_SH_MAX && SEG_S <= LB_PIECE << LB_SH_MAX, "one piece per unit at the widest block");
+static_assert(64 >> LB_SH_MIN <= 4, "a load's blocks packed into one word");
+template <int ET, int WS>
+__device__ __forceinline__ int lb_unit_w(const typename Elem<ET>::T *__restrict__ row, double bs, const TreeBufs &b, int n,
+                                         int r, int c0, int c1, double sDr, double &q, int &idx, int isub,
+                                         double sDm, bool ubinf) {
+	typedef typename Elem<ET>::T T;
+	constexpr int BB = ET == 8 ? LB_BB_D : LB_BB_N;
+	const int lane = threadIdx.x & 63;
+	constexpr int ws = WS, W = 1 << ws, K = 64 >> ws;
+	const int grp = lane >> ws, lcol = lane & (W - 1);
+	const double ub = ubinf ? INFINITY : b.ubq[r];
+	const unsigned *line = lb_line(b, r);
+	int loaded = 0;
+	int p0 = c0;
+	do {
+		const int p1 = p0 + (LB_PIECE << ws) < c1 ? p0 + (LB_PIECE << ws) : c1;
+		const int bl0 = p0 >> ws, nbk = (p1 - p0 + W - 1) >> ws;
+		unsigned lbb[4];
+		double msb[4];
+#pragma unroll
+		for(int h = 0; h < 4; ++h) {
+			const int t = lane + 64 * h;
+			lbb[h] = t < nbk ? line[bl0 + t] : 0u;
+			msb[h] = t < nbk ? b.msd[bl0 + t] : 0.0;
+		}
+		unsigned long long need[4];
+#pragma unroll
+		for(int h = 0; h < 4; ++h) {
+			const int t = lane + 64 * h;
+			const double lb = qcrit(n, n, (double) __uint_as_float(lbb[h]), sDr, msb[h]);
+			need[h] = __ballot(t < nbk && !(lb > ub));
+		}
+		int h = 0;
+		while(true) {
+			unsigned pk[BB];
+			int nb = 0;
+#pragma unroll
+			for(int m = 0; m < BB; ++m) {
+				pk[m] = 0;
+				for(int g = 0; g < K; ++g) {
+					while(h < 4 && !need[h]) ++h;
+					if(h == 4) break;
+					const int bit = __ffsll((long long) need[h]) - 1;
+					need[h] &= need[h] - 1;
+					const int t = 64 * h + bit;
+					pk[m] |= (unsigned) t << (8 * g);
+					++nb;
+					loaded += (bl0 + t + 1) << ws < c1 ? W : c1 - ((bl0 + t) << ws);
+				}
+			}
+			if(!nb) break;
+			T v[BB];
+			double sk[BB];
+#pragma unroll
+			for(int m = 0; m < BB; ++m) {
+				int c = ((bl0 + (int) ((pk[m] >> (8 * grp)) & 255u)) << ws) + lcol;
+				c = m * K + grp < nb && c < c1 ? c : c1 - 1;
+				v[m] = row[c];
+				sk[m] = b.sD[c];
+			}
+#pragma unroll
+			for(int m = 0; m < BB; ++m) {
+				const int c = ((bl0 + (int) ((pk[m] >> (8 * grp)) & 255u)) << ws) + lcol;
+				const double d = Elem<ET>::get(v[m], bs);
+				const double x = qcrit(n, n, d, sDr, c == isub ? sDm : sk[m]);
+				if(m * K + grp < nb && c < c1 && 0 <= d && qarg_better(x, c, q, idx)) {
+					q = x;
+					idx = c;
+				}
+			}
+		}
+		p0 += LB_PIECE << ws;
+	} while(WS < LB_SH_MAX && p0 < c1);
+	return (c1 - c0) - loaded;
+}
 template <int ET>
 __device__ __forceinline__ int lb_unit(const typename Elem<ET>::T *__restrict__ row, double bs, const TreeBufs &b, int n,
                                        int r, int c0, int c1, double sDr, double &q, int &idx, int isub,
                                        double sDm, bool ubinf) {
+	switch(b.lbsh) {
+		case 4: return lb_unit_w<ET, 4>(row, bs, b, n, r, c0, c1, sDr, q, idx, isub, sDm, ubinf);
+		case 5: return lb_unit_w<ET, 5>(row, bs, b, n, r, c0, c1, sDr, q, idx, isub, sDm, ubinf);
+		default: return lb_unit_w<ET, 6>(row, bs, b, n, r, c0, c1, sDr, q, idx, isub, sDm, ubinf);
+	}
+}
+
+template <int ET, int G, int WS>
+__device__ __forceinline__ long long lb_unit_gw(const typename Elem<ET>::T *const (&row)[G], double bs, const TreeBufs &b,
+                                                int n, const int (&r)[G], const bool (&act)[G], int c0,
+                                                const int (&c1)[G], int cmax, const double (&sDr)[G], double (&q)[G],
+                                                int (&idx)[G]) {
 	typedef typename Elem<ET>::T T;
+	static_assert(G * (64 >> LB_SH_MIN) <= 32, "a load's (row, group) needs in one word");
 	constexpr int BB = ET == 8 ? LB_BB_D : LB_BB_N;
 	const int lane = threadIdx.x & 63;
-	const int bl0 = c0 / LBW, nbk = (c1 - c0 + LBW - 1) / LBW;
-	const double ub = ubinf ? INFINITY : b.ubq[r];
-	unsigned lbb[4];
-	double msb[4];
-	const unsigned *line = lb_line(b, r);
-#pragma unroll
-	for(int h = 0; h < 4; ++h) {
-		const int t = lane + 64 * h;
-		lbb[h] = t < nbk ? line[bl0 + t] : 0u;
-		msb[h] = t < nbk ? b.msd[bl0 + t] : 0.0;
-	}
-	unsigned long long need[4];
-#pragma unroll
-	for(int h = 0; h < 4; ++h) {
-		const int t = lane + 64 * h;
-		const double lb = qcrit(n, n, (double) __uint_as_float(lbb[h]), sDr, msb[h]);
-		need[h] = __ballot(t < nbk && !(lb > ub));
-	}
-	int loaded = 0;
-	int h = 0;
-	while(true) {
-		int blk[BB], nb = 0;
-		while(nb < BB && h < 4) {
-			if(!need[h]) {
-				++h;
-				continue;
-			}
-			const int bit = __ffsll((long long) need[h]) - 1;
-			need[h] &= need[h] - 1;
-			blk[nb++] = bl0 + 64 * h + bit;
-		}
-		if(!nb) break;
-		T v[BB];
-		double sk[BB];
-#pragma unroll
-		for(int m = 0; m < BB; ++m) {
-			int c = (m < nb ? blk[m] : blk[0]) * LBW + lane;
-			c = c < c1 ? c : c1 - 1;
-			v[m] = row[c];
-			sk[m] = b.sD[c];
-		}
-#pragma unroll
-		for(int m = 0; m < BB; ++m) {
-			const int c = (m < nb ? blk[m] : blk[0]) * LBW + lane;
-			const double d = Elem<ET>::get(v[m], bs);
-			const double x = qcrit(n, n, d, sDr, c == isub ? sDm : sk[m]);
-			if(m < nb && c < c1 && 0 <= d && qarg_better(x, c, q, idx)) {
-				q = x;
-				idx = c;
-			}
-		}
-		for(int m = 0; m < nb; ++m) loaded += (blk[m] + 1) * LBW < c1 ? LBW : c1 - blk[m] * LBW;
-	}
-	return (c1 - c0) - loaded;
-}
-
-template <int ET, int G>
-__device__ __forceinline__ long long lb_unit_g(const typename Elem<ET>::T *const (&row)[G], double bs, const TreeBufs &b,
-                                               int n, const int (&r)[G], const bool (&act)[G], int c0,
-                                               const int (&c1)[G], int cmax, const double (&sDr)[G], double (&q)[G],
-                                               int (&idx)[G]) {
-	typedef typename Elem<ET>::T T;
-	constexpr int BB = ET == 8 ? LB_BB_D : LB_BB_N;
-	const int lane = threadIdx.x & 63;
-	const int bl0 = c0 / LBW, nbkm = (cmax - c0 + LBW - 1) / LBW;
-	double msb[4];
-#pragma unroll
-	for(int h = 0; h < 4; ++h) {
-		const int t = lane + 64 * h;
-		msb[h] = t < nbkm ? b.msd[bl0 + t] : 0.0;
-	}
-	unsigned long long need[G][4], any[4] = {0, 0, 0, 0};
-#pragma unroll
-	for(int k = 0; k < G; ++k) {
-		const int nbk = act[k] ? (c1[k] - c0 + LBW - 1) / LBW : 0;
-		const double ub = act[k] ? b.ubq[r[k]] : 0.0;
-		const unsigned *line = lb_line(b, act[k] ? r[k] : 1);
+	constexpr int ws = WS, W = 1 << ws, K = 64 >> ws;
+	const int grp = lane >> ws, lcol = lane & (W - 1);
+	long long loaded = 0;
+	int p0 = c0;
+	do {
+		const int p1 = p0 + (LB_PIECE << ws) < cmax ? p0 + (LB_PIECE << ws) : cmax;
+		const int bl0 = p0 >> ws, nbkm = (p1 - p0 + W - 1) >> ws;
+		double msb[4];
 #pragma unroll
 		for(int h = 0; h < 4; ++h) {
 			const int t = lane + 64 * h;
-			const unsigned lbv = t < nbk ? line[bl0 + t] : 0u;
-			const double lb = qcrit(n, n, (double) __uint_as_float(lbv), sDr[k], msb[h]);
-			need[k][h] = __ballot(t < nbk && !(lb > ub));
-			any[h] |= need[k][h];
-		}
-	}
-	long long loaded = 0;
-	int h = 0;
-	while(true) {
-		int blk[BB], nb = 0;
-		while(nb < BB && h < 4) {
-			if(!any[h]) {
-				++h;
-				continue;
-			}
-			const int bit = __ffsll((long long) any[h]) - 1;
-			any[h] &= any[h] - 1;
-			blk[nb++] = 64 * h + bit;
-		}
-		if(!nb) break;
-		double sk[BB];
-		T v[G][BB];
-#pragma unroll
-		for(int m = 0; m < BB; ++m) {
-			const int t = m < nb ? blk[m] : blk[0];
-			int c = (bl0 + t) * LBW + lane;
-			sk[m] = b.sD[c < cmax ? c : cmax - 1];
-#pragma unroll
-			for(int k = 0; k < G; ++k) {
-				v[k][m] = 0;
-				if((need[k][t >> 6] >> (t & 63)) & 1)
-					v[k][m] = row[k][c < c1[k] ? c : c1[k] - 1];
-			}
-		}
-#pragma unroll
-		for(int m = 0; m < BB; ++m) {
-			const int t = m < nb ? blk[m] : blk[0];
-			const int c = (bl0 + t) * LBW + lane;
-#pragma unroll
-			for(int k = 0; k < G; ++k) {
-				if(m >= nb || !((need[k][t >> 6] >> (t & 63)) & 1)) continue;
-				const double d = Elem<ET>::get(v[k][m], bs);
-				const double x = qcrit(n, n, d, sDr[k], sk[m]);
-				if(c < c1[k] && 0 <= d && qarg_better(x, c, q[k], idx[k])) {
-					q[k] = x;
-					idx[k] = c;
-				}
-			}
-		}
-		for(int m = 0; m < nb; ++m) {
-			const int c = (bl0 + blk[m]) * LBW;
-#pragma unroll
-			for(int k = 0; k < G; ++k)
-				if((need[k][blk[m] >> 6] >> (blk[m] & 63)) & 1) loaded += c + LBW < c1[k] ? LBW : c1[k] - c;
-		}
-	}
+			msb[h] = t < nbkm ? b.msd[bl0 + t] : 0.0;
+		}
+		unsigned long long need[G][4], any[4] = {0, 0, 0, 0};
+#pragma unroll
+		for(int k = 0; k < G; ++k) {
+			const int e1 = c1[k] < p1 ? c1[k] : p1;
+			const int nbk = act[k] && e1 > p0 ? (e1 - p0 + W - 1) >> ws : 0;
+			const double ub = act[k] ? b.ubq[r[k]] : 0.0;
+			const unsigned *line = lb_line(b, act[k] ? r[k] : 1);
+#pragma unroll
+			for(int h = 0; h < 4; ++h) {
+				const int t = lane + 64 * h;
+				const unsigned lbv = t < nbk ? line[bl0 + t] : 0u;
+				const double lb = qcrit(n, n, (double) __uint_as_float(lbv), sDr[k], msb[h]);
+				need[k][h] = __ballot(t < nbk && !(lb > ub));
+				any[h] |= need[k][h];
+			}
+		}
+		int h = 0;
+		while(true) {
+			unsigned pk[BB], rm[BB];
+			int nb = 0;
+#pragma unroll
+			for(int m = 0; m < BB; ++m) {
+				pk[m] = 0;
+				rm[m] = 0;
+				for(int g = 0; g < K; ++g) {
+					while(h < 4 && !any[h]) ++h;
+					if(h == 4) break;
+					const int bit = __ffsll((long long) any[h]) - 1;
+					any[h] &= any[h] - 1;
+					const int t = 64 * h + bit;
+					pk[m] |= (unsigned) t << (8 * g);
+					++nb;
+					const int c = (bl0 + t) << ws;
+#pragma unroll
+					for(int k = 0; k < G; ++k)
+						if((need[k][h] >> bit) & 1) {
+							rm[m] |= 1u << (k * 4 + g);
+							loaded += c + W < c1[k] ? W : c1[k] - c;
+						}
+				}
+			}
+			if(!nb) break;
+			double sk[BB];
+			T v[G][BB];
+#pragma unroll
+			for(int m = 0; m < BB; ++m) {
+				const int c = ((bl0 + (int) ((pk[m] >> (8 * grp)) & 255u)) << ws) + lcol;
+				sk[m] = b.sD[m * K + grp < nb && c < cmax ? c : cmax - 1];
+#pragma unroll
+				for(int k = 0; k < G; ++k) {
+					v[k][m] = 0;
+					if((rm[m] >> (k * 4 + grp)) & 1)
+						v[k][m] = row[k][c < c1[k] ? c : c1[k] - 1];
+				}
+			}
+#pragma unroll
+			for(int m = 0; m < BB; ++m) {
+				const int c = ((bl0 + (int) ((pk[m] >> (8 * grp)) & 255u)) << ws) + lcol;
+#pragma unroll
+				for(int k = 0; k < G; ++k) {
+					if(!((rm[m] >> (k * 4 + grp)) & 1)) continue;
+					const double d = Elem<ET>::get(v[k][m], bs);
+					const double x = qcrit(n, n, d, sDr[k], sk[m]);
+					if(c < c1[k] && 0 <= d && qarg_better(x, c, q[k], idx[k])) {
+						q[k] = x;
+						idx[k] = c;
+					}
+				}
+			}
+		}
+		p0 += LB_PIECE << ws;
+	} while(WS < LB_SH_MAX && p0 < cmax);
 	long long span = 0;
 #pragma unroll
 	for(int k = 0; k < G; ++k) span += act[k] ? c1[k] - c0 : 0;
 	return span - loaded;
 }
-
-template <int ET, class Rows, class Tail = NoTail, bool STREAM = false, int PRUNE = 0, bool CMP = false, bool LB = false>
-__global__ __launch_bounds__(TB) void k_dnj_scan_v(const typename Elem<ET>::T *__restrict__ D, double bs, TreeBufs b,
+#define LB_SCAN_WAVES(ET, PRUNE, LB) ((LB) && (LB) < LB_SH_MAX && (ET) == 8 && (PRUNE) == 0 ? 6 : 1)
+template <class F>
+static inline void lb_width_dispatch(int sh, F f) {
+	switch(sh) {
+		case 4: f(std::integral_constant<int, 4>()); break;
+		case 5: f(std::integral_constant<int, 5>()); break;
+		default: f(std::integral_constant<int, 6>()); break;
+	}
+}
+
+template <int ET, class Rows, class Tail = NoTail, bool STREAM = false, int PRUNE = 0, bool CMP = false, int LB = 0>
+__global__ __launch_bounds__(TB) __attribute__((amdgpu_waves_per_eu(LB_SCAN_WAVES(ET, PRUNE, LB))))
+void k_dnj_scan_v(const typename Elem<ET>::T *__restrict__ D, double bs, TreeBufs b,
                                                    int n, Rows rows, int seg, Tail tail = Tail()) {
 	typedef typename Elem<ET>::T T;
 	static_assert(!(LB && PRUNE == 1), "the block bounds serve the compacted scan (its S units fold elsewhere)");
@@ -1507,7 +1557,7 @@
 		if(LB) {
 			double q = DBL_MAX;
 			int idx = 0;
-			lbskip += lb_unit<ET>(row, bs, b, n, r, c0, c1, sDr, q, idx);
+			lbskip += lb_unit_w<ET, LB ? LB : LB_SH_MAX>(row, bs, b, n, r, c0, c1, sDr, q, idx, -1, 0.0, false);
 			qarg_wave_reduce(q, idx);
 			tail_unit(tail, b, n, u, ua, ua + dcdiv(r, seg), r, q, idx, e, Tn);
 			return;
@@ -1984,7 +2034,7 @@
 		atomicAdd((unsigned long long *) &ctl->cells_pruned, (unsigned long long) pruned);
 }
 
-template <int ET, int G, int UC, bool PRUNE2, bool LB = false>
+template <int ET, int G, int UC, bool PRUNE2, int LB = 0>
 __global__ __launch_bounds__(TB) void k_dnj_scan_gc(const typename Elem<ET>::T *__restrict__ D, double bs, TreeBufs b,
                                                     int n, int seg) {
 	typedef typename Elem<ET>::T T;
@@ -2045,7 +2095,7 @@
 			q[t] = DBL_MAX;
 			idx[t] = 0;
 		}
-		if(LB) lbskip += lb_unit_g<ET, G>(row, bs, b, n, r, act, c0, c1, cmax, sDr, q, idx);
+		if(LB) lbskip += lb_unit_gw<ET, G, LB ? LB : LB_SH_MAX>(row, bs, b, n, r, act, c0, c1, cmax, sDr, q, idx);
 		for(int base = c0; !LB && base < cmax; base += 64 * UC) {
 			double sk[UC];
 			T vv[G][UC];
diff --git a/ccphylo_amd/csrc/ccg_tree_common.h b/ccphylo_amd/csrc/ccg_tree_common.h
--- a/ccphylo_amd/csrc/ccg_tree_common.h
+++ b/ccphylo_amd/csrc/ccg_tree_common.h
@@ -107,12 +107,14 @@
 	double *msd;
 	double *ubq;
 	long long lbs;
+	int lbsh;
 	int lbw;
 	int xs_allpre;
 	long long *lbskip;
 };
 
-#define LBW 64
+#define LB_SH_MAX 6
+#define LB_SH_MIN 4
 #define LB_SLOT 16
 #define LB_SCAN 4096
 #define LB_HELP 8192
@@ -164,6 +166,31 @@
 	const int inc = wave_incl_sum(v);
 	*total = __builtin_amdgcn_readlane(inc, 63);
 	return inc - v;
+}
+
+__device__ __forceinline__ unsigned group_min_u32(unsigned v, int ws) {
+#define S_(C, R)                                                          \
+	{                                                                     \
+		const unsigned t_ = (unsigned) dpp_i<C, R>((int) 0xFFFFFFFFu, (int) v); \
+		v = t_ < v ? t_ : v;                                              \
+	}
+	S_(DPP_ROW_SHR1, 0xF) S_(DPP_ROW_SHR2, 0xF) S_(DPP_ROW_SHR4, 0xF) S_(DPP_ROW_SHR8, 0xF)
+	if(ws >= 5) S_(DPP_ROW_BCAST15, 0xA)
+	if(ws >= 6) S_(DPP_ROW_BCAST31, 0xC)
+#undef S_
+	return v;
+}
+__device__ __forceinline__ double group_max_d(double x, int ws) {
+#define S_(C, R)                                   \
+	{                                              \
+		const double t_ = dpp_d<C, R>(-DBL_MAX, x); \
+		x = t_ > x ? t_ : x;                       \
+	}
+	S_(DPP_ROW_SHR1, 0xF) S_(DPP_ROW_SHR2, 0xF) S_(DPP_ROW_SHR4, 0xF) S_(DPP_ROW_SHR8, 0xF)
+	if(ws >= 5) S_(DPP_ROW_BCAST15, 0xA)
+	if(ws >= 6) S_(DPP_ROW_BCAST31, 0xC)
+#undef S_
+	return x;
 }
 
 __device__ __forceinline__ double wave_sum_fixed(double x) {
diff --git a/ccphylo_amd/csrc/ccg_tree_run.h b/ccphylo_amd/csrc/ccg_tree_run.h
--- a/ccphylo_amd/csrc/ccg_tree_run.h
+++ b/ccphylo_amd/csrc/ccg_tree_run.h
@@ -154,12 +154,14 @@
 
 struct LbLayout {
 	long long LS;
+	int sh;
 	size_t lbb, msb, ubb, skb;
 	size_t bytes() const { return lbb + msb + ubb + skb; }
 };
-static inline LbLayout lb_layout(int n0, long long owned_rows) {
+static inline LbLayout lb_layout(int n0, long long owned_rows, int sh) {
 	LbLayout l;
-	l.LS = (n0 + LBW - 1) / LBW;
+	l.sh = sh;
+	l.LS = (n0 + (1 << sh) - 1) >> sh;
 	l.lbb = ((size_t) owned_rows * l.LS * 4 + 255) & ~(size_t) 255;
 	l.msb = ((size_t) (l.LS + 1) * 8 + 255) & ~(size_t) 255;
 	l.ubb = ((size_t) n0 * 8 + 255) & ~(size_t) 255;
@@ -172,10 +174,19 @@
 	b.msd = (double *) (m + l.lbb);
 	b.ubq = (double *) (m + l.lbb + l.msb);
 	b.lbs = l.LS;
+	b.lbsh = l.sh;
 	b.lbw = lbw;
 	b.lbskip = (long long *) (m + l.lbb + l.msb + l.ubb);
 	CCG_CHECK(hipMemsetAsync(b.lbskip, 0, l.skb, st));
 	return CCG_OK;
+}
+template <class Take>
+static inline bool lb_alloc_fit(int n0, long long owned_rows, int sh, Take take, LbLayout *l) {
+	for(; sh <= LB_SH_MAX; ++sh) {
+		*l = lb_layout(n0, owned_rows, sh);
+		if(take(l->bytes()) == CCG_OK) return true;
+	}
+	return false;
 }
 static inline int lb_harvest(const TreeBufs &b, size_t slots, hipStream_t st, TreeCtl &h) {
 	if(!b.lbskip) return CCG_OK;
diff --git a/ccphylo_amd/csrc/tree.hip b/ccphylo_amd/csrc/tree.hip
--- a/ccphylo_amd/csrc/tree.hip
+++ b/ccphylo_amd/csrc/tree.hip
@@ -80,9 +80,10 @@
 	if(b.lbm) {
 		const bool rowj = k < j;
 		const unsigned x = lb_bits(Elem<ET>::get(v, bs));
-		const unsigned mn = wave_min_u32(rowj ? x : 0xFFFFFFFFu);
-		if((threadIdx.x & 63) == 0 && k < j) b.lbm[(long long) j * b.lbs + (k >> 6)] = mn;
-		if(k > j && k < n && k != i) __hip_atomic_fetch_min(b.lbm + (long long) k * b.lbs + (j >> 6), x, __ATOMIC_RELAXED, __HIP_MEMORY_SCOPE_AGENT);
+		const int ws = b.lbsh, wl = (1 << ws) - 1;
+		const unsigned mn = group_min_u32(rowj ? x : 0xFFFFFFFFu, ws);
+		if((threadIdx.x & wl) == wl && k - wl < j) b.lbm[(long long) j * b.lbs + (k >> ws)] = mn;
+		if(k > j && k < n && k != i) __hip_atomic_fetch_min(b.lbm + (long long) k * b.lbs + (j >> ws), x, __ATOMIC_RELAXED, __HIP_MEMORY_SCOPE_AGENT);
 	}
 	update_partials(b, n, exact, k, d, cnt, slot);
 	if(exact) xs_join_row(b, n, slot, d, xs_tag(n));
@@ -140,25 +141,27 @@
 	const int lane = threadIdx.x & 63;
 	const int r = blockIdx.x * (TB / 64) + (threadIdx.x >> 6);
 	if(r >= n) return;
-	if(r < (n + LBW - 1) / LBW) {
-		const int c = r * LBW + lane;
-		const double mx = wave_max_d(c < n ? b.sD[c] : -DBL_MAX);
-		if(lane == 0) b.msd[r] = mx;
+	const int ws = b.lbsh, wl = (1 << ws) - 1;
+	if(r < (n + 63) / 64) {
+		const int c = r * 64 + lane;
+		const double mx = group_max_d(c < n ? b.sD[c] : -DBL_MAX, ws);
+		if((lane & wl) == wl && c - wl < n) b.msd[c >> ws] = mx;
 	}
 	if(lane == 0) b.ubq[r] = INFINITY;
 	const typename Elem<ET>::T *row = D + tri(r);
-	const int nbk = (r + LBW - 1) / LBW;
+	const int nbk = (r + 63) / 64;
 	for(int u0 = 0; u0 < nbk; u0 += BB) {
 		unsigned x[BB];
 #pragma unroll
 		for(int m = 0; m < BB; ++m) {
-			const int c = (u0 + m) * LBW + lane;
+			const int c = (u0 + m) * 64 + lane;
 			x[m] = u0 + m < nbk && c < r ? lb_bits(Elem<ET>::get(row[c], bs)) : 0xFFFFFFFFu;
 		}
 #pragma unroll
 		for(int m = 0; m < BB; ++m) {
-			const unsigned mn = wave_min_u32(x[m]);
-			if(lane == 0 && u0 + m < nbk) b.lbm[(long long) r * b.lbs + u0 + m] = mn;
+			const int c = (u0 + m) * 64 + lane;
+			const unsigned mn = group_min_u32(x[m], ws);
+			if((lane & wl) == wl && c - wl < r) b.lbm[(long long) r * b.lbs + (c >> ws)] = mn;
 		}
 	}
 }
@@ -908,14 +911,16 @@
 	}
 	if(b.lbm) {
 		const unsigned x = lb_bits(Elem<ET>::get(vm, bs));
+		const int ws = b.lbsh, wl = (1 << ws) - 1;
+		const bool last = (lane & wl) == wl;
 		if(move) {
-			const unsigned mn = wave_min_u32(k < i ? x : 0xFFFFFFFFu);
-			if(lane == 0 && k < i) b.lbm[(long long) i * b.lbs + (k >> 6)] = mn;
-			if(k > i && k < nn) __hip_atomic_fetch_min(b.lbm + (long long) k * b.lbs + (i >> 6), x, __ATOMIC_RELAXED, __HIP_MEMORY_SCOPE_AGENT);
+			const unsigned mn = group_min_u32(k < i ? x : 0xFFFFFFFFu, ws);
+			if(last && k - wl < i) b.lbm[(long long) i * b.lbs + (k >> ws)] = mn;
+			if(k > i && k < nn) __hip_atomic_fetch_min(b.lbm + (long long) k * b.lbs + (i >> ws), x, __ATOMIC_RELAXED, __HIP_MEMORY_SCOPE_AGENT);
 		}
 		const double sf = k < nn ? (move && k == i ? sDm : sDk) : -DBL_MAX;
-		const double mx = wave_max_d(sf);
-		if(lane == 0 && k < nn) b.msd[k >> 6] = mx;
+		const double mx = group_max_d(sf, ws);
+		if(last && k - wl < nn) b.msd[k >> ws] = mx;
 	}
 	double vk = DBL_MAX, qpc = INFINITY;
 	if(PV && k >= 1 && k < nn && k != i && k != j) {
@@ -1571,6 +1576,7 @@
 	b.msd = NULL;
 	b.ubq = NULL;
 	b.lbs = 0;
+	b.lbsh = LB_SH_MAX;
 	b.lbw = 0;
 	b.lbskip = NULL;
 	b.xs_allpre = getenv("CCG_XS_ALLPRE") && atoi(getenv("CCG_XS_ALLPRE")) != 0;
@@ -1638,14 +1644,14 @@
 			else k_dnj_scan_w<ET, GEN><<<f.grid, TB, 0, st>>>(D, bs, b, n, dr, seg);
 			break;
 		case SCAN_WAVE16:
-			if(f.lb && f.prune == 2) k_dnj_scan_v<ET, DenseRows, NoTail, false, 2, true, true><<<f.grid, TB, 0, st>>>(D, bs, b, n, dr, seg);
-			else if(f.lb) k_dnj_scan_v<ET, DenseRows, NoTail, false, 0, true, true><<<f.grid, TB, 0, st>>>(D, bs, b, n, dr, seg);
+			if(f.lb && f.prune == 2) lb_width_dispatch(b.lbsh, [&](auto ws) { k_dnj_scan_v<ET, DenseRows, NoTail, false, 2, true, decltype(ws)::value><<<f.grid, TB, 0, st>>>(D, bs, b, n, dr, seg); });
+			else if(f.lb) lb_width_dispatch(b.lbsh, [&](auto ws) { k_dnj_scan_v<ET, DenseRows, NoTail, false, 0, true, decltype(ws)::value><<<f.grid, TB, 0, st>>>(D, bs, b, n, dr, seg); });
 			else if(f.stream) launch_scan_v<ET, true>(f, st, D, bs, b, n, seg);
 			else launch_scan_v<ET, false>(f, st, D, bs, b, n, seg);
 			break;
 		case SCAN_GROUP:
 		case SCAN_GROUP_CMP:
-			if(f.lb) k_dnj_scan_gc<ET, 4, 8, false, true><<<f.grid, TB, 0, st>>>(D, bs, b, n, seg);
+			if(f.lb) lb_width_dispatch(b.lbsh, [&](auto ws) { k_dnj_scan_gc<ET, 4, 8, false, decltype(ws)::value><<<f.grid, TB, 0, st>>>(D, bs, b, n, seg); });
 			else if(f.G == 8) launch_scan_g<ET, 8, 4>(f, st, D, bs, b, n, seg);
 			else launch_scan_g<ET, 4, 8>(f, st, D, bs, b, n, seg);
 			break;
@@ -1870,9 +1876,9 @@
 	CCG_TRY(run.read_ctl(h));
 	const bool general = h.has_missing != 0 || resumed_counts;
 	if(a->method == CCG_TREE_DNJ && !general && g_grid.lb && n0 > g_grid.lb_min_n) {
-		const LbLayout lb = lb_layout(n0, n0);
+		LbLayout lb;
 		void *lbmem = NULL;
-		if(ccg_ctx_workspace(ctx, CCG_WS_TREE_LB, lb.bytes(), &lbmem) == CCG_OK) {
+		if(lb_alloc_fit(n0, n0, g_grid.lb_sh, [&](size_t bytes) { return ccg_ctx_workspace(ctx, CCG_WS_TREE_LB, bytes, &lbmem); }, &lb)) {
 			CCG_TRY(lb_bind(b, lbmem, lb, 0, st));
 			k_lb_init<ET><<<cdiv(n0, TB / 64), TB, 0, st>>>(D, n0, bs, b);
 			launches += 1;
@@ -1882,9 +1888,13 @@
 			if(!cmp_env) {
 				const ScanForm f = dnj_scan_form(g_grid, n0, ET, false, true);
 				int per_cu = 0;
-				const void *fn = f.prune == 2 ? (const void *) k_dnj_scan_v<ET, DenseRows, NoTail, false, 2, true, true>
-				                              : (const void *) k_dnj_scan_v<ET, DenseRows, NoTail, false, 0, true, true>;
-				if(f.kernel == SCAN_GROUP_CMP) fn = (const void *) k_dnj_scan_gc<ET, 4, 8, false, true>;
+				const void *fn = NULL;
+				lb_width_dispatch(b.lbsh, [&](auto ws) {
+					constexpr int WS = decltype(ws)::value;
+					fn = f.prune == 2 ? (const void *) k_dnj_scan_v<ET, DenseRows, NoTail, false, 2, true, WS>
+					                  : (const void *) k_dnj_scan_v<ET, DenseRows, NoTail, false, 0, true, WS>;
+					if(f.kernel == SCAN_GROUP_CMP) fn = (const void *) k_dnj_scan_gc<ET, 4, 8, false, WS>;
+				});
 				CCG_CHECK(hipOccupancyMaxActiveBlocksPerMultiprocessor(&per_cu, fn, TB, 0));
 				const int cus = ctx->cus > 0 && ctx->cus < ctx->ncu ? ctx->cus : ctx->ncu;
 				g_grid.cmp_blocks = per_cu * cus > 64 ? per_cu * cus : 64;
diff --git a/ccphylo_amd/csrc/tree_shard_dnj.hip b/ccphylo_amd/csrc/tree_shard_dnj.hip
--- a/ccphylo_amd/csrc/tree_shard_dnj.hip
+++ b/ccphylo_amd/csrc/tree_shard_dnj.hip
@@ -355,12 +355,13 @@
 	}
 	if(b.lbm) {
 		const unsigned x = lb_bits(Elem<ET>::get(v, bs));
+		const int ws = b.lbsh, wl = (1 << ws) - 1;
 		if(sh.owns(j)) {
-			const unsigned mn = wave_min_u32(k < j ? x : 0xFFFFFFFFu);
-			if((tid & 63) == 0 && k < j) lb_line(b, j)[k >> 6] = mn;
+			const unsigned mn = group_min_u32(k < j ? x : 0xFFFFFFFFu, ws);
+			if((tid & wl) == wl && k - wl < j) lb_line(b, j)[k >> ws] = mn;
 		}
 		if(k > j && k < n && k != i && sh.owns(k))
-			__hip_atomic_fetch_min(lb_line(b, k) + (j >> 6), x, __ATOMIC_RELAXED, __HIP_MEMORY_SCOPE_AGENT);
+			__hip_atomic_fetch_min(lb_line(b, k) + (j >> ws), x, __ATOMIC_RELAXED, __HIP_MEMORY_SCOPE_AGENT);
 	}
 	update_partials(b, n, s_exact, k, d, cnt, blockIdx.x);
 	if(s_exact) xs_join_row(b, n, blockIdx.x, d, xs_tag(n));
@@ -500,17 +501,19 @@
 	if((size_t) k * 4 < rec_slot(n, sh.world).f_off) ((unsigned *) R)[k] = 0;
 	if(b.lbm) {
 		const unsigned x = lb_bits(Elem<ET>::get(vm, bs));
+		const int ws = b.lbsh, wl = (1 << ws) - 1;
+		const bool last = (lane & wl) == wl;
 		if(move) {
 			if(sh.owns(i)) {
-				const unsigned mn = wave_min_u32(k < i ? x : 0xFFFFFFFFu);
-				if(lane == 0 && k < i) lb_line(b, i)[k >> 6] = mn;
+				const unsigned mn = group_min_u32(k < i ? x : 0xFFFFFFFFu, ws);
+				if(last && k - wl < i) lb_line(b, i)[k >> ws] = mn;
 			}
 			if(k > i && k < nn && sh.owns(k))
-				__hip_atomic_fetch_min(lb_line(b, k) + (i >> 6), x, __ATOMIC_RELAXED, __HIP_MEMORY_SCOPE_AGENT);
+				__hip_atomic_fetch_min(lb_line(b, k) + (i >> ws), x, __ATOMIC_RELAXED, __HIP_MEMORY_SCOPE_AGENT);
 		}
 		const double sf = k < nn ? (move && k == i ? sDm : sDk) : -DBL_MAX;
-		const double mx = wave_max_d(sf);
-		if(lane == 0 && k < nn) b.msd[k >> 6] = mx;
+		const double mx = group_max_d(sf, ws);
+		if(last && k - wl < nn) b.msd[k >> ws] = mx;
 	}
 	double qpc = INFINITY;
 	if(PV && k >= 1 && k < nn && k != i && k != j && sh.owns(k)) {
@@ -603,28 +606,30 @@
 	const int lane = threadIdx.x & 63;
 	const int w = blockIdx.x * (TB / 64) + (threadIdx.x >> 6);
 	if(w >= n) return;
-	if(w < (n + LBW - 1) / LBW) {
-		const int c = w * LBW + lane;
-		const double mx = wave_max_d(c < n ? b.sD[c] : -DBL_MAX);
-		if(lane == 0) b.msd[w] = mx;
+	const int ws = b.lbsh, wl = (1 << ws) - 1;
+	if(w < (n + 63) / 64) {
+		const int c = w * 64 + lane;
+		const double mx = group_max_d(c < n ? b.sD[c] : -DBL_MAX, ws);
+		if((lane & wl) == wl && c - wl < n) b.msd[c >> ws] = mx;
 	}
 	if(lane == 0) b.ubq[w] = INFINITY;
 	const int r = ((w >> 3) * sh.world + sh.rank) * 8 + (w & 7);
 	if(r >= n) return;
 	const typename Elem<ET>::T *row = D + sh.off(r);
 	unsigned *line = lb_line(b, r);
-	const int nbk = (r + LBW - 1) / LBW;
+	const int nbk = (r + 63) / 64;
 	for(int u0 = 0; u0 < nbk; u0 += BB) {
 		unsigned x[BB];
 #pragma unroll
 		for(int m = 0; m < BB; ++m) {
-			const int c = (u0 + m) * LBW + lane;
+			const int c = (u0 + m) * 64 + lane;
 			x[m] = u0 + m < nbk && c < r ? lb_bits(Elem<ET>::get(row[c], bs)) : 0xFFFFFFFFu;
 		}
 #pragma unroll
 		for(int m = 0; m < BB; ++m) {
-			const unsigned mn = wave_min_u32(x[m]);
-			if(lane == 0 && u0 + m < nbk) line[u0 + m] = mn;
+			const int c = (u0 + m) * 64 + lane;
+			const unsigned mn = group_min_u32(x[m], ws);
+			if((lane & wl) == wl && c - wl < r) line[c >> ws] = mn;
 		}
 	}
 }
@@ -737,8 +742,8 @@
 	CCG_TRY(shd_init_hnj<ET>(D, n0, bs, sh, cr, st, b, R));
 	run.launches += 2;
 	if(grid.lb && n0 > grid.lb_min_n) {
-		const LbLayout lb = lb_layout(n0, (long long) cdiv(cdiv(n0, 8), sh.world) * 8);
-		if(lbmem.alloc(lb.bytes()) == CCG_OK) {
+		LbLayout lb;
+		if(lb_alloc_fit(n0, (long long) cdiv(cdiv(n0, 8), sh.world) * 8, grid.lb_sh, [&](size_t bytes) { return lbmem.alloc(bytes); }, &lb)) {
 			CCG_TRY(lb_bind(b, lbmem.p, lb, sh.world, st));
 			k_shd_lb_init<ET><<<cdiv(n0, TB / 64), TB, 0, st>>>(D, n0, bs, b, sh);
 			CCG_CHECK(hipGetLastError());
@@ -761,8 +766,8 @@
 			const RecTail<ET> rt{D, sh, Sl, pcnt};
 			switch(f.kernel) {
 				case SCAN_WAVE16:
-					if(f.lb && f.stream) k_dnj_scan_v<ET, Shard, RecTail<ET>, true, 0, false, true><<<f.grid, TB, 0, st>>>(D, bs, b, n, sh, seg, rt);
-					else if(f.lb) k_dnj_scan_v<ET, Shard, RecTail<ET>, false, 0, false, true><<<f.grid, TB, 0, st>>>(D, bs, b, n, sh, seg, rt);
+					if(f.lb && f.stream) lb_width_dispatch(b.lbsh, [&](auto ws) { k_dnj_scan_v<ET, Shard, RecTail<ET>, true, 0, false, decltype(ws)::value><<<f.grid, TB, 0, st>>>(D, bs, b, n, sh, seg, rt); });
+					else if(f.lb) lb_width_dispatch(b.lbsh, [&](auto ws) { k_dnj_scan_v<ET, Shard, RecTail<ET>, false, 0, false, decltype(ws)::value><<<f.grid, TB, 0, st>>>(D, bs, b, n, sh, seg, rt); });
 					else if(f.stream) k_dnj_scan_v<ET, Shard, RecTail<ET>, true><<<f.grid, TB, 0, st>>>(D, bs, b, n, sh, seg, rt);
 					else k_dnj_scan_v<ET, Shard, RecTail<ET>><<<f.grid, TB, 0, st>>>(D, bs, b, n, sh, seg, rt);
 					break;
```
